# TheoCoombes/ClipCap

Measured on AMD Instinct MI355X. Metric: train samples/sec (512-d prefix, 40-tok caption), higher is better.
Workload: dtype bf16; 1 GPU; BASELINE configs[1]: TransformerMapper(8L,P=L=10,H=8)+frozen GPT-2-small; per_gpu_batch=256, global_batch=256, encoder_dim=512, train_language_model=False, parallelism=dp1

## Files before the change

clipcap_amd/csrc/api.hip:

```cpp
#include "../../include/clipcap_hip.h"
#include "gemm_api.h"
#include "kernels.h"
#include "shared.h"
#include "layout.h"
#include <vector>

using namespace CC_NS;

namespace {

#define CC_TIMED(site, st, expr)                 \
    do {                                         \
        cc_shared::ProfScope _ps(site, st);      \
        int _e = (expr);                         \
        if (_e != CC_OK) return _e;              \
    } while (0)

struct TileScope {
    int old;
    bool on;
    explicit TileScope(int mode) : old(cc_shared::g_gemm_tile_mode), on(mode != -2) { if (on) cc_shared::g_gemm_tile_mode = mode; }
    ~TileScope() { if (on) cc_shared::g_gemm_tile_mode = old; }
};
inline int env_tile(const char* name) {
// ... 29 lines not shown
    Carver cv(ws);
    const int S = c->W * c->P + c->L;
    const size_t M = (size_t)B * S, D = c->D;
    w.emb16 = cv.take<act_t>((size_t)B * c->W * c->E);
    w.lin_tmp = c->W > 1 ? cv.take<float>((size_t)B * c->W * c->P * D) : nullptr;
    const int nx = save ? c->N + 1 : 2;
    float* xb[MAX_LAYERS + 1];
    for (int i = 0; i < nx; i++) xb[i] = cv.take<float>(M * D);
    for (int l = 0; l <= c->N; l++) w.x[l] = save ? xb[l] : xb[l & 1];
    const int nl = save ? c->N : 1;
    for (int l = 0; l < c->N; l++) {
        const bool fresh = l < nl;
        w.x1[l] = fresh ? cv.take<float>(M * D) : w.x1[0];
        w.xn1[l] = fresh ? cv.take<act_t>(M * D) : w.xn1[0];
        w.xn2[l] = fresh ? cv.take<act_t>(M * D) : w.xn2[0];
        w.qkv[l] = fresh ? cv.take<act_t>(M * 3 * D) : w.qkv[0];
        w.att[l] = fresh ? cv.take<act_t>(M * D) : w.att[0];
        w.h[l] = fresh ? cv.take<act_t>(M * c->Hm) : w.h[0];
        w.lse[l] = fresh ? cv.take<float>((size_t)B * c->H * S) : w.lse[0];
        w.mean1[l] = fresh ? cv.take<float>(M) : w.mean1[0];
        w.rstd1[l] = fresh ? cv.take<float>(M) : w.rstd1[0];
        w.mean2[l] = fresh ? cv.take<float>(M) : w.mean2[0];
        w.rstd2[l] = fresh ? cv.take<float>(M) : w.rstd2[0];
    }
    if (save) {
        w.dx32 = cv.take<float>(M * D);
        w.dx16 = cv.take<act_t>(M * D);
        w.dx16b = cv.take<act_t>(M * D);
        w.dh16 = cv.take<act_t>(M * c->Hm);
        w.dxn16 = cv.take<act_t>(M * D);
        w.datt16 = cv.take<act_t>(M * D);
        w.dqkv16 = cv.take<act_t>(M * 3 * D);
        w.dlin16 = cv.take<act_t>((size_t)B * c->W * c->P * D);
        w.own_grads = !kX3 && M <= (size_t)kDeferRows && c->N <= 8;
        for (int l = 0; l < c->N; l++) {
            const bool own = w.own_grads;
            w.gdx[l] = own ? cv.take<act_t>(M * D) : w.dx16;
            w.gdxb[l] = own ? cv.take<act_t>(M * D) : w.dx16b;
            w.gdh[l] = own ? cv.take<act_t>(M * c->Hm) : w.dh16;
            w.gdqkv[l] = own ? cv.take<act_t>(M * 3 * D) : w.dqkv16;
        }
        w.wg_scratch = cv.take<float>(WGRAD_SCRATCH_BYTES / sizeof(float));
        w.red = cv.take<float>(RED_SCRATCH_FLOATS);
        w.adelta = cv.take<float>((size_t)B * c->H * S);
        w.gimg = kX3 ? reinterpret_cast<uint16_t*>(cv.take<char>(x3_img(M, std::max<size_t>(3 * (size_t)D, c->Hm)))) : nullptr;
    } else {
        w.dx32 = nullptr; w.dx16 = w.dx16b = w.dh16 = w.dxn16 = w.datt16 = w.dqkv16 = w.dlin16 = nullptr; w.wg_scratch = nullptr; w.adelta = nullptr;
        w.red = nullptr;
        w.gimg = nullptr;
        for (int l = 0; l < c->N; l++) w.gdx[l] = w.gdxb[l] = w.gdh[l] = w.gdqkv[l] = nullptr;
        w.own_grads = false;
    }
    w.x3 = nullptr; w.x3_bytes = 0;
    if (kX3) {
        const size_t Hm = c->Hm, Mb = (size_t)B * c->W, PD = (size_t)c->P * D;
        size_t need = std::max(x3_img(Mb, c->E), x3_img(M, std::max(D, Hm)));
        if (save) {
            need = std::max(need, x3_img(M, 3 * D));
            need = std::max(need, std::max(x3_img(M, D) + x3_img(M, Hm), x3_img(M, 3 * D) + x3_img(M, D)));
            need = std::max(need, x3_img(Mb, PD) + x3_img(Mb, c->E));
        }
        w.x3_bytes = need;
        w.x3 = cv.take<char>(need);
    }
    w.bytes = cv.bytes();
}

struct MapperPass {
    hipStream_t st;
    MapperOff o;
    MapperWS w;
    Call cx;
    int D, PP, S, M, H, hd, Hm, PD;
    MapperPass(const cc_mapper_cfg* c, int B, int save, void* ws, void* stream)
        : st(S_(stream)), o(c), D(c->D), PP(c->W * c->P), S(PP + c->L), M(B * S), H(c->H), hd(c->D / c->H), Hm(c->Hm), PD(c->P * c->D) {
        mapper_carve(c, B, save, ws, w);
        cx = call_of(st, w);
    }
};

static bool x3_img_on() {
    static const bool on = []() { const char* e = cc_lab_env("CC_X3_IMG"); return !e || atoi(e) != 0; }();
    return on;
}
static bool lm_exp_form(const cc_gpt2_shape* s) {
    static const bool env = []() { const char* e = cc_lab_env("CC_LM_EXPFORM"); return !e || atoi(e) != 0; }();
    if (CC_OP == 0) return env;
    if (CC_OP == 2) return env && x3_img_on() && s->mode == 1;
    return false;
}
static Act lm_logits(const cc_gpt2_cfg* c, const cc_gpt2_shape* s, act_t* logits16) { return Act(logits16, (kX3 && lm_exp_form(s)) ? c->Vp : 0); }

struct Gpt2WS {
    float* x[MAX_LAYERS + 1];
    float* x1[MAX_LAYERS];
    act_t *qkv[MAX_LAYERS], *u[MAX_LAYERS];
    Act xn1[MAX_LAYERS], xn2[MAX_LAYERS], att[MAX_LAYERS], hact[MAX_LAYERS];
    float *lse[MAX_LAYERS], *mean1[MAX_LAYERS], *rstd1[MAX_LAYERS], *mean2[MAX_LAYERS], *rstd2[MAX_LAYERS];
    act_t* hf16;
    float *meanf, *rstdf;
    int *target, *row_map;
    int* keep;
    act_t* logits16;
    float *pmax, *psum, *tgt_logit, *lse_row, *row_loss;
    float *cref, *lmfac;
    act_t* hfs16;
    float* dx32;
    Act dx16, dx16b, du16, dqkv16;
    act_t *dhf16, *dxn16, *datt16;
    float* wg_scratch;
    float* red;
    void* scat;
    float* adelta;
    char* x3;
    size_t x3_bytes;
    size_t bytes;
};

void gpt2_carve(const cc_gpt2_cfg* c, const cc_gpt2_shape* s, int cap, void* ws, Gpt2WS& w) {
    Carver cv(ws);
    const int B = s->B, T = s->T, hd = c->D / c->H;
    const size_t M = (size_t)B * T, D = c->D, Mc = (size_t)B * cap;
    const bool keep = s->mode >= 1, full = s->mode >= 2;
    const auto take_img = [&](size_t n) { return cv.take<act_t>(n * ((kX3 && !full) ? 3 : 2) / 2); };
    const bool img = kX3 && !full && x3_img_on();
    const bool bimg = img && keep && s->p_resid == 0.f && s->p_attn == 0.f && s->p_embd == 0.f;
    const int xw = img ? (int)D : 0, attw = (img && attn_fwd_can_image(T, hd)) ? (int)D : 0, hw = img ? 4 * (int)D : 0;
    const int dxw = bimg ? (int)D : 0, dqw = (bimg && attn_bwd_can_image(T, hd)) ? 3 * (int)D : 0;
    const int nx = keep ? c->NL + 1 : 2;
    float* xb[MAX_LAYERS + 1];
    for (int i = 0; i < nx; i++) xb[i] = cv.take<float>(M * D);
    for (int l = 0; l <= c->NL; l++) w.x[l] = keep ? xb[l] : xb[l & 1];
    for (int l = 0; l < c->NL; l++) {
        const bool k0 = keep || l == 0, f0 = full || l == 0;
        w.x1[l] = k0 ? cv.take<float>(M * D) : w.x1[0];
        w.qkv[l] = k0 ? cv.take<act_t>(M * 3 * D) : w.qkv[0];
        w.u[l] = k0 ? cv.take<act_t>(M * 4 * D) : w.u[0];
        w.lse[l] = k0 ? cv.take<float>((size_t)B * c->H * T) : w.lse[0];
        w.mean1[l] = k0 ? cv.take<float>(M) : w.mean1[0];
        w.rstd1[l] = k0 ? cv.take<float>(M) : w.rstd1[0];
        w.mean2[l] = k0 ? cv.take<float>(M) : w.mean2[0];
        w.rstd2[l] = k0 ? cv.take<float>(M) : w.rstd2[0];
        w.xn1[l] = f0 ? Act(take_img(M * D), xw) : w.xn1[0];
        w.xn2[l] = f0 ? Act(take_img(M * D), xw) : w.xn2[0];
        w.att[l] = k0 ? Act(take_img(M * D), attw) : w.att[0];
        w.hact[l] = f0 ? Act(take_img(M * 4 * D), hw) : w.hact[0];
    }
    const size_t Mh = std::max(M, Mc);
    w.hf16 = cv.take<act_t>(Mh * D);
    w.meanf = cv.take<float>(Mh);
    w.rstdf = cv.take<float>(Mh);
    w.target = cv.take<int>(Mh);
    w.row_map = cv.take<int>(Mh);
    w.keep = nullptr;
    if (keep) {
        const int npart = c->Vp / 64;
        w.logits16 = take_img(Mc * c->Vp);
        w.pmax = cv.take<float>(Mc * npart);
        w.psum = cv.take<float>(Mc * npart);
        w.tgt_logit = cv.take<float>(Mc);
        w.lse_row = cv.take<float>(Mc);
        w.row_loss = cv.take<float>(Mc);
        w.cref = cv.take<float>(Mc);
        w.lmfac = cv.take<float>(2 * Mc);
        w.hfs16 = full ? cv.take<act_t>(Mc * D) : nullptr;
        w.dx32 = cv.take<float>(M * D);
        w.dx16 = Act(take_img(M * D), dxw);
        w.dx16b = full ? Act(cv.take<act_t>(M * D)) : w.dx16;
        w.dhf16 = cv.take<act_t>(Mc * D);
        w.du16 = Act(take_img(M * 4 * D), hw);
        w.dxn16 = cv.take<act_t>(M * D);
        w.datt16 = cv.take<act_t>(M * D);
        w.dqkv16 = Act(take_img(M * 3 * D), dqw);
        w.wg_scratch = full ? cv.take<float>(WGRAD_SCRATCH_BYTES / sizeof(float)) : nullptr;
        w.red = full ? cv.take<float>(RED_SCRATCH_FLOATS) : nullptr;
        w.scat = full ? cv.take<char>(scatter_ws_bytes((int)Mc, (int)D)) : nullptr;
        w.adelta = cv.take<float>((size_t)B * c->H * T);
    } else {
        w.wg_scratch = nullptr; w.adelta = nullptr; w.red = nullptr; w.scat = nullptr;
        w.logits16 = nullptr; w.pmax = w.psum = w.tgt_logit = w.lse_row = w.row_loss = nullptr;
        w.cref = w.lmfac = nullptr; w.hfs16 = nullptr;
        w.dx32 = nullptr; w.dx16 = w.dx16b = w.du16 = w.dqkv16 = Act(); w.dhf16 = w.dxn16 = w.datt16 = nullptr;
        if (Mc > 0) {
            const int npart = c->Vp / 64;
            w.pmax = cv.take<float>(Mc * npart);
            w.psum = cv.take<float>(Mc * npart);
            w.tgt_logit = cv.take<float>(Mc);
            w.lse_row = cv.take<float>(Mc);
            w.keep = cv.take<int>(Mc);
        }
    }
    w.x3 = nullptr; w.x3_bytes = 0;
    if (kX3) {
        size_t need = x3_img(Mh, 4 * D);
        if (keep) need = std::max(need, x3_img(Mc, c->Vp));
        if (full) need = std::max(need, std::max(x3_img(M, D) + x3_img(M, 4 * D), x3_img(Mc, c->Vp) + x3_img(Mc, D)));
        w.x3_bytes = need;
        w.x3 = cv.take<char>(need);
    }
    w.bytes = cv.bytes();
}

struct Gpt2Pass {
    hipStream_t st;
    Gpt2Off o;
    Gpt2WS w;
    Call cx;
    int D, M, H, hd;
    Gpt2Pass(const cc_gpt2_cfg* c, const cc_gpt2_shape* s, int cap, void* ws, void* stream)
        : st(S_(stream)), o(c), D(c->D), M(s->B * s->T), H(c->H), hd(c->D / c->H) {
        gpt2_carve(c, s, cap, ws, w);
        cx = call_of(st, w);
    }
};

}

extern "C" {

int CC_API(cc_mapper_bwd_range)(const cc_mapper_cfg* c, int32_t B, const float* w32, const uint16_t* w16, void* ws, const float* dout, float* g32,
                        int32_t l_hi, int32_t l_lo, void* stream);
int CC_API(cc_gpt2_bwd_range)(const cc_gpt2_cfg* c, const cc_gpt2_shape* s, const float* w32, const uint16_t* w16, void* ws, const int64_t* tokens,
                      float* dprefix, float* g32, int32_t l_hi, int32_t l_lo, void* stream);

int64_t CC_API(cc_mapper_param_count)(const cc_mapper_cfg* cfg) {
    if (!mapper_cfg_ok(cfg)) return CC_ERR_SHAPE;
    return MapperOff(cfg).total;
}

int CC_API(cc_mapper_param_offsets)(const cc_mapper_cfg* cfg, int64_t* offs) {
    if (!mapper_cfg_ok(cfg) || !offs) return CC_ERR_SHAPE;
    const MapperOff o(cfg);
    *offs++ = o.lin_w; *offs++ = o.lin_b; *offs++ = o.prefix; *offs++ = o.pos;
    for (int l = 0; l < cfg->N; l++) offs = put_layer(offs, o.layer(l));
    return CC_OK;
}

int64_t CC_API(cc_mapper_ws_bytes)(const cc_mapper_cfg* cfg, int32_t B, int32_t save) {
    if (!mapper_cfg_ok(cfg) || B <= 0) return CC_ERR_SHAPE;
    MapperWS w;
    mapper_carve(cfg, B, save, nullptr, w);
    return (int64_t)w.bytes;
}

#if CC_OP == 2
static int mapper_sync_x3(const cc_mapper_cfg* c, const float* w32, uint16_t* w16, hipStream_t st) {
    const MapperOff o(c);
    const int D = c->D, Hm = c->Hm;
    X3SplitBatch sb;
    sb.add(w32 + o.lin_w, W16(w16, o.lin_w), c->P * D, c->E, 0, 1);
    for (int l = 0; l < c->N; l++) {
        const auto y = o.layer(l);
        const int64_t off[4] = {y.wq, y.wp, y.w1, y.w2};
        const int R[4] = {3 * D, D, Hm, D}, C[4] = {D, D, D, Hm};
        for (int i = 0; i < 4; i++) {
            if (sb.n + 2 > 32) { CC_TRY(x3_split_multi(sb, st)); sb.n = 0; }
            sb.add(w32 + off[i], W16(w16, off[i]), R[i], C[i], 0, 1);
            sb.add(w32 + off[i], W16(w16, o.total + off[i]), R[i], C[i], 1, 1);
        }
    }
    return x3_split_multi(sb, st);
}
#endif

static int mapper_transposes(const cc_mapper_cfg* c, uint16_t* w16, hipStream_t st) {
    if (kX3) return CC_ERR_ARG;
    const MapperOff o(c);
    op16_t* t = w16 + o.total;
    const int D = c->D, Hm = c->Hm;
    TransposeBatch tb;
    for (int l = 0; l < c->N; l++) {
        const auto y = o.layer(l);
        tb.add(w16 + y.wq, t + y.wq, 3 * D, D);
        tb.add(w16 + y.wp, t + y.wp, D, D);
        tb.add(w16 + y.w1, t + y.w1, Hm, D);
        tb.add(w16 + y.w2, t + y.w2, D, Hm);
        if (tb.n == 32) { CC_TRY(transpose_bf16_multi(tb, st)); tb.n = 0; }
    }
    CC_TRY(transpose_bf16_multi(tb, st));
    return CC_OK;
}

int CC_API(cc_mapper_sync_weights)(const cc_mapper_cfg* c, const float* w32, uint16_t* w16, void* stream) {
    if (!mapper_cfg_ok(c) || !w32 || !w16) return CC_ERR_ARG;
    hipStream_t st = S_(stream);
#if CC_OP == 2
    return mapper_sync_x3(c, w32, w16, st);
#else
    CC_TRY(f32_to_bf16(w32, w16, (size_t)MapperOff(c).total, st));
    return mapper_transposes(c, w16, st);
#endif
}

int CC_API(cc_mapper_transpose_weights)(const cc_mapper_cfg* c, uint16_t* w16, void* stream) {
    if (!mapper_cfg_ok(c) || !w16) return CC_ERR_ARG;
    return mapper_transposes(c, w16, S_(stream));
}

int CC_API(cc_mapper_fwd)(const cc_mapper_cfg* c, int32_t B, const float* w32, const uint16_t* w16, const float* emb, void* ws, float* out,
                  int32_t save, void* stream) {
    if (!mapper_cfg_ok(c) || B <= 0 || !w32 || !w16 || !emb || !ws || !out) return CC_ERR_ARG;
    MapperPass ps(c, B, save, ws, stream);
    auto& [st, o, w, cx, D, PP, S, M, H, hd, Hm, PD] = ps;
    CC_TRY(f32_to_act(emb, w.emb16, (size_t)B * c->W * c->E, st));
    if (c->W == 1) {
        CC_TRY(gemm_f32out(0, 0, w.emb16, c->E, W16(w16, o.lin_w), c->E, B, PD, c->E, w.x[0], S * D, w32 + o.lin_b, 0, 1.0f, 1, cx));
    } else {
        CC_TRY(gemm_f32out(0, 0, w.emb16, c->E, W16(w16, o.lin_w), c->E, B * c->W, PD, c->E, w.lin_tmp, PD, w32 + o.lin_b, 0, 1.0f, 1, cx));
        CC_TRY(copy_rows(w.lin_tmp, (size_t)PP * D, w.x[0], (size_t)S * D, PP * D, B, st));
        if (o.pos >= 0) CC_TRY(add_rows(w.x[0], (size_t)S * D, w32 + o.pos, PP * D, B, st));
    }
    CC_TRY(broadcast_rows(w.x[0] + (size_t)PP * D, (size_t)S * D, w32 + o.prefix, c->L * D, B, st));
    for (int l = 0; l < c->N; l++) {
        const auto y = o.layer(l);
        CC_TRY(ln_fwd(w.x[l], D, nullptr, w32 + y.n1w, w32 + y.n1b, w.xn1[l], nullptr, w.mean1[l], w.rstd1[l], M, D, st));
        CC_TIMED(CC_SITE_MAPPER_QKV_FWD, st, gemm_bf16out(0, 0, w.xn1[l], D, W16(w16, y.wq), D, M, 3 * D, D, w.qkv[l], 3 * D, nullptr, 0, nullptr, cx));
        CC_TRY(attn_fwd(w.qkv[l], B, S, H, hd, false, w.att[l], w.lse[l], st));
        CC_TRY(gemm_resid(0, 0, w.att[l], D, W16(w16, y.wp), D, M, D, D, w.x1[l], w.x[l], D, w32 + y.bp, cx));
        CC_TRY(ln_fwd(w.x1[l], D, nullptr, w32 + y.n2w, w32 + y.n2b, w.xn2[l], nullptr, w.mean2[l], w.rstd2[l], M, D, st));
        CC_TIMED(CC_SITE_MAPPER_FC1_FWD, st, gemm_bf16out(0, 0, w.xn2[l], D, W16(w16, y.w1), D, M, Hm, D, w.h[l], Hm, w32 + y.b1, 1, nullptr, cx));
        CC_TRY(gemm_resid(0, 0, w.h[l], Hm, W16(w16, y.w2), Hm, M, D, Hm, w.x[l + 1], w.x1[l], D, w32 + y.b2, cx));
    }
    CC_TRY(copy_rows(w.x[c->N] + (size_t)PP * D, (size_t)S * D, out, (size_t)c->L * D, c->L * D, B, st));
    return CC_OK;
}

int CC_API(cc_mapper_attention_probs)(const cc_mapper_cfg* c, int32_t B, void* ws, int32_t layer, float* out, void* stream) {
    if (!mapper_cfg_ok(c) || B <= 0 || !ws || !out || layer < 0 || layer >= c->N) return CC_ERR_ARG;
    MapperPass ps(c, B, 1, ws, stream);
    return attn_probs(ps.w.qkv[layer], B, ps.S, ps.H, ps.hd, out, ps.st);
}

int CC_API(cc_mapper_bwd)(const cc_mapper_cfg* c, int32_t B, const float* w32, const uint16_t* w16, void* ws, const float* dout, float* g32,
                  void* stream) {
    if (!mapper_cfg_ok(c)) return CC_ERR_ARG;
    return CC_API(cc_mapper_bwd_range)(c, B, w32, w16, ws, dout, g32, c->N, 0, stream);
}

int CC_API(cc_mapper_bwd_range)(const cc_mapper_cfg* c, int32_t B, const float* w32, const uint16_t* w16, void* ws, const float* dout, float* g32,
                        int32_t l_hi, int32_t l_lo, void* stream) {
    if (!mapper_cfg_ok(c) || B <= 0 || !w32 || !w16 || !ws || !dout || !g32 || l_lo < 0 || l_hi > c->N || l_lo > l_hi) return CC_ERR_ARG;
    MapperPass ps(c, B, 1, ws, stream);
    auto& [st, o, w, cx, D, PP, S, M, H, hd, Hm, PD] = ps;
    const uint16_t* w16t = W16(w16, o.total);
    if (l_hi == c->N) {
        if (hipMemsetAsync(w.dx32, 0, (size_t)M * D * sizeof(float), st) != hipSuccess) return CC_ERR_LAUNCH;
        CC_TRY(copy_rows(dout, (size_t)c->L * D, w.dx32 + (size_t)PP * D, (size_t)S * D, c->L * D, B, st));
        if (c->N > 0) CC_TRY(f32_to_act(w.dx32, w.gdx[c->N - 1], (size_t)M * D, st));
    }
    WgradBatch wb;
    wb.defer = true;
    constexpr bool kDeferAll = !kX3;
    static const bool defer_all_on = []() { const char* e = cc_lab_env("CC_MAPPER_WGRAD_DEFER"); return !e || atoi(e) != 0; }();
    static const int defer_rows = []() { const char* e = cc_lab_env("CC_MAPPER_DEFER_ROWS"); return e ? std::min(atoi(e), kDeferRows) : kDeferRows; }();
    const bool defer_all = kDeferAll && defer_all_on && w.own_grads && 4 * (l_hi - l_lo) <= 32 && M <= defer_rows;
    if (defer_all) { wb.direct = true; wb.cap = 4 * (l_hi - l_lo); }
    ColsumBatch cs;
#if CC_OP == 2
    static const bool share = []() { const char* e = cc_lab_env("CC_X3_SHARE"); return !e || atoi(e) != 0; }();
    int g2rc = CC_OK;
    auto G2 = [&](const act_t* t, int width) -> ActIn {
        if (!share) return t;
        auto& [st, o, w, cx, D, PP, S, M, H, hd, Hm, PD] = ps;
        g2rc = x3_split_rows(t, (size_t)width, w.gimg, M, width, 0, st);
        return ActIn(reinterpret_cast<const act_t*>(w.gimg), width);
    };
#else
    auto G2 = [&](const act_t* t, int) -> ActIn { return t; };
    const int g2rc = CC_OK;
#endif
    for (int l = l_hi - 1; l >= l_lo; l--) {
        const auto y = o.layer(l);
        act_t* dx16 = w.gdx[l];
        act_t* dx16b = w.gdxb[l];
        act_t* dh16 = w.gdh[l];
        act_t* dqkv16 = w.gdqkv[l];
        act_t* dx16_below = l > 0 ? w.gdx[l - 1] : w.datt16;
        const ActIn gx = G2(dx16, D);
        CC_TRY(g2rc);
        CC_TIMED(CC_SITE_MAPPER_WGRAD_FC2, st, gemm_wgrad(gx, D, w.h[l], Hm, D, Hm, M, g32 + y.w2, Hm, w.wg_scratch, cx, &wb));
        if (l == c->N - 1) CC_TRY(colsum_bf16(dx16, D, M, D, g32 + y.b2, cx));
        CC_TRY(gemm_dact(0, 0, gx, D, W16(w16t, y.w2), D, M, Hm, D, dh16, Hm, w.h[l], 1, cx));
        const ActIn gh = G2(dh16, Hm);
        CC_TRY(g2rc);
        CC_TRY(gemm_wgrad(gh, Hm, w.xn2[l], D, Hm, D, M, g32 + y.w1, D, w.wg_scratch, cx, &wb));
        if (defer_all) cs.add(dh16, g32 + y.b1);
        else CC_TRY(colsum_bf16(dh16, Hm, M, Hm, g32 + y.b1, cx));
        CC_TRY(gemm_bf16out(0, 0, gh, Hm, W16(w16t, y.w1), Hm, M, D, Hm, w.dxn16, D, nullptr, 0, nullptr, cx));
        CC_TRY(ln_bwd(w.dxn16, w.x1[l], D, nullptr, w.mean2[l], w.rstd2[l], w32 + y.n2w, w.dx32, w.dx32, dx16b, g32 + y.n2w,
                      g32 + y.n2b, M, D, cx, g32 + y.bp));
        const ActIn gb = G2(dx16b, D);
        CC_TRY(g2rc);
        CC_TRY(gemm_wgrad(gb, D, w.att[l], D, D, D, M, g32 + y.wp, D, w.wg_scratch, cx, &wb));
        CC_TRY(gemm_bf16out(0, 0, gb, D, W16(w16t, y.wp), D, M, D, D, w.datt16, D, nullptr, 0, nullptr, cx));
        CC_TRY(attn_bwd(w.qkv[l], w.datt16, w.att[l], w.lse[l], w.adelta, B, S, H, hd, false, dqkv16, st));
        const ActIn gq = G2(dqkv16, 3 * D);
        CC_TRY(g2rc);
        CC_TRY(gemm_wgrad(gq, 3 * D, w.xn1[l], D, 3 * D, D, M, g32 + y.wq, D, w.wg_scratch, cx, &wb));
        CC_TRY(gemm_bf16out(0, 0, gq, 3 * D, W16(w16t, y.wq), 3 * D, M, D, 3 * D, w.dxn16, D, nullptr, 0, nullptr, cx));
        if (!defer_all) CC_TRY(wgrad_flush(wb, st));
        CC_TRY(ln_bwd(w.dxn16, w.x[l], D, nullptr, w.mean1[l], w.rstd1[l], w32 + y.n1w, w.dx32, w.dx32, dx16_below, g32 + y.n1w,
                      g32 + y.n1b, M, D, cx, l > 0 ? g32 + o.layer(l - 1).b2 : nullptr));
    }
    CC_TRY(wgrad_flush(wb, st));
    CC_TRY(colsum_bf16_multi(cs, Hm, M, Hm, cx));
    if (l_lo > 0) return CC_OK;
    CC_TRY(batch_sum(w.dx32 + (size_t)PP * D, (size_t)S * D, g32 + o.prefix, c->L * D, B, cx));
    if (o.pos >= 0) CC_TRY(batch_sum(w.dx32, (size_t)S * D, g32 + o.pos, PP * D, B, cx));
    CC_TRY(slice_f32_to_bf16(w.dx32, (size_t)S * D, w.dlin16, (size_t)PP * D, PP * D, B, st));
    CC_TRY(gemm_wgrad(w.dlin16, PD, w.emb16, c->E, PD, c->E, B * c->W, g32 + o.lin_w, c->E, w.wg_scratch, cx));
    CC_TRY(colsum_bf16(w.dlin16, PD, B * c->W, PD, g32 + o.lin_b, cx));
    return CC_OK;
}

namespace {
static bool gelu_grad_fwd() {
    static const bool on = []() { const char* e = cc_lab_env("CC_GELU_GRAD_FWD"); return !e || atoi(e) != 0; }();
    return on;
}
static bool shape_ok(const cc_gpt2_cfg* c, const cc_gpt2_shape* s) {
    return s && s->B > 0 && s->T > 0 && s->L >= 0 && s->L <= s->T && s->cap >= s->T - s->L && s->mode >= 0 && s->mode <= 2 && s->T <= c->NPOS &&
           s->p_embd >= 0.f && s->p_embd < 1.f && s->p_attn >= 0.f && s->p_attn < 1.f && s->p_resid >= 0.f && s->p_resid < 1.f;
}
}

int64_t CC_API(cc_gpt2_param_count)(const cc_gpt2_cfg* cfg) {
    if (!gpt2_cfg_ok(cfg)) return CC_ERR_SHAPE;
    return Gpt2Off(cfg).total;
}

int CC_API(cc_gpt2_param_offsets)(const cc_gpt2_cfg* cfg, int64_t* offs) {
    if (!gpt2_cfg_ok(cfg) || !offs) return CC_ERR_SHAPE;
    const Gpt2Off o(cfg);
    *offs++ = o.wte; *offs++ = o.wpe;
    for (int l = 0; l < cfg->NL; l++) offs = put_layer(offs, o.layer(l));
    *offs++ = o.lnf_w; *offs++ = o.lnf_b;
    return CC_OK;
}

int64_t CC_API(cc_gpt2_ws_bytes)(const cc_gpt2_cfg* cfg, const cc_gpt2_shape* s) {
    if (!gpt2_cfg_ok(cfg) || !shape_ok(cfg, s)) return CC_ERR_SHAPE;
    Gpt2WS w;
    gpt2_carve(cfg, s, s->T - s->L, nullptr, w);
    return (int64_t)w.bytes;
}

#if CC_OP == 2
static int gpt2_sync_x3(const cc_gpt2_cfg* c, const float* w32, uint16_t* w16, hipStream_t st) {
    const Gpt2Off o(c);
    const int D = c->D;
    X3SplitBatch sb;
    sb.add(w32 + o.wte, W16(w16, o.wte), c->Vp, D, 0, 1);
    sb.add(w32 + o.wte, W16(w16, o.total + o.wte), c->Vp, D, 1, 1);
    CC_TRY(x3_split_multi(sb, st));
    sb.n = 0;
    for (int l = 0; l < c->NL; l++) {
        const auto y = o.layer(l);
        const int64_t off[4] = {y.aw, y.pw, y.fw, y.p2w};
        const int R[4] = {D, D, D, 4 * D}, C[4] = {3 * D, D, 4 * D, D};
        for (int i = 0; i < 4; i++) {
            if (sb.n + 2 > 32) { CC_TRY(x3_split_multi(sb, st)); sb.n = 0; }
            sb.add(w32 + off[i], W16(w16, off[i]), R[i], C[i], 0, 1);
            sb.add(w32 + off[i], W16(w16, o.total + off[i]), R[i], C[i], 1, 1);
        }
    }
    return x3_split_multi(sb, st);
}
#endif

static int gpt2_transposes(const cc_gpt2_cfg* c, uint16_t* w16, hipStream_t st) {
    if (kX3) return CC_ERR_ARG;
    const Gpt2Off o(c);
    op16_t* t = w16 + o.total;
    const int D = c->D;
    CC_TRY(transpose_bf16(w16 + o.wte, t + o.wte, c->Vp, D, st));
    TransposeBatch tb;
    for (int l = 0; l < c->NL; l++) {
        const auto y = o.layer(l);
        tb.add(w16 + y.aw, t + y.aw, D, 3 * D);
        tb.add(w16 + y.pw, t + y.pw, D, D);
        tb.add(w16 + y.fw, t + y.fw, D, 4 * D);
        tb.add(w16 + y.p2w, t + y.p2w, 4 * D, D);
        if (tb.n == 32) { CC_TRY(transpose_bf16_multi(tb, st)); tb.n = 0; }
    }
    CC_TRY(transpose_bf16_multi(tb, st));
    return CC_OK;
}

int CC_API(cc_gpt2_sync_weights)(const cc_gpt2_cfg* c, const float* w32, uint16_t* w16, void* stream) {
    if (!gpt2_cfg_ok(c) || !w32 || !w16) return CC_ERR_ARG;
    hipStream_t st = S_(stream);
#if CC_OP == 2
    return gpt2_sync_x3(c, w32, w16, st);
#else
    CC_TRY(f32_to_bf16(w32, w16, (size_t)Gpt2Off(c).total, st));
    return gpt2_transposes(c, w16, st);
#endif
}

int CC_API(cc_gpt2_transpose_weights)(const cc_gpt2_cfg* c, uint16_t* w16, void* stream) {
    if (!gpt2_cfg_ok(c) || !w16) return CC_ERR_ARG;
    return gpt2_transposes(c, w16, S_(stream));
}

int CC_API(cc_dropout_mask)(uint64_t seed, int32_t site, int32_t layer, float p, int64_t n, uint8_t* out, void* stream) {
    if (!out || n < 0 || site < 0 || site > 3 || layer < 0 || layer > 255 || p < 0.f || p >= 1.f) return CC_ERR_ARG;
    return dropout_mask_u8(out, (size_t)n, make_drop(p, seed, (unsigned)site, (unsigned)layer), S_(stream));
}

int CC_API(cc_gpt2_embed)(const cc_gpt2_cfg* c, const cc_gpt2_shape* s, const float* w32, const float* prefix, const int64_t* tokens, void* ws,
                  void* stream) {
    if (!gpt2_cfg_ok(c) || !shape_ok(c, s) || !w32 || !ws || (s->L > 0 && !prefix) || (s->T > s->L && !tokens)) return CC_ERR_ARG;
    Gpt2Pass ps(c, s, s->T - s->L, ws, stream);
    auto& [st, o, w, cx, D, M, H, hd] = ps;
    CC_TRY(embed_concat(prefix, reinterpret_cast<const long long*>(tokens), s->cap, w32 + o.wte, w32 + o.wpe, w.x[0], s->B, s->L, s->T, D, 0, st));
    return dropout_f32(w.x[0], (size_t)s->B * s->T * D, make_drop(s->p_embd, s->drop_seed, DROP_EMBD, 0), st);
}

int CC_API(cc_gpt2_embed_from)(const cc_gpt2_cfg* c, const cc_gpt2_shape* s, const float* w32, const float* inputs_embeds, void* ws,
                       void* stream) {
    if (!gpt2_cfg_ok(c) || !shape_ok(c, s) || !w32 || !ws || !inputs_embeds) return CC_ERR_ARG;
    Gpt2Pass ps(c, s, s->T - s->L, ws, stream);
    return embed_concat(inputs_embeds, nullptr, 0, w32 + ps.o.wte, w32 + ps.o.wpe, ps.w.x[0], s->B, s->T, s->T, ps.D, 0, ps.st);
}

int CC_API(cc_gpt2_fwd)(const cc_gpt2_cfg* c, const cc_gpt2_shape* s, const float* w32, const uint16_t* w16, void* ws, void* stream) {
    if (!gpt2_cfg_ok(c) || !shape_ok(c, s) || !w32 || !w16 || !ws) return CC_ERR_ARG;
    Gpt2Pass ps(c, s, s->T - s->L, ws, stream);
    auto& [st, o, w, cx, D, M, H, hd] = ps;
    const uint16_t* w16t = W16(w16, o.total);
    for (int l = 0; l < c->NL; l++) {
        const auto y = o.layer(l);
        CC_TRY(ln_fwd(w.x[l], D, nullptr, w32 + y.l1w, w32 + y.l1b, w.xn1[l], nullptr, w.mean1[l], w.rstd1[l], M, D, st));
        CC_TRY(gemm_bf16out(0, 0, w.xn1[l], D, W16(w16t, y.aw), D, M, 3 * D, D, w.qkv[l], 3 * D, w32 + y.ab, 0, nullptr, cx));
        CC_TRY(attn_fwd(w.qkv[l], s->B, s->T, H, hd, true, w.att[l], w.lse[l], st, make_drop(s->p_attn, s->drop_seed, DROP_ATTN, l)));
        {
            static const int tile_proj = env_tile("CC_TILE_PROJ");
            TileScope ts(tile_proj);
            CC_TRY(gemm_resid(0, 0, w.att[l], D, W16(w16t, y.pw), D, M, D, D, w.x1[l], w.x[l], D, w32 + y.pb, cx,
                              make_drop(s->p_resid, s->drop_seed, DROP_RESID_ATTN, l)));
        }
        CC_TRY(ln_fwd(w.x1[l], D, nullptr, w32 + y.l2w, w32 + y.l2b, w.xn2[l], nullptr, w.mean2[l], w.rstd2[l], M, D, st));
        {
            static const int tile_fc = env_tile("CC_TILE_FC");
            TileScope ts(tile_fc);
            CC_TIMED(CC_SITE_GPT2_FC_FWD, st, gemm_bf16out(0, 0, w.xn2[l], D, W16(w16t, y.fw), D, M, 4 * D, D, w.hact[l], 4 * D, w32 + y.fb, (s->mode >= 1 && gelu_grad_fwd()) ? 3 : 2,
                                                            s->mode >= 1 ? w.u[l] : nullptr, cx));
        }
        {
            static const int tile_proj2 = env_tile("CC_TILE_PROJ2");
            TileScope ts(tile_proj2);
            CC_TIMED(CC_SITE_GPT2_PROJ2_FWD, st, gemm_resid(0, 0, w.hact[l], 4 * D, W16(w16t, y.p2w), 4 * D, M, D, 4 * D, w.x[l + 1], w.x1[l], D, w32 + y.p2b, cx,
                                                           make_drop(s->p_resid, s->drop_seed, DROP_RESID_MLP, l)));
        }
    }
    return CC_OK;
}

int CC_API(cc_gpt2_logits)(const cc_gpt2_cfg* c, const cc_gpt2_shape* s, const float* w32, const uint16_t* w16, void* ws, float* logits,
                   int64_t ldl, void* stream) {
    if (!gpt2_cfg_ok(c) || !shape_ok(c, s) || !w32 || !w16 || !ws || !logits) return CC_ERR_ARG;
    const int Ns = std::min(c->Vp, rup(c->V, 8));
    if (ldl < Ns || (ldl & 3) || ldl > 0x7fffffff) return CC_ERR_SHAPE;
    Gpt2Pass ps(c, s, s->T - s->L, ws, stream);
    auto& [st, o, w, cx, D, M, H, hd] = ps;
    CC_TRY(ln_fwd(w.x[c->NL], D, nullptr, w32 + o.lnf_w, w32 + o.lnf_b, w.hf16, nullptr, w.meanf, w.rstdf, M, D, st));
    return gemm_f32out(0, 0, w.hf16, D, W16(w16, o.wte), D, M, Ns, D, logits, (int)ldl, nullptr, 0, 1.0f, 1, cx);
}

int CC_API(cc_lmhead_ce_fwd)(const cc_gpt2_cfg* c, const cc_gpt2_shape* s, const float* w32, const uint16_t* w16, void* ws, const int64_t* tokens,
                     float* stats, void* stream) {
    if (!gpt2_cfg_ok(c) || !shape_ok(c, s) || s->mode < 1 || s->L < 1 || !w32 || !w16 || !ws || !tokens || !stats) return CC_ERR_ARG;
    const int cap = s->T - s->L;
    if (cap != s->cap) return CC_ERR_SHAPE;
    Gpt2Pass ps(c, s, cap, ws, stream);
    auto& [st, o, w, cx, D, M, H, hd] = ps;
    const int Mc = s->B * cap, npart = c->Vp / 64;
    if (hipMemsetAsync(stats, 0, 2 * sizeof(float), st) != hipSuccess) return CC_ERR_LAUNCH;
    CC_TRY(ce_targets(reinterpret_cast<const long long*>(tokens), w.target, w.row_map, s->B, cap, s->L, s->T, st));
    CC_TRY(ln_fwd(w.x[c->NL], D, w.row_map, w32 + o.lnf_w, w32 + o.lnf_b, w.hf16, nullptr, w.meanf, w.rstdf, Mc, D, st));
    const bool ef = lm_exp_form(s);
    const op16_t* wte_rows = kX3 ? reinterpret_cast<const op16_t*>(w32 + o.wte) : W16(w16, o.wte);
    if (ef) CC_TRY(lm_tgt_ref(w.hf16, wte_rows, D, w.target, w.cref, Mc, st));
    CC_TIMED(CC_SITE_LMHEAD_FWD, st, gemm_lmhead(w.hf16, D, W16(w16, o.wte), D, Mc, c->Vp, c->V, D, lm_logits(c, s, w.logits16), c->Vp, w.pmax, w.psum, npart, w.target, w.tgt_logit, cx,
                                                 ef ? w.cref : nullptr));
    CC_TRY(ce_rows(w.pmax, w.psum, npart, w.target, ef ? w.cref : w.tgt_logit, w.lse_row, w.row_loss, stats, Mc, st));
    return CC_OK;
}

int CC_API(cc_lmhead_score)(const cc_gpt2_cfg* c, const cc_gpt2_shape* s, const float* w32, const uint16_t* w16, void* ws, const int64_t* tokens,
                    int32_t ignore_zero, float* token_logprob, float* sample_stats, void* stream) {
    if (!gpt2_cfg_ok(c) || !shape_ok(c, s) || s->mode != 0 || s->L < 1 || !w32 || !w16 || !ws || !tokens || !token_logprob || !sample_stats)
        return CC_ERR_ARG;
    const int cap = s->T - s->L;
    if (cap < 1 || cap != s->cap) return CC_ERR_SHAPE;
    Gpt2Pass ps(c, s, cap, ws, stream);
    auto& [st, o, w, cx, D, M, H, hd] = ps;
    const int Mc = s->B * cap, npart = c->Vp / 64;
    CC_TRY(ce_targets(reinterpret_cast<const long long*>(tokens), w.target, w.row_map, s->B, cap, s->L, s->T, st));
    CC_TRY(score_keep(reinterpret_cast<const long long*>(tokens), w.keep, Mc, ignore_zero, st));
    CC_TRY(ln_fwd(w.x[c->NL], D, w.row_map, w32 + o.lnf_w, w32 + o.lnf_b, w.hf16, nullptr, w.meanf, w.rstdf, Mc, D, st));
    CC_TIMED(CC_SITE_LMHEAD_FWD, st, gemm_lmhead_score(w.hf16, D, W16(w16, o.wte), D, Mc, c->Vp, c->V, D, w.pmax, w.psum, npart, w.target, w.tgt_logit, cx));
    return score_rows(w.pmax, w.psum, npart, w.keep, w.tgt_logit, w.lse_row, token_logprob, sample_stats, s->B, cap, st);
}

int CC_API(cc_lmhead_ce_bwd)(const cc_gpt2_cfg* c, const cc_gpt2_shape* s, const float* w32, const uint16_t* w16, void* ws, const float* denom,
                     const float* loss_scale, float* g32, void* stream) {
    if (!gpt2_cfg_ok(c) || !shape_ok(c, s) || s->mode < 1 || !w32 || !w16 || !ws || !denom || (s->mode == 2 && !g32)) return CC_ERR_ARG;
    const int cap = s->T - s->L;
    Gpt2Pass ps(c, s, cap, ws, stream);
    auto& [st, o, w, cx, D, M, H, hd] = ps;
    const int Mc = s->B * cap;
    const bool full = s->mode == 2;
    const bool ef = lm_exp_form(s);
    const LmFix fix{w.lmfac, w.target, kX3 ? reinterpret_cast<const op16_t*>(w32 + o.wte) : W16(w16, o.wte)};
    if (ef) CC_TRY(lm_rowfac(w.cref, w.lse_row, w.target, denom, loss_scale, w.lmfac, Mc, st));
    const Act lg = lm_logits(c, s, w.logits16);
    ActIn dlog = lg;
    op16_t* dimg = (kX3 && !ef && !full && x3_img_on()) ? x3_scratch_block(cx, x3_img(Mc, c->Vp)) : nullptr;
    if (dimg) dlog = ActIn(reinterpret_cast<const act_t*>(dimg), c->Vp);
    if (!ef) CC_TRY(ce_dlogits(w.logits16, c->Vp, c->V, w.target, w.lse_row, denom, loss_scale, Mc, st, dimg));
    const auto lm_dgrad = [&]() {
        auto& [st, o, w, cx, D, M, H, hd] = ps;
        const int rc = gemm_nt_deepk(dlog, c->Vp, W16(w16, o.total + o.wte), c->Vp, Mc, D, c->Vp, w.dhf16, D, reinterpret_cast<float*>(w.du16.p),
                                     (size_t)M * 4 * D * sizeof(act_t), cx, ef ? &fix : nullptr);
        if (rc != CC_ERR_SHAPE) return rc;
        const int rc2 = gemm_bf16out(0, 0, dlog, c->Vp, W16(w16, o.total + o.wte), c->Vp, Mc, D, c->Vp, w.dhf16, D, nullptr, 0, nullptr, cx);
        return (rc2 != CC_OK || !ef) ? rc2 : lm_dgrad_fix(w.dhf16, w.lmfac, w.target, fix.wte, D, Mc, st);
    };
    CC_TIMED(CC_SITE_LMHEAD_DGRAD, st, lm_dgrad());
    if (full) {
        if (ef) {
            CC_TRY(lm_scale_rows(w.hf16, w.lmfac, w.hfs16, D, Mc, st));
            CC_TRY(gemm_wgrad(lg, c->Vp, w.hfs16, D, c->Vp, D, Mc, g32 + o.wte, D, w.wg_scratch, cx));
            ScatterSrc oh;
            oh.ids32 = w.target; oh.act = w.hf16; oh.fac = w.lmfac;
            CC_TRY(scatter_rows(oh, Mc, D, c->Vp, g32 + o.wte, w.scat, st));
        } else {
            CC_TRY(gemm_wgrad(lg, c->Vp, w.hf16, D, c->Vp, D, Mc, g32 + o.wte, D, w.wg_scratch, cx));
        }
    }
    if (hipMemsetAsync(w.dx32, 0, (size_t)M * D * sizeof(float), st) != hipSuccess) return CC_ERR_LAUNCH;
    const size_t dx16_bytes = (size_t)M * D * (w.dx16.img ? 3 * sizeof(op16_t) : sizeof(act_t));
    if (hipMemsetAsync(w.dx16.p, 0, dx16_bytes, st) != hipSuccess) return CC_ERR_LAUNCH;
    CC_TRY(ln_bwd(w.dhf16, w.x[c->NL], D, w.row_map, w.meanf, w.rstdf, w32 + o.lnf_w, nullptr, w.dx32, w.dx16, full ? g32 + o.lnf_w : nullptr,
                  full ? g32 + o.lnf_b : nullptr, Mc, D, cx));
    return CC_OK;
}

int CC_API(cc_lmhead_put_x)(const cc_gpt2_cfg* c, const cc_gpt2_shape* s, void* ws, const float* x, void* stream) {
    if (!gpt2_cfg_ok(c) || !shape_ok(c, s) || !ws || !x) return CC_ERR_ARG;
    Gpt2Pass ps(c, s, s->T - s->L, ws, stream);
    const size_t bytes = (size_t)s->B * s->T * c->D * sizeof(float);
    return hipMemcpyAsync(ps.w.x[c->NL], x, bytes, hipMemcpyDeviceToDevice, ps.st) == hipSuccess ? CC_OK : CC_ERR_LAUNCH;
}

int CC_API(cc_lmhead_get)(const cc_gpt2_cfg* c, const cc_gpt2_shape* s, void* ws, int32_t field, void* dst, int64_t dst_bytes, void* stream) {
    if (!gpt2_cfg_ok(c) || !shape_ok(c, s) || !ws || !dst || field < CC_LM_LSE || field > CC_LM_DX32) return CC_ERR_ARG;
    if (s->T - s->L < 1) return CC_ERR_SHAPE;
    Gpt2Pass ps(c, s, s->T - s->L, ws, stream);
    const Gpt2WS& w = ps.w;
    const size_t Mc = (size_t)s->B * (s->T - s->L), M = (size_t)s->B * s->T, D = c->D;
    const void* src = nullptr;
    size_t bytes = 0;
    switch (field) {
        case CC_LM_LSE: src = w.lse_row; bytes = Mc * sizeof(float); break;
        case CC_LM_TGT: src = (s->mode >= 1 && lm_exp_form(s)) ? w.cref : w.tgt_logit; bytes = Mc * sizeof(float); break;
        case CC_LM_ROW_LOSS: src = w.row_loss; bytes = Mc * sizeof(float); break;
        case CC_LM_HF: src = w.hf16; bytes = Mc * D * sizeof(act_t); break;
        case CC_LM_DHF: src = w.dhf16; bytes = Mc * D * sizeof(act_t); break;
        default: src = w.dx32; bytes = M * D * sizeof(float); break;
    }
    if (!src) return CC_ERR_STATE;
    if (dst_bytes < 0 || (size_t)dst_bytes != bytes) return CC_ERR_SHAPE;
    return hipMemcpyAsync(dst, src, bytes, hipMemcpyDeviceToDevice, ps.st) == hipSuccess ? CC_OK : CC_ERR_LAUNCH;
}

int CC_API(cc_gpt2_logits_bwd)(const cc_gpt2_cfg* c, const cc_gpt2_shape* s, const float* w32, const uint16_t* w16, void* ws, const float* dlogits,
                       int64_t ldl, float* dx0, float* g32, void* stream) {
    if (!gpt2_cfg_ok(c) || !shape_ok(c, s) || s->mode < 1 || s->L != 0 || !w32 || !w16 || !ws || !dlogits || ldl < c->V || (s->mode == 2 && !g32))
        return CC_ERR_ARG;
    Gpt2Pass ps(c, s, s->T, ws, stream);
    auto& [st, o, w, cx, D, M, H, hd] = ps;
    const bool full = s->mode == 2;
    CC_TRY(f32_to_op16_pad(dlogits, ldl, c->V, w.logits16, c->Vp, M, st));
    CC_TRY(gemm_bf16out(0, 0, w.logits16, c->Vp, W16(w16, o.total + o.wte), c->Vp, M, D, c->Vp, w.dhf16, D, nullptr, 0, nullptr, cx));
    if (full) CC_TRY(gemm_wgrad(w.logits16, c->Vp, w.hf16, D, c->Vp, D, M, g32 + o.wte, D, w.wg_scratch, cx));
    if (hipMemsetAsync(w.dx32, 0, (size_t)M * D * sizeof(float), st) != hipSuccess) return CC_ERR_LAUNCH;
    CC_TRY(ln_bwd(w.dhf16, w.x[c->NL], D, nullptr, w.meanf, w.rstdf, w32 + o.lnf_w, nullptr, w.dx32, w.dx16, full ? g32 + o.lnf_w : nullptr,
                  full ? g32 + o.lnf_b : nullptr, M, D, cx));
    CC_TRY(CC_API(cc_gpt2_bwd_range)(c, s, w32, w16, ws, nullptr, nullptr, g32, c->NL, 0, stream));
    if (dx0 && hipMemcpyAsync(dx0, w.dx32, (size_t)M * D * sizeof(float), hipMemcpyDeviceToDevice, st) != hipSuccess) return CC_ERR_LAUNCH;
    return CC_OK;
}

int CC_API(cc_gpt2_bwd)(const cc_gpt2_cfg* c, const cc_gpt2_shape* s, const float* w32, const uint16_t* w16, void* ws, const int64_t* tokens,
                float* dprefix, float* g32, void* stream) {
    if (!gpt2_cfg_ok(c)) return CC_ERR_ARG;
    return CC_API(cc_gpt2_bwd_range)(c, s, w32, w16, ws, tokens, dprefix, g32, c->NL, 0, stream);
}

int CC_API(cc_gpt2_bwd_range)(const cc_gpt2_cfg* c, const cc_gpt2_shape* s, const float* w32, const uint16_t* w16, void* ws, const int64_t* tokens,
                      float* dprefix, float* g32, int32_t l_hi, int32_t l_lo, void* stream) {
    if (!gpt2_cfg_ok(c) || !shape_ok(c, s) || s->mode < 1 || !w32 || !w16 || !ws || (s->L > 0 && !dprefix) || (s->mode == 2 && !g32) ||
        l_lo < 0 || l_hi > c->NL || l_lo > l_hi)
        return CC_ERR_ARG;
    Gpt2Pass ps(c, s, s->T - s->L, ws, stream);
    auto& [st, o, w, cx, D, M, H, hd] = ps;
    const int D3 = 3 * D, D4 = 4 * D;
    const bool full = s->mode == 2;
    WgradBatch wb;
    wb.defer = full;
    WgradBatch* wbp = full ? &wb : nullptr;
    if (full && (w.dx16.img || w.dx16b.img || w.du16.img || w.dqkv16.img)) return CC_ERR_STATE;
    for (int l = l_hi - 1; l >= l_lo; l--) {
        const auto y = o.layer(l);
        const bool top = l == c->NL - 1;
        if (top) CC_TRY(dropout_bf16(w.dx16.p, (size_t)M * D, make_drop(s->p_resid, s->drop_seed, DROP_RESID_MLP, l), st));
        if (full) {
            CC_TRY(gemm_wgrad(w.hact[l], D4, w.dx16.p, D, D4, D, M, g32 + y.p2w, D, w.wg_scratch, cx, wbp));
            if (top) CC_TRY(colsum_bf16(w.dx16.p, D, M, D, g32 + y.p2b, cx));
        }
        {
            static const int tile_dact = env_tile("CC_TILE_DACT");
            TileScope ts(tile_dact);
            CC_TRY(gemm_dact(0, 0, w.dx16, D, W16(w16, y.p2w), D, M, D4, D, w.du16, D4, w.u[l], gelu_grad_fwd() ? 3 : 2, cx));
        }
        if (full) {
            CC_TRY(gemm_wgrad(w.xn2[l], D, w.du16.p, D4, D, D4, M, g32 + y.fw, D4, w.wg_scratch, cx, wbp));
            CC_TRY(colsum_bf16(w.du16.p, D4, M, D4, g32 + y.fb, cx));
        }
        CC_TIMED(CC_SITE_GPT2_FC_DGRAD, st, gemm_bf16out(0, 0, w.du16, D4, W16(w16, y.fw), D4, M, D, D4, w.dxn16, D, nullptr, 0, nullptr, cx));
        CC_TRY(ln_bwd(w.dxn16, w.x1[l], D, nullptr, w.mean2[l], w.rstd2[l], w32 + y.l2w, w.dx32, w.dx32, w.dx16b, full ? g32 + y.l2w : nullptr,
                      full ? g32 + y.l2b : nullptr, M, D, cx, full ? g32 + y.pb : nullptr,
                      make_drop(s->p_resid, s->drop_seed, DROP_RESID_ATTN, l)));
        if (full) CC_TRY(gemm_wgrad(w.att[l], D, w.dx16b.p, D, D, D, M, g32 + y.pw, D, w.wg_scratch, cx, wbp));
        CC_TRY(gemm_bf16out(0, 0, w.dx16b, D, W16(w16, y.pw), D, M, D, D, w.datt16, D, nullptr, 0, nullptr, cx));
        CC_TRY(attn_bwd(w.qkv[l], w.datt16, w.att[l].p, w.lse[l], w.adelta, s->B, s->T, H, hd, true, w.dqkv16, st,
                        make_drop(s->p_attn, s->drop_seed, DROP_ATTN, l)));
        if (full) {
            CC_TRY(gemm_wgrad(w.xn1[l], D, w.dqkv16.p, D3, D, D3, M, g32 + y.aw, D3, w.wg_scratch, cx, wbp));
            CC_TRY(colsum_bf16(w.dqkv16.p, D3, M, D3, g32 + y.ab, cx));
        }
        CC_TRY(gemm_bf16out(0, 0, w.dqkv16, D3, W16(w16, y.aw), D3, M, D, D3, w.dxn16, D, nullptr, 0, nullptr, cx));
        if (full) CC_TRY(wgrad_flush(wb, st));
        CC_TRY(ln_bwd(w.dxn16, w.x[l], D, nullptr, w.mean1[l], w.rstd1[l], w32 + y.l1w, w.dx32, w.dx32, w.dx16, full ? g32 + y.l1w : nullptr,
                      full ? g32 + y.l1b : nullptr, M, D, cx, (full && l > 0) ? g32 + o.layer(l - 1).p2b : nullptr,
                      l > 0 ? make_drop(s->p_resid, s->drop_seed, DROP_RESID_MLP, l - 1) : Drop()));
    }
    if (l_lo > 0) return CC_OK;
    CC_TRY(dropout_f32(w.dx32, (size_t)M * D, make_drop(s->p_embd, s->drop_seed, DROP_EMBD, 0), st));
    if (s->L > 0) CC_TRY(copy_rows(w.dx32, (size_t)s->T * D, dprefix, (size_t)s->L * D, s->L * D, s->B, st));
    if (full) {
        if (tokens) {
            ScatterSrc e;
            e.ids64 = reinterpret_cast<const long long*>(tokens);
            e.ids_ld = s->cap;
            e.f32 = w.dx32 + (size_t)s->L * D; e.rpb = s->T - s->L; e.bstride = (size_t)s->T * D;
            CC_TRY(scatter_rows(e, s->B * (s->T - s->L), D, c->Vp, g32 + o.wte, w.scat, st));
        }
        CC_TRY(batch_sum(w.dx32, (size_t)s->T * D, g32 + o.wpe, s->T * D, s->B, cx));
    }
    return CC_OK;
}

int CC_API(cc_adamw_step)(float* p32, const float* g32, float* m, float* v, int64_t n, float lr, float beta1, float beta2, float eps,
                  float weight_decay, int32_t step, float grad_scale, const float* loss_scale, const float* found_inf, void* stream) {
    if (!p32 || !g32 || !m || !v || n < 0 || step < 0 || (step == 0 && !loss_scale)) return CC_ERR_ARG;
    return adamw(p32, g32, m, v, (size_t)n, lr, beta1, beta2, eps, weight_decay, step, grad_scale, loss_scale, found_inf, S_(stream));
}

int CC_API(cc_adamw_step_cast)(float* p32, const float* g32, float* m, float* v, int64_t n, float lr, float beta1, float beta2, float eps,
                       float weight_decay, int32_t step, float grad_scale, const float* loss_scale, const float* found_inf, uint16_t* w16, void* stream) {
    if (!p32 || !g32 || !m || !v || !w16 || n < 0 || step < 0 || (step == 0 && !loss_scale)) return CC_ERR_ARG;
    if (kX3) return CC_ERR_ARG;
    return adamw(p32, g32, m, v, (size_t)n, lr, beta1, beta2, eps, weight_decay, step, grad_scale, loss_scale, found_inf, S_(stream), w16);
}

int CC_API(cc_adamw_step_clip)(float* p32, const float* g32, float* m, float* v, int64_t n, float lr, float beta1, float beta2, float eps,
                       float weight_decay, int32_t step, float grad_scale, const float* loss_scale, const float* found_inf, const float* clip,
                       uint16_t* w16, void* stream) {
    if (!p32 || !g32 || !m || !v || n < 0 || step < 0 || (step == 0 && !loss_scale)) return CC_ERR_ARG;
    if (w16 && kX3) return CC_ERR_ARG;
    return adamw(p32, g32, m, v, (size_t)n, lr, beta1, beta2, eps, weight_decay, step, grad_scale, loss_scale, found_inf, S_(stream), w16, clip);
}

int64_t CC_API(cc_grad_norm_scratch_floats)(void) { return (int64_t)GRAD_NORM_BLOCKS; }

int CC_API(cc_grad_sqnorm)(const float* g32, int64_t n, float* scratch, float* sumsq, void* stream) {
    if (!g32 || !scratch || !sumsq || n < 0) return CC_ERR_ARG;
    return grad_sqnorm(g32, (size_t)n, scratch, sumsq, S_(stream));
}

int CC_API(cc_grad_clip_coef)(const float* sumsq, float max_norm, float grad_scale, const float* loss_scale, float* clip, void* stream) {
    if (!sumsq || !clip || !(max_norm >= 0.f)) return CC_ERR_ARG;
    return grad_clip_coef(sumsq, max_norm, grad_scale, loss_scale, clip, S_(stream));
}

int CC_API(cc_cast_op16)(const float* src, uint16_t* dst, int64_t n, void* stream) {
    if (!src || !dst || n < 0 || kX3) return CC_ERR_ARG;
    return f32_to_bf16(src, dst, (size_t)n, S_(stream));
}

int CC_API(cc_grad_wire_pack)(const float* g32, uint16_t* wire, int64_t n, void* stream) {
    if (!g32 || !wire || n < 0) return CC_ERR_ARG;
    return wire_pack(g32, wire, (size_t)n, S_(stream));
}

int CC_API(cc_grad_wire_unpack)(const uint16_t* wire, float* g32, int64_t n, void* stream) {
    if (!g32 || !wire || n < 0) return CC_ERR_ARG;
    return wire_unpack(wire, g32, (size_t)n, S_(stream));
}

int CC_API(cc_grad_nonfinite)(const float* g32, int64_t n, float* found_inf, void* stream) {
    if (!g32 || !found_inf || n < 0) return CC_ERR_ARG;
    return grad_nonfinite(g32, (size_t)n, found_inf, S_(stream));
}

int CC_API(cc_loss_scale_update)(float* state, float* found_inf, float growth, float backoff, int32_t interval, void* stream) {
    if (!state || !found_inf || growth < 1.f || backoff <= 0.f || backoff > 1.f || interval < 1) return CC_ERR_ARG;
    return loss_scale_update(state, found_inf, growth, backoff, interval, S_(stream));
}

int CC_API(cc_gemm_op16_f32)(int32_t al, int32_t bl, const uint16_t* A, int32_t lda, const uint16_t* B, int32_t ldb, int32_t M, int32_t N, int32_t K,
                     float* C, int32_t ldc, const float* bias, int32_t ksplit, void* stream) {
    if (!A || !B || !C || kX3) return CC_ERR_ARG;
    Call cx{S_(stream)};
    return gemm_f32out(al, bl, reinterpret_cast<const act_t*>(A), lda, B, ldb, M, N, K, C, ldc, ksplit > 1 ? nullptr : bias, ksplit > 1 ? 2 : 0, 1.0f, ksplit, cx);
}

int64_t CC_API(cc_wgrad_scratch_bytes)(void) { return (int64_t)WGRAD_SCRATCH_BYTES; }

int CC_API(cc_gemm_wgrad)(const uint16_t* X, int32_t ldx, const uint16_t* Y, int32_t ldy, int32_t Mw, int32_t Nw, int32_t K, float* dW, int32_t ldw,
                  float* scratch, void* stream) {
    if (!X || !Y || !dW || kX3) return CC_ERR_ARG;
    Call cx{S_(stream)};
    return gemm_wgrad(reinterpret_cast<const act_t*>(X), ldx, reinterpret_cast<const act_t*>(Y), ldy, Mw, Nw, K, dW, ldw, scratch, cx);
}

int CC_API(cc_layernorm_fwd)(const float* x, const float* gamma, const float* beta, uint16_t* y, float* mean, float* rstd, int32_t rows, int32_t D,
                     void* stream) {
    if (!x || !gamma || !beta || !y) return CC_ERR_ARG;
    return ln_fwd(x, D, nullptr, gamma, beta, reinterpret_cast<act_t*>(y), nullptr, mean, rstd, rows, D, S_(stream));
}

int64_t CC_API(cc_red_scratch_floats)(void) { return (int64_t)RED_SCRATCH_FLOATS; }

int CC_API(cc_layernorm_bwd)(const uint16_t* dy, const float* x, int32_t ldx, const int32_t* row_map, const float* mean, const float* rstd,
                     const float* gamma, const float* dres, float* dx32, uint16_t* dx16, float* dgamma, float* dbeta, float* dcol, int32_t rows,
                     int32_t D, float* red_ws, void* stream) {
    if (!dy || !x || !mean || !rstd || !gamma || !dx32 || !dgamma != !dbeta || kX3) return CC_ERR_ARG;
    Call cx{S_(stream), red_ws};
    return ln_bwd(reinterpret_cast<const act_t*>(dy), x, ldx, row_map, mean, rstd, gamma, dres, dx32, reinterpret_cast<act_t*>(dx16), dgamma,
                  dbeta, rows, D, cx, dcol);
}

int CC_API(cc_colsum_bf16)(const uint16_t* X, int32_t ld, int32_t M, int32_t N, float* out, float* red_ws, void* stream) {
    if (!X || !out || kX3) return CC_ERR_ARG;
    Call cx{S_(stream), red_ws};
    return colsum_bf16(reinterpret_cast<const act_t*>(X), ld, M, N, out, cx);
}

int CC_API(cc_colsum_multi)(const uint16_t* const* X_host, float* const* out_host, int32_t n, int32_t ld, int32_t M, int32_t N, float* red_ws,
                    void* stream) {
    if (!X_host || !out_host || n < 0 || n > 32 || kX3) return CC_ERR_ARG;
    ColsumBatch b;
    for (int i = 0; i < n; i++) {
        if (!X_host[i] || !out_host[i]) return CC_ERR_ARG;
        b.add(reinterpret_cast<const act_t*>(X_host[i]), out_host[i]);
    }
    Call cx{S_(stream), red_ws};
    return colsum_bf16_multi(b, ld, M, N, cx);
}

int CC_API(cc_batch_sum)(const float* src, int64_t src_stride, float* dst, int32_t len, int32_t B, float* red_ws, void* stream) {
    if (!src || !dst || len < 0 || src_stride < len) return CC_ERR_ARG;
    Call cx{S_(stream), red_ws};
    return batch_sum(src, (size_t)src_stride, dst, len, B, cx);
}

int CC_API(cc_attention_fwd)(const uint16_t* qkv, int32_t B, int32_t S, int32_t H, int32_t hd, int32_t causal, uint16_t* out, float* lse, void* stream) {
    if (!qkv || !out) return CC_ERR_ARG;
    return attn_fwd(reinterpret_cast<const act_t*>(qkv), B, S, H, hd, causal != 0, reinterpret_cast<act_t*>(out), lse, S_(stream));
}

int CC_API(cc_attention_bwd)(const uint16_t* qkv, const uint16_t* dout, const uint16_t* o, const float* lse, float* delta_ws, int32_t B, int32_t S,
                     int32_t H, int32_t hd, int32_t causal, uint16_t* dqkv, void* stream) {
    if (!qkv || !dout || !lse || !dqkv) return CC_ERR_ARG;
    return attn_bwd(reinterpret_cast<const act_t*>(qkv), reinterpret_cast<const act_t*>(dout), reinterpret_cast<const act_t*>(o), lse, delta_ws, B, S, H, hd,
                    causal != 0, reinterpret_cast<act_t*>(dqkv), S_(stream));
}

int CC_API(cc_attention_fwd_x)(const uint16_t* qkv, int32_t B, int32_t S, int32_t H, int32_t hd, int32_t causal, uint16_t* out, int32_t out_img, float* lse,
                       float p, uint64_t seed, int32_t layer, void* stream) {
    if (!qkv || !out || !(p >= 0.f && p < 1.f) || layer < 0 || layer > 255 || out_img < 0 || (!kX3 && out_img)) return CC_ERR_ARG;
    return attn_fwd(reinterpret_cast<const act_t*>(qkv), B, S, H, hd, causal != 0, Act(reinterpret_cast<act_t*>(out), out_img), lse, S_(stream),
                    make_drop(p, seed, DROP_ATTN, (unsigned)layer));
}

int CC_API(cc_attention_bwd_x)(const uint16_t* qkv, const uint16_t* dout, const uint16_t* o, const float* lse, float* delta_ws, int32_t B, int32_t S,
                       int32_t H, int32_t hd, int32_t causal, uint16_t* dqkv, int32_t dqkv_img, float p, uint64_t seed, int32_t layer, void* stream) {
    if (!qkv || !dout || !lse || !dqkv || !(p >= 0.f && p < 1.f) || layer < 0 || layer > 255 || dqkv_img < 0 || (!kX3 && dqkv_img)) return CC_ERR_ARG;
    return attn_bwd(reinterpret_cast<const act_t*>(qkv), reinterpret_cast<const act_t*>(dout), reinterpret_cast<const act_t*>(o), lse, delta_ws, B, S, H, hd,
                    causal != 0, Act(reinterpret_cast<act_t*>(dqkv), dqkv_img), S_(stream), make_drop(p, seed, DROP_ATTN, (unsigned)layer));
}

namespace {
inline bool al16(const void* p) { return ((uintptr_t)p & 15) == 0; }
inline bool hook_operands_ok(int al, int bl, const void* A, int a_img, int lda, const void* B, int ldb, int M, int N, int K) {
    if (!A || !B || !al16(A) || !al16(B) || M <= 0 || N <= 0 || K <= 0 || a_img < 0) return false;
    if (!kX3 && a_img) return false;
    return lda >= (a_img ? 0 : (al ? M : K)) && ldb >= (bl ? N : K);
}
inline void hook_scratch(Call& cx, void* x3, int64_t x3_bytes) {
    if (kX3 && x3 && x3_bytes > 0 && al16(x3)) { cx.x3 = static_cast<char*>(x3); cx.x3_bytes = (size_t)x3_bytes; }
}
inline bool hook_c_img_ok(int c_img, int N) { return c_img == 0 || (kX3 && c_img == N); }
}

int64_t CC_API(cc_x3_image_bytes)(int64_t rows, int64_t depth) {
    if (rows < 0 || depth < 0) return CC_ERR_ARG;
    return (int64_t)x3_img((size_t)rows, (size_t)depth);
}

int CC_API(cc_x3_split_rows)(const float* src, int64_t ld, int32_t rows, int32_t width, int32_t form, uint16_t* dst, void* stream) {
#if CC_OP == 2
    if (!src || !dst || rows < 0 || width < 0 || ld < width || (form != 0 && form != 1)) return CC_ERR_ARG;
    return x3_split_rows(src, (size_t)ld, dst, rows, width, form, S_(stream));
#else
    (void)src; (void)ld; (void)rows; (void)width; (void)form; (void)dst; (void)stream;
    return CC_ERR_ARG;
#endif
}

int CC_API(cc_gemm_act)(int32_t al, int32_t bl, const void* A, int32_t a_img, int32_t lda, const uint16_t* B, int32_t ldb, int32_t M, int32_t N, int32_t K,
                void* C, int32_t c_img, int32_t ldc, const float* bias, int32_t act, void* pre, void* x3, int64_t x3_bytes, void* stream) {
    if (!hook_operands_ok(al, bl, A, a_img, lda, B, ldb, M, N, K) || !C || !al16(C) || !al16(pre) || !al16(bias) || ldc < N || act < 0 || act > 3 ||
        !hook_c_img_ok(c_img, N))
        return CC_ERR_ARG;
    Call cx{S_(stream)};
    hook_scratch(cx, x3, x3_bytes);
    return gemm_bf16out(al, bl, ActIn(static_cast<const act_t*>(A), a_img), lda, B, ldb, M, N, K, Act(static_cast<act_t*>(C), c_img), ldc, bias, act,
                        static_cast<act_t*>(pre), cx);
}

int CC_API(cc_gemm_resid)(int32_t al, int32_t bl, const void* A, int32_t a_img, int32_t lda, const uint16_t* B, int32_t ldb, int32_t M, int32_t N, int32_t K,
                  float* out, const float* res, int32_t ld, const float* bias, float p, uint64_t seed, int32_t site, int32_t layer, void* x3,
                  int64_t x3_bytes, void* stream) {
    if (!hook_operands_ok(al, bl, A, a_img, lda, B, ldb, M, N, K) || !out || !res || !al16(out) || !al16(res) || !al16(bias) || ld < N || site < 0 ||
        site > 3 || layer < 0 || layer > 255 || p < 0.f || p >= 1.f)
        return CC_ERR_ARG;
    Call cx{S_(stream)};
    hook_scratch(cx, x3, x3_bytes);
    return gemm_resid(al, bl, ActIn(static_cast<const act_t*>(A), a_img), lda, B, ldb, M, N, K, out, res, ld, bias, cx,
                      make_drop(p, seed, (unsigned)site, (unsigned)layer));
}

int CC_API(cc_gemm_dact)(int32_t al, int32_t bl, const void* A, int32_t a_img, int32_t lda, const uint16_t* B, int32_t ldb, int32_t M, int32_t N, int32_t K,
                 void* C, int32_t c_img, int32_t ldc, const void* aux, int32_t act, void* x3, int64_t x3_bytes, void* stream) {
    if (!hook_operands_ok(al, bl, A, a_img, lda, B, ldb, M, N, K) || !C || !aux || !al16(C) || !al16(aux) || ldc < N || act < 1 || act > 3 ||
        !hook_c_img_ok(c_img, N))
        return CC_ERR_ARG;
    Call cx{S_(stream)};
    hook_scratch(cx, x3, x3_bytes);
    return gemm_dact(al, bl, ActIn(static_cast<const act_t*>(A), a_img), lda, B, ldb, M, N, K, Act(static_cast<act_t*>(C), c_img), ldc,
                     static_cast<const act_t*>(aux), act, cx);
}

int CC_API(cc_gemm_f32)(int32_t al, int32_t bl, const void* A, int32_t a_img, int32_t lda, const uint16_t* B, int32_t ldb, int32_t M, int32_t N, int32_t K,
                float* C, int32_t ldc, const float* bias, int32_t mode, float alpha, int32_t ksplit, void* x3, int64_t x3_bytes, void* stream) {
    if (!hook_operands_ok(al, bl, A, a_img, lda, B, ldb, M, N, K) || !C || !al16(C) || !al16(bias) || ldc < N || mode < 0 || mode > 2 || ksplit < 1 ||
        (bias && mode != 0))
        return CC_ERR_ARG;
    Call cx{S_(stream)};
    hook_scratch(cx, x3, x3_bytes);
    return gemm_f32out(al, bl, ActIn(static_cast<const act_t*>(A), a_img), lda, B, ldb, M, N, K, C, ldc, bias, mode, alpha, ksplit, cx);
}

int CC_API(cc_gemm_wgrad_split)(const void* X, int32_t x_img, int32_t ldx, const float* Y, int32_t ldy, int32_t Mw, int32_t Nw, int32_t K, float* dW,
                     int32_t ldw, float* scratch, void* x3, int64_t x3_bytes, void* stream) {
#if CC_OP == 2
    if (!X || !Y || !dW || !al16(X) || !al16(Y) || !al16(dW) || Mw <= 0 || Nw <= 0 || K <= 0 || x_img < 0 || (!x_img && ldx < Mw) || ldy < Nw || ldw < Nw)
        return CC_ERR_ARG;
    Call cx{S_(stream)};
    hook_scratch(cx, x3, x3_bytes);
    return gemm_wgrad(ActIn(static_cast<const act_t*>(X), x_img), ldx, Y, ldy, Mw, Nw, K, dW, ldw, scratch, cx);
#else
    (void)X; (void)x_img; (void)ldx; (void)Y; (void)ldy; (void)Mw; (void)Nw; (void)K; (void)dW; (void)ldw; (void)scratch; (void)x3; (void)x3_bytes; (void)stream;
    return CC_ERR_ARG;
#endif
}

}
```

clipcap_amd/csrc/gemm.hip.h:

```cpp
#pragma once
#include <cstdlib>
#include <type_traits>
#include "common.hip.h"
#include "gemm_api.h"

namespace CC_NS {

constexpr int G_BM = 128, G_BN = 128, G_BK = 64, G_THREADS = 256;
constexpr int G_TILE_BYTES = G_BM * G_BK * 2;
constexpr int G_EPI_LD = 68;

struct GemmShape {
    int M, N, K;
    int lda, ldb;
    int k_chunk;
    int group_m;
    int stagger;
    int flags = 0;
};

__device__ __forceinline__ int g_lds_off(int row, int chunk) {
    return row * 128 + (((chunk ^ (row >> 1) ^ ((row >> 4) & 3)) & 7) << 4);
}

// ... 1475 lines not shown
    __device__ __forceinline__ void bias8(int col, float (&b)[8]) const { load_bias8(bias, col, Ns, b); }
    __device__ __forceinline__ void fin(int row, int col, float (&v)[8], const float (&b)[8]) const {
        if (row >= M || col >= Ns) return;
#pragma unroll
        for (int e = 0; e < 8; e++) v[e] += b[e];
        act_st8(C + (size_t)row * ldc + col, v);
    }
};

struct EpiResid {
    float* out;
    const float* res;
    const float* bias;
    int ld, M, Ns;
    Drop drop;
    __device__ __forceinline__ void operator()(int row, int col, float (&v)[8]) const {
        if (row >= M || col >= Ns) return;
        const size_t o = (size_t)row * ld + col;
        const float4 r0 = *reinterpret_cast<const float4*>(res + o);
        const float4 r1 = *reinterpret_cast<const float4*>(res + o + 4);
        float4 b0 = make_float4(0, 0, 0, 0), b1 = b0;
        if (bias) {
            b0 = *reinterpret_cast<const float4*>(bias + col);
            b1 = *reinterpret_cast<const float4*>(bias + col + 4);
        }
        float y[8] = {v[0] + b0.x, v[1] + b0.y, v[2] + b0.z, v[3] + b0.w, v[4] + b1.x, v[5] + b1.y, v[6] + b1.z, v[7] + b1.w};
        if (drop.thresh) {
#pragma unroll
            for (int e = 0; e < 8; e += 2) {
                float m0, m1;
                drop_mul_pair(drop, (unsigned)o + e, m0, m1);
                y[e] *= m0; y[e + 1] *= m1;
            }
        }
        const float r[8] = {r0.x, r0.y, r0.z, r0.w, r1.x, r1.y, r1.z, r1.w};
        store_sum(o, r, y);
    }
    bool acc_init = false;
    __device__ __forceinline__ bool init_from_input() const { return acc_init; }
    __device__ __forceinline__ void init4(int row, int col, f32x4& a) const {
        if (row >= M || col >= Ns) return;
        const float4 r = *reinterpret_cast<const float4*>(res + (size_t)row * ld + col);
        a[0] = r.x; a[1] = r.y; a[2] = r.z; a[3] = r.w;
    }
    static constexpr bool kPre = true;
    __device__ __forceinline__ void pre4(int row, int col, f32x4& a) const {
        if (acc_init || row >= M || col >= Ns) return;
        const size_t o = (size_t)row * ld + col;
        const float4 r = *reinterpret_cast<const float4*>(res + o);
        if (drop.thresh) {
            float4 b = make_float4(0, 0, 0, 0);
            if (bias) b = *reinterpret_cast<const float4*>(bias + col);
            float m0, m1, m2, m3;
            drop_mul_pair(drop, (unsigned)o, m0, m1);
            drop_mul_pair(drop, (unsigned)o + 2, m2, m3);
            a[0] = r.x + m0 * (a[0] + b.x);
            a[1] = r.y + m1 * (a[1] + b.y);
            a[2] = r.z + m2 * (a[2] + b.z);
            a[3] = r.w + m3 * (a[3] + b.w);
            return;
        }
        a[0] += r.x; a[1] += r.y; a[2] += r.z; a[3] += r.w;
    }
    __device__ __forceinline__ void bias8(int col, float (&b)[8]) const { load_bias8(drop.thresh ? nullptr : bias, col, Ns, b); }
    __device__ __forceinline__ void fin(int row, int col, float (&v)[8], const float (&b)[8]) const {
        if (row >= M || col >= Ns) return;
        store_sum((size_t)row * ld + col, v, b);
    }
  private:
    __device__ __forceinline__ void store_sum(size_t o, const float (&x)[8], const float (&y)[8]) const {
        *reinterpret_cast<float4*>(out + o) = make_float4(x[0] + y[0], x[1] + y[1], x[2] + y[2], x[3] + y[3]);
        *reinterpret_cast<float4*>(out + o + 4) = make_float4(x[4] + y[4], x[5] + y[5], x[6] + y[6], x[7] + y[7]);
    }
};

struct EpiF32 {
    float* C;
    const float* bias;
    int ldc, M, Ns;
    int mode;
    float alpha;
    size_t zstride = 0;
    __device__ __forceinline__ void operator()(int row, int col, float (&v)[8]) const {
        if (row >= M || col >= Ns) return;
        float* p = C + (size_t)row * ldc + col + (mode == 3 ? blockIdx.z * zstride : 0);
        if (mode == 2) {
#pragma unroll
            for (int e = 0; e < 8; e++) __hip_atomic_fetch_add(p + e, alpha * v[e], __ATOMIC_RELAXED, __HIP_MEMORY_SCOPE_AGENT);
            return;
        }
        float4 o0 = make_float4(alpha * v[0], alpha * v[1], alpha * v[2], alpha * v[3]);
        float4 o1 = make_float4(alpha * v[4], alpha * v[5], alpha * v[6], alpha * v[7]);
        if (mode == 0 && bias) {
            const float4 b0 = *reinterpret_cast<const float4*>(bias + col);
            const float4 b1 = *reinterpret_cast<const float4*>(bias + col + 4);
            o0.x += b0.x; o0.y += b0.y; o0.z += b0.z; o0.w += b0.w; o1.x += b1.x; o1.y += b1.y; o1.z += b1.z; o1.w += b1.w;
        }
        if (mode == 1) {
            const float4 c0 = *reinterpret_cast<const float4*>(p);
            const float4 c1 = *reinterpret_cast<const float4*>(p + 4);
            o0.x += c0.x; o0.y += c0.y; o0.z += c0.z; o0.w += c0.w; o1.x += c1.x; o1.y += c1.y; o1.z += c1.z; o1.w += c1.w;
        }
        *reinterpret_cast<float4*>(p) = o0;
        *reinterpret_cast<float4*>(p + 4) = o1;
    }
    static constexpr bool kPre = true;
    __device__ __forceinline__ void pre4(int row, int col, f32x4& a) const {
        a[0] *= alpha; a[1] *= alpha; a[2] *= alpha; a[3] *= alpha;
        if (mode != 1 || row >= M || col >= Ns) return;
        const float4 c = *reinterpret_cast<const float4*>(C + (size_t)row * ldc + col);
        a[0] += c.x; a[1] += c.y; a[2] += c.z; a[3] += c.w;
    }
    __device__ __forceinline__ void bias8(int col, float (&b)[8]) const { load_bias8(mode == 0 ? bias : nullptr, col, Ns, b); }
    __device__ __forceinline__ void fin(int row, int col, float (&v)[8], const float (&b)[8]) const {
        if (row >= M || col >= Ns) return;
        float* p = C + (size_t)row * ldc + col + (mode == 3 ? blockIdx.z * zstride : 0);
        if (mode == 2) {
#pragma unroll
            for (int e = 0; e < 8; e++) __hip_atomic_fetch_add(p + e, v[e], __ATOMIC_RELAXED, __HIP_MEMORY_SCOPE_AGENT);
            return;
        }
        *reinterpret_cast<float4*>(p) = make_float4(v[0] + b[0], v[1] + b[1], v[2] + b[2], v[3] + b[3]);
        *reinterpret_cast<float4*>(p + 4) = make_float4(v[4] + b[4], v[5] + b[5], v[6] + b[6], v[7] + b[7]);
    }
};

template <int ACT = -1>
struct EpiDActT {
    act_t* C;
    const act_t* aux;
    int ldc, M, Ns;
    int act;
    int img = 0;
    __device__ __forceinline__ int act_() const { return ACT >= 0 ? ACT : act; }
    __device__ __forceinline__ void operator()(int row, int col, float (&v)[8]) const {
        if (row >= M || col >= Ns) return;
        const size_t o = (size_t)row * ldc + col;
        float a[8];
        act_ld8(aux + o, a);
        if (act_() == 1) {
#pragma unroll
            for (int e = 0; e < 8; e++) v[e] = a[e] > 0.f ? v[e] : 0.f;
        } else if (act_() == 3) {
#pragma unroll
            for (int e = 0; e < 8; e++) v[e] *= a[e];
        } else {
#pragma unroll
            for (int e = 0; e < 8; e++) v[e] *= gelu_new_grad(a[e]);
        }
        epi_store8(C, ldc, row, col, v, img);
    }
    typedef act_raw8 StripAux;
    __device__ __forceinline__ act_raw8 load_aux(int row, int col) const {
        return (row < M && col < Ns) ? act_ldraw8(aux + (size_t)row * ldc + col) : act_zero8();
    }
    __device__ __forceinline__ void operator()(int row, int col, float (&v)[8], const act_raw8& ax) const {
        if (row >= M || col >= Ns) return;
        float a[8];
        act_unpack8(ax, a);
        if (act_() == 1) {
#pragma unroll
            for (int e = 0; e < 8; e++) v[e] = a[e] > 0.f ? v[e] : 0.f;
        } else if (act_() == 3) {
#pragma unroll
            for (int e = 0; e < 8; e++) v[e] *= a[e];
        } else {
#pragma unroll
            for (int e = 0; e < 8; e++) v[e] *= gelu_new_grad(a[e]);
        }
        epi_store8(C, ldc, row, col, v, img);
    }
    static constexpr bool kPre = true;
    __device__ __forceinline__ void pre4(int row, int col, f32x4& a) const {
        if (row >= M || col >= Ns) return;
        float x[4];
        act_unpack4(act_ldraw4(aux + (size_t)row * ldc + col), x[0], x[1], x[2], x[3]);
#pragma unroll
        for (int e = 0; e < 4; e++) a[e] = act_() == 1 ? (x[e] > 0.f ? a[e] : 0.f) : (act_() == 3 ? a[e] * x[e] : a[e] * gelu_new_grad(x[e]));
    }
    __device__ __forceinline__ void bias8(int, float (&b)[8]) const {
#pragma unroll
        for (int e = 0; e < 8; e++) b[e] = 0.f;
    }
    __device__ __forceinline__ void fin(int row, int col, float (&v)[8], const float (&)[8]) const {
        if (row >= M || col >= Ns) return;
        epi_store8(C, ldc, row, col, v, img);
    }
};
using EpiDAct = EpiDActT<>;
template <class E> struct epi_is_dact { static constexpr bool value = false; };
template <int A> struct epi_is_dact<EpiDActT<A>> { static constexpr bool value = true; };

template <int LO, int HI>
__device__ __forceinline__ float xor_max(float m) {
#pragma unroll
    for (int d = LO; d <= HI; d <<= 1) m = fmaxf(m, __shfl_xor(m, d, 64));
    return m;
}
template <int LO, int HI>
__device__ __forceinline__ float xor_sum(float s) {
#pragma unroll
    for (int d = LO; d <= HI; d <<= 1) s += __shfl_xor(s, d, 64);
    return s;
}
__device__ __forceinline__ void row_stats8(int col, int V, const float (&v)[8], float& m, float& s) {
    m = -INFINITY;
#pragma unroll
    for (int e = 0; e < 8; e++)
        if (col + e < V) m = fmaxf(m, v[e]);
    m = xor_max<1, 4>(m);
    s = 0.f;
#pragma unroll
    for (int e = 0; e < 8; e++)
        if (col + e < V) s += __expf(v[e] - m);
    s = xor_sum<1, 4>(s);
}
template <bool ZERO_PAD, bool FAST>
__device__ __forceinline__ void row_stats_strip(int ca, int cb, int V, float (&va)[8], float (&vb)[8], float& m, float& s) {
    constexpr float L2E = 1.4426950408889634f;
    s = 0.f;
    if (FAST && __builtin_amdgcn_readfirstlane(ca | 63) < V) {
        m = fmaxf(fmaxf(fmaxf(va[0], va[1]), fmaxf(va[2], va[3])), fmaxf(fmaxf(va[4], va[5]), fmaxf(va[6], va[7])));
        m = fmaxf(m, fmaxf(fmaxf(fmaxf(vb[0], vb[1]), fmaxf(vb[2], vb[3])), fmaxf(fmaxf(vb[4], vb[5]), fmaxf(vb[6], vb[7]))));
        m = xor_max<16, 32>(m);
        const float ml = -m * L2E;
#pragma unroll
        for (int e = 0; e < 8; e++) s += __builtin_amdgcn_exp2f(fmaf(va[e], L2E, ml)) + __builtin_amdgcn_exp2f(fmaf(vb[e], L2E, ml));
    } else {
        m = -INFINITY;
#pragma unroll
        for (int e = 0; e < 8; e++) {
            if (ca + e >= V) { if (ZERO_PAD) va[e] = 0.f; } else m = fmaxf(m, va[e]);
            if (cb + e >= V) { if (ZERO_PAD) vb[e] = 0.f; } else m = fmaxf(m, vb[e]);
        }
        m = xor_max<16, 32>(m);
#pragma unroll
        for (int e = 0; e < 8; e++) {
            if (ca + e < V) s += __expf(va[e] - m);
            if (cb + e < V) s += __expf(vb[e] - m);
        }
    }
    s = xor_sum<16, 32>(s);
}
template <class E>
__device__ __forceinline__ void put_partials(const E& f, int row, int col, float m, float s) {
    const int blk = col >> 6;
    f.pmax[(size_t)row * f.npart + blk] = m;
    f.psum[(size_t)row * f.npart + blk] = (m == -INFINITY) ? 0.f : s;
}

struct EpiLMHead {
    act_t* C;
    float* pmax;
    float* psum;
    const int* target;
    float* tgt_logit;
    int ldc, M, V, npart;
    __device__ __forceinline__ void operator()(int row, int col, float (&v)[8]) const {
        const bool ok = row < M && col < ldc;
        float m = -INFINITY;
#pragma unroll
        for (int e = 0; e < 8; e++) {
            if (col + e >= V) v[e] = 0.f; else m = fmaxf(m, v[e]);
        }
        m = fmaxf(m, __shfl_xor(m, 1, 64));
        m = fmaxf(m, __shfl_xor(m, 2, 64));
        m = fmaxf(m, __shfl_xor(m, 4, 64));
        float s = 0.f;
#pragma unroll
        for (int e = 0; e < 8; e++)
            if (col + e < V) s += __expf(v[e] - m);
        s += __shfl_xor(s, 1, 64);
        s += __shfl_xor(s, 2, 64);
        s += __shfl_xor(s, 4, 64);
        if (!ok) return;
        if ((col & 63) == 0) {
            const int blk = col >> 6;
            pmax[(size_t)row * npart + blk] = m;
            psum[(size_t)row * npart + blk] = (m == -INFINITY) ? 0.f : s;
        }
        const int t = target[row] - col;
        if (t >= 0 && t < 8) tgt_logit[row] = v[t];
        act_st8(C + (size_t)row * ldc + col, v);
    }
    typedef int RowAux;
    __device__ __forceinline__ int load_row(int row) const { return row < M ? target[row] : -1; }
    __device__ __forceinline__ void strip(int row, int ca, int cb, float (&va)[8], float (&vb)[8], int t) const {
        float m, s;
        row_stats_strip<true, true>(ca, cb, V, va, vb, m, s);
        if (row >= M) return;
        if ((ca & 63) == 0 && ca < ldc) put_partials(*this, row, ca, m, s);
        if (ca < ldc) {
            if (t >= ca && t < ca + 8) tgt_logit[row] = va[t - ca];
            act_st8(C + (size_t)row * ldc + ca, va);
        }
        if (cb < ldc) {
            if (t >= cb && t < cb + 8) tgt_logit[row] = vb[t - cb];
            act_st8(C + (size_t)row * ldc + cb, vb);
        }
    }
};
struct EpiLMHeadExp {
    act_t* C;
    float* pmax;
    float* psum;
    const float* cref;
    int ldc, M, V, npart;
    int img = 0;
    __device__ __forceinline__ void operator()(int row, int col, float (&v)[8]) const {
        constexpr float L2E = 1.4426950408889634f;
        const bool ok = row < M && col < ldc;
        const float ml = -(row < M ? cref[row] : 0.f) * L2E;
        float s = 0.f;
#pragma unroll
        for (int e = 0; e < 8; e++) {
            v[e] = (col + e < V) ? __builtin_amdgcn_exp2f(fminf(fmaf(v[e], L2E, ml), 80.f * L2E)) : 0.f;
            s += v[e];
        }
        s += __shfl_xor(s, 1, 64);
        s += __shfl_xor(s, 2, 64);
        s += __shfl_xor(s, 4, 64);
        if (!ok) return;
        if ((col & 63) == 0) {
            const int blk = col >> 6;
            pmax[(size_t)row * npart + blk] = col < V ? cref[row] : -INFINITY;
            psum[(size_t)row * npart + blk] = s;
        }
        epi_store8(C, ldc, row, col, v, img);
    }
    typedef float RowAux;
    __device__ __forceinline__ float load_row(int row) const { return row < M ? cref[row] : 0.f; }
    __device__ __forceinline__ void strip(int row, int ca, int cb, float (&va)[8], float (&vb)[8], float c) const {
        constexpr float L2E = 1.4426950408889634f;
        const float ml = -c * L2E;
        const bool inside = __builtin_amdgcn_readfirstlane(ca | 63) < V;
        float s = 0.f;
#pragma unroll
        for (int e = 0; e < 8; e++) {
            const float ea = __builtin_amdgcn_exp2f(fminf(fmaf(va[e], L2E, ml), 80.f * L2E));
            const float eb = __builtin_amdgcn_exp2f(fminf(fmaf(vb[e], L2E, ml), 80.f * L2E));
            va[e] = (inside || ca + e < V) ? ea : 0.f;
            vb[e] = (inside || cb + e < V) ? eb : 0.f;
            s += va[e] + vb[e];
        }
        s += __shfl_xor(s, 16, 64);
        s += __shfl_xor(s, 32, 64);
        if (row >= M) return;
        if ((ca & 63) == 0 && ca < ldc) {
            const int blk = ca >> 6;
            pmax[(size_t)row * npart + blk] = ca < V ? c : -INFINITY;
            psum[(size_t)row * npart + blk] = s;
        }
        if (ca < ldc) epi_store8(C, ldc, row, ca, va, img);
        if (cb < ldc) epi_store8(C, ldc, row, cb, vb, img);
    }
};
struct EpiLogits {
    float* C;
    float* pmax;
    float* psum;
    int ldc, M, Ns, V, npart;
    __device__ __forceinline__ void operator()(int row, int col, float (&v)[8]) const {
        const bool ok = row < M && col < Ns;
        float m, s;
        row_stats8(col, V, v, m, s);
        if (!ok) return;
        if ((col & 63) == 0) put_partials(*this, row, col, m, s);
        float* p = C + (size_t)row * ldc + col;
        *reinterpret_cast<float4*>(p) = make_float4(v[0], v[1], v[2], v[3]);
        *reinterpret_cast<float4*>(p + 4) = make_float4(v[4], v[5], v[6], v[7]);
    }
    typedef int RowAux;
    __device__ __forceinline__ int load_row(int) const { return 0; }
    __device__ __forceinline__ void strip(int row, int ca, int cb, float (&va)[8], float (&vb)[8], int) const {
        float m, s;
        row_stats_strip<false, false>(ca, cb, V, va, vb, m, s);
        if (row >= M) return;
        if ((ca & 63) == 0 && ca < Ns) put_partials(*this, row, ca, m, s);
        if (ca < Ns) {
            float* p = C + (size_t)row * ldc + ca;
            *reinterpret_cast<float4*>(p) = make_float4(va[0], va[1], va[2], va[3]);
            *reinterpret_cast<float4*>(p + 4) = make_float4(va[4], va[5], va[6], va[7]);
        }
        if (cb < Ns) {
            float* p = C + (size_t)row * ldc + cb;
            *reinterpret_cast<float4*>(p) = make_float4(vb[0], vb[1], vb[2], vb[3]);
            *reinterpret_cast<float4*>(p + 4) = make_float4(vb[4], vb[5], vb[6], vb[7]);
        }
    }
};
struct EpiLMHeadScore {
    float* pmax;
    float* psum;
    const int* target;
    float* tgt_logit;
    int M, N, V, npart;
    __device__ __forceinline__ void operator()(int row, int col, float (&v)[8]) const {
        const bool ok = row < M && col < N;
        float m, s;
        row_stats8(col, V, v, m, s);
        if (!ok) return;
        if ((col & 63) == 0) put_partials(*this, row, col, m, s);
        const int t = target[row] - col;
        if (t >= 0 && t < 8) tgt_logit[row] = v[t];
    }
    typedef int RowAux;
    __device__ __forceinline__ int load_row(int row) const { return row < M ? target[row] : -1; }
    __device__ __forceinline__ void strip(int row, int ca, int cb, float (&va)[8], float (&vb)[8], int t) const {
        float m, s;
        row_stats_strip<false, true>(ca, cb, V, va, vb, m, s);
        if (row >= M) return;
        if ((ca & 63) == 0 && ca < N) put_partials(*this, row, ca, m, s);
        if (t >= ca && t < ca + 8 && ca < N) tgt_logit[row] = va[t - ca];
        if (t >= cb && t < cb + 8 && cb < N) tgt_logit[row] = vb[t - cb];
    }
};
template <> struct epi_row_strip<EpiLogits> { static constexpr bool value = true; };
template <> struct epi_row_strip<EpiLMHead> { static constexpr bool value = true; };
template <> struct epi_row_strip<EpiLMHeadScore> { static constexpr bool value = true; };
template <> struct epi_row_strip<EpiLMHeadExp> { static constexpr bool value = true; };

template <auto Kernel, class... Args>
inline void launch_dyn(dim3 grid, dim3 block, size_t shmem, hipStream_t st, const Args&... args) {
    static bool attr = false;
    if (!attr) { (void)hipFuncSetAttribute((const void*)Kernel, hipFuncAttributeMaxDynamicSharedMemorySize, (int)shmem); attr = true; }
    hipLaunchKernelGGL(Kernel, grid, block, shmem, st, args...);
}
template <class Epi>
inline int launch_gemm_s64(const op16_t* A, int lda, const op16_t* B, int ldb, int M, int N, int K, int ksplit, int nj, const Epi& epi, int* ks_eff,
                           hipStream_t st, const op16_t* Bimg = nullptr);
inline bool x3_fused_on() {
    static const bool on = kX3 && !(cc_lab_env("CC_X3_FUSED") && atoi(cc_lab_env("CC_X3_FUSED")) == 0);
    return on;
}
template <class Epi>
inline int launch_gemm(int al, int bl, const op16_t* A, int lda, const op16_t* B, int ldb, int M, int N, int K,
                       int ksplit, const Epi& epi, hipStream_t st, int tile = -2, int group_m = 0) {
    if (M <= 0 || N <= 0 || K <= 0) return CC_OK;
    if ((lda & 7) || (ldb & 7) || ((uintptr_t)A & 15) || ((uintptr_t)B & 15)) return CC_ERR_SHAPE;
    if (al == 0 && (K & 7)) return CC_ERR_SHAPE;
    if (bl == 0 && (K & 7)) return CC_ERR_SHAPE;
    if (al == 1 && (M & 7)) return CC_ERR_SHAPE;
    if (bl == 1 && (N & 7)) return CC_ERR_SHAPE;
    if constexpr (!epi_row_strip<Epi>::value && !epi_strip_aux<Epi>::value) {
        if (g_gemm_s64 > 0 && al == 0 && bl == 0 && (K % G_BK) == 0 && M <= 1024)
            return launch_gemm_s64(A, lda, B, ldb, M, N, K, ksplit, g_gemm_s64, epi, nullptr, st);
    }
    GemmShape g;
    g.M = M; g.N = N; g.K = K; g.lda = lda; g.ldb = ldb;
    static const int env_group = []() { const char* e = cc_lab_env("CC_GROUP_M"); return e ? atoi(e) : 0; }();
    g.group_m = env_group > 0 ? env_group : (group_m > 0 ? group_m : 8);
    static const int env_stagger = []() { const char* e = cc_lab_env("CC_GEMM_STAGGER"); return e ? atoi(e) : 0; }();
    g.stagger = env_stagger;
    if (ksplit < 1) ksplit = 1;
    int kt = (K + G_BK - 1) / G_BK;
    int per = (kt + ksplit - 1) / ksplit;
    ksplit = (kt + per - 1) / per;
    g.k_chunk = per * G_BK;
    dim3 grid(((M + G_BM - 1) / G_BM) * ((N + G_BN - 1) / G_BN), 1, ksplit);
    const int s256 = tile != -2 ? tile : g_gemm_tile_mode;
    int nj = 0, ni = 8;
    constexpr bool can160 = !kX3 && !epi_row_strip<Epi>::value && !epi_is_dact<Epi>::value;
    constexpr bool zsplit_ok = std::is_same<Epi, EpiF32>::value;
    if (al == 0 && bl == 0 && (K % H_BK) == 0 && (ksplit == 1 || (zsplit_ok && tile > 0)) && s256 != 0) {
        const long tm = (M + H_BM - 1) / H_BM, t128 = (long)grid.x;
        const long t256 = tm * ((N + 255) / 256), t192 = tm * ((N + 191) / 192), t320 = (long)((M + 319) / 320) * ((N + 255) / 256);
        const double c128 = t128 <= 256 ? 16384.0 / 0.75 : (double)((t128 + 511) / 512) * 32768.0;
        const double c256 = (double)((t256 + 255) / 256) * 65536.0 / 1.2, c192 = (double)((t192 + 255) / 256) * 49152.0 / 1.15;
        const double c320 = (double)((t320 + 255) / 256) * 81920.0 / 1.3;
        constexpr bool can192 = !epi_row_strip<Epi>::value;
        constexpr bool can320 = !epi_is_dact<Epi>::value;
        const long t160 = (long)((M + 159) / 160) * ((N + 255) / 256);
        const double c160 = (double)((t160 + 255) / 256) * 40960.0 / 1.1;
        static const bool s160_on = []() { const char* e = cc_lab_env("CC_GEMM_S160"); return !e || atoi(e) != 0; }();
        if (can160 && (s256 == 6 || s256 == 7 || (s256 < 0 && s160_on && ksplit == 1 && c160 < 0.98 * c128 && c160 < 0.98 * c256 && c160 < 0.98 * c320 && (!can192 || c160 < 0.98 * c192)))) { nj = 4; ni = 5; }
        else if (s256 == 5 || (can320 && s256 < 0 && c320 < 0.98 * c128 && c320 < c256 && (!can192 || c320 < c192))) { nj = 4; ni = 10; }
        else if (s256 == 4 || (s256 < 0 && c256 < 0.98 * c128 && (!can192 || c256 <= c192))) nj = 4;
        else if (can192 && (s256 == 3 || (s256 < 0 && c192 < 0.98 * c128))) nj = 3;
    }
    if (nj) {
        const int bm = 32 * ni;
        const size_t sh = (size_t)H_NS * (bm + H_BN) * H_BK * 2;
        const dim3 gr((unsigned)(((M + bm - 1) / bm) * ((N + 64 * nj - 1) / (64 * nj))), 1, (unsigned)ksplit);
        if (nj == 4 && ni == 8) launch_dyn<gemm_nt_stag256_kernel<Epi, 4, false, 8>>(gr, dim3(512), sh, st, A, B, g, epi);
        else if (nj == 4 && ni == 5) {
            if constexpr (can160) {
                static const bool q4_on = []() { const char* e = cc_lab_env("CC_GEMM_Q4"); return !e || atoi(e) != 0; }();
                const bool fits32 = (size_t)M * (size_t)lda * 2 < 0xffff0000ull && (size_t)N * (size_t)ldb * 2 < 0xffff0000ull;
                const int ns = (K % 192 == 0 && K >= 384) ? 3 : ((K % 128 == 0 && K >= 256) ? 2 : 0);
                static const bool q4_last = []() { const char* e = cc_lab_env("CC_Q4_LAST"); return !e || atoi(e) != 0; }();
                g.flags = q4_last ? 0 : 1;
                if (ns && fits32 && ksplit == 1 && s256 != 6 && (q4_on || s256 == 7)) {
                    static const int ncu = []() { int n = 0, dev = 0; (void)hipGetDevice(&dev); (void)hipDeviceGetAttribute(&n, hipDeviceAttributeMultiprocessorCount, dev); return n > 0 ? n : 256; }();
                    const int tiles = ((M + 159) / 160) * ((N + 255) / 256);
                    const dim3 gq((unsigned)(tiles < ncu ? tiles : ncu));
                    if (ns == 3) {
                        launch_dyn<gemm_nt_q4_kernel<Epi, 5, 3>>(gq, dim3(256), (size_t)3 * (160 + 256) * 128, st, A, B, g, epi);
                    } else {
                        launch_dyn<gemm_nt_q4_kernel<Epi, 5, 2>>(gq, dim3(256), (size_t)2 * (160 + 256) * 128, st, A, B, g, epi);
                    }
                } else launch_dyn<gemm_nt_stag256_kernel<Epi, 4, false, 5>>(gr, dim3(512), sh, st, A, B, g, epi);
            }
        }
        else if (nj == 4) launch_dyn<gemm_nt_stag256_kernel<Epi, 4, false, 10>>(gr, dim3(512), sh, st, A, B, g, epi);
        else if constexpr (!epi_row_strip<Epi>::value) {
            bool fused = false;
            if constexpr (kX3) {
                const bool x3f_on = x3_fused_on();
                if (x3f_on && (K % (3 * H_BK)) == 0 && ksplit <= K / (3 * H_BK)) {
                    launch_dyn<gemm_nt_stag256_kernel<Epi, 3, false, 8, true>>(gr, dim3(512), sh, st, A, B, g, epi);
                    fused = true;
                }
            }
            if (!fused) launch_dyn<gemm_nt_stag256_kernel<Epi, 3, false, 8>>(gr, dim3(512), sh, st, A, B, g, epi);
        }
    } else
#ifdef CC_GEMM_ABLATION
    static const int abl = []() { const char* e = cc_lab_env("CC_GEMM_ABL"); return e ? atoi(e) : 0; }();
    if (al == 0 && bl == 0 && (K % G_BK) == 0 && abl == 1) { hipLaunchKernelGGL((gemm_nt_glds_kernel<Epi, 1>), grid, dim3(G_THREADS), 0, st, A, B, g, epi); }
    else if (al == 0 && bl == 0 && (K % G_BK) == 0 && abl == 2) { hipLaunchKernelGGL((gemm_nt_glds_kernel<Epi, 2>), grid, dim3(G_THREADS), 0, st, A, B, g, epi); }
    else if (al == 0 && bl == 0 && (K % G_BK) == 0 && abl == 4) { hipLaunchKernelGGL((gemm_nt_glds_kernel<Epi, 4>), grid, dim3(G_THREADS), 0, st, A, B, g, epi); }
    else if (al == 0 && bl == 0 && (K % G_BK) == 0 && abl == 5) { hipLaunchKernelGGL((gemm_nt_glds_kernel<Epi, 5>), grid, dim3(G_THREADS), 0, st, A, B, g, epi); }
    else if (al == 0 && bl == 0 && (K % G_BK) == 0 && abl == 6) { hipLaunchKernelGGL((gemm_nt_glds_kernel<Epi, 6>), grid, dim3(G_THREADS), 0, st, A, B, g, epi); }
    else
#endif
    if (al == 0 && bl == 0 && (K % G_BK) == 0 && (long)grid.x * grid.z <= 256 && g_gemm_tile_mode != 0 && K / (int)grid.z >= 4 * G_BK) {
        constexpr size_t sh4 = (size_t)8 * G_TILE_BYTES;
        bool fused = false;
        if constexpr (kX3) {
            const bool x3f_on = x3_fused_on();
            if (g_gemm_small_x2 && x3f_on && ksplit == 1 && (K % (3 * G_BK)) == 0) {
                launch_dyn<gemm_nt_glds4x2_x3f_kernel<Epi>>(grid, dim3(2 * G_THREADS), sh4, st, A, B, g, epi);
                fused = true;
            }
        }
        if (fused) {}
        else if (g_gemm_small_x2) launch_dyn<gemm_nt_glds4x2_kernel<Epi>>(grid, dim3(2 * G_THREADS), sh4, st, A, B, g, epi);
        else launch_dyn<gemm_nt_glds4_kernel<Epi>>(grid, dim3(G_THREADS), sh4, st, A, B, g, epi);
    } else if (al == 0 && bl == 0 && (K % G_BK) == 0) {
        bool fused = false;
        if constexpr (kX3) {
            const bool x3f_on = x3_fused_on();
            if (x3f_on && ksplit == 1 && (K % (3 * G_BK)) == 0) {
                hipLaunchKernelGGL((gemm_nt_glds_x3f_kernel<Epi>), grid, dim3(G_THREADS), 0, st, A, B, g, epi);
                fused = true;
            }
        }
        if (!fused) hipLaunchKernelGGL((gemm_nt_glds_kernel<Epi>), grid, dim3(G_THREADS), 0, st, A, B, g, epi);
    }
    else if (al == 0 && bl == 0)
        hipLaunchKernelGGL((gemm_bf16_kernel<0, 0, Epi>), grid, dim3(G_THREADS), 0, st, A, B, g, epi);
    else if (al == 0 && bl == 1)
        hipLaunchKernelGGL((gemm_bf16_kernel<0, 1, Epi>), grid, dim3(G_THREADS), 0, st, A, B, g, epi);
    else if (al == 1 && bl == 1)
        hipLaunchKernelGGL((gemm_bf16_kernel<1, 1, Epi>), grid, dim3(G_THREADS), 0, st, A, B, g, epi);
    else
        return CC_ERR_ARG;
    return hipGetLastError() == hipSuccess ? CC_OK : CC_ERR_LAUNCH;
}

template <class Epi>
inline int launch_gemm_s64(const op16_t* A, int lda, const op16_t* B, int ldb, int M, int N, int K, int ksplit, int nj, const Epi& epi, int* ks_eff,
                           hipStream_t st, const op16_t* Bimg) {
    if ((K % G_BK) || (lda & 7) || (ldb & 7) || ((uintptr_t)A & 15) || ((uintptr_t)B & 15)) return CC_ERR_SHAPE;
    GemmShape g;
    g.M = M; g.N = N; g.K = K; g.lda = lda; g.ldb = ldb;
    g.group_m = 8;
    g.stagger = 0;
    if (ksplit < 1) ksplit = 1;
    const int kt = K / G_BK;
    const int per = (kt + ksplit - 1) / ksplit;
    ksplit = (kt + per - 1) / per;
    g.k_chunk = per * G_BK;
    if (ks_eff) *ks_eff = ksplit;
    const int tm = (M + 63) / 64;
#ifdef CC_EXPERIMENTS
    if (nj == 3 && Bimg && (N % 64) == 0 && ((uintptr_t)Bimg & 15) == 0) {
        constexpr size_t sh = (size_t)4 * 128 * 128;
        launch_dyn<gemm_nt_s64kwb_kernel<Epi, 4>>(dim3((unsigned)(tm * (N / 64)), 1, (unsigned)ksplit), dim3(320), sh, st, A, Bimg, g, epi);
    } else
#else
    (void)Bimg;
#endif
    if (nj == 4) {
        constexpr size_t sh = (size_t)4 * 6 * 16 * 64 * sizeof(float);
        launch_dyn<gemm_nt_s80kw_kernel<Epi>>(dim3((unsigned)(((M + 79) / 80) * ((N + 63) / 64)), 1, (unsigned)ksplit), dim3(G_THREADS), sh, st, A, B, g, epi);
    } else if (nj == 3) {
        constexpr size_t sh = (size_t)4 * 128 * 128;
        launch_dyn<gemm_nt_s64kw_kernel<Epi>>(dim3((unsigned)(tm * ((N + 63) / 64)), 1, (unsigned)ksplit), dim3(G_THREADS), sh, st, A, B, g, epi);
    } else if (nj == 2) {
        launch_dyn<gemm_nt_s64_kernel<Epi, 2, 3, 1>>(dim3((unsigned)(tm * ((N + 127) / 128)), 1, (unsigned)ksplit), dim3(G_THREADS), (size_t)3 * (64 + 128) * 128, st, A, B, g, epi);
    } else {
        launch_dyn<gemm_nt_s64_kernel<Epi, 1, 4, 1>>(dim3((unsigned)(tm * ((N + 63) / 64)), 1, (unsigned)ksplit), dim3(G_THREADS), (size_t)4 * (64 + 64) * 128, st, A, B, g, epi);
    }
    return hipGetLastError() == hipSuccess ? CC_OK : CC_ERR_LAUNCH;
}

template <class Epi>
inline int launch_gemm_tt256(const op16_t* A, int lda, const op16_t* B, int ldb, int M, int N, int K, int ksplit, const Epi& epi, int* ks_eff,
                             hipStream_t st) {
    if ((K % H_BK) || (M & 7) || (N & 7) || (lda & 7) || (ldb & 7) || ((uintptr_t)A & 15) || ((uintptr_t)B & 15)) return CC_ERR_SHAPE;
    GemmShape g;
    g.M = M; g.N = N; g.K = K; g.lda = lda; g.ldb = ldb;
    g.group_m = 8;
    g.stagger = 0;
    if (ksplit < 1) ksplit = 1;
    const int kt = (K + G_BK - 1) / G_BK;
    const int per = (kt + ksplit - 1) / ksplit;
    ksplit = (kt + per - 1) / per;
    g.k_chunk = per * G_BK;
    if (ks_eff) *ks_eff = ksplit;
    constexpr size_t sh = (size_t)H_NS * H_STAGE;
    const dim3 gr((unsigned)(((M + H_BM - 1) / H_BM) * ((N + H_BN - 1) / H_BN)), 1, (unsigned)ksplit);
    launch_dyn<gemm_nt_stag256_kernel<Epi, 4, true>>(gr, dim3(512), sh, st, A, B, g, epi);
    return hipGetLastError() == hipSuccess ? CC_OK : CC_ERR_LAUNCH;
}

constexpr int TT_GROUP_MAX = 32;
struct TTGroup {
    const op16_t* A[TT_GROUP_MAX];
    const op16_t* B[TT_GROUP_MAX];
    GemmShape g[TT_GROUP_MAX];
    float* slab[TT_GROUP_MAX];
    size_t zstride[TT_GROUP_MAX];
    int ldc[TT_GROUP_MAX];
    int first[TT_GROUP_MAX + 1];
    int n;
    int mode;
    int whole = -1, split = 1;
    float* tail = nullptr;
};
__device__ __forceinline__ int tt_group_find(const TTGroup& grp, int L) {
    int i = 0;
    for (int k = 1; k < grp.n; k++)
        if (L >= grp.first[k]) i = k;
    return i;
}
static __global__ __launch_bounds__(G_THREADS, 1) void gemm_tt_glds4_group_kernel(TTGroup grp) {
    extern __shared__ __attribute__((aligned(1024))) char smemt[];
    const int L = xcd_remap(blockIdx.x, gridDim.x);
    const int i = tt_group_find(grp, L);
    const GemmShape g = grp.g[i];
    const int tiles = ((g.M + G_BM - 1) / G_BM) * ((g.N + G_BN - 1) / G_BN);
    const int local = L - grp.first[i];
    const int z = local / tiles, tile = local - z * tiles;
    EpiF32 e{grp.slab[i] + (size_t)z * grp.zstride[i], nullptr, grp.ldc[i], g.M, g.N, grp.mode, 1.0f};
    gemm_tt_glds4_body(grp.A[i], grp.B[i], g, e, tile, z, smemt);
}
static __global__ __launch_bounds__(512, 1) void gemm_tt_stag256_group_kernel(TTGroup grp) {
    extern __shared__ __attribute__((aligned(1024))) char smem[];
    if (grp.whole >= 0) {
        const int b = (int)blockIdx.x;
        const bool cut = b >= grp.whole;
        const int Lt = cut ? grp.whole + (b - grp.whole) / grp.split : xcd_remap(b, grp.whole);
        const int i = tt_group_find(grp, Lt);
// ... 89 lines not shown
```

clipcap_amd/csrc/gemm_inst_lmhead.hip:

```cpp
#include "gemm.hip.h"
#include "gemm_api.h"
namespace CC_NS {
int gemm_lmhead(ActIn A, int lda, const op16_t* B, int ldb, int M, int Vp, int V, int K, Act Co, int ldc, float* pmax,
                float* psum, int npart, const int* target, float* tgt_logit, Call& cx, const float* cref) {
    const hipStream_t st = cx.st;
    act_t* const C = Co.p;
    cc_shared::ProfScope _all(cc_shared::SITE_ALL_GEMMS, st, 2.0 * M * V * (double)K);
    if ((ldc & 63) || ldc < Vp || npart * 64 < Vp) return CC_ERR_SHAPE;
    const op16_t* A16;
    const int rca = nt_operand(cx, A, 0, 0, M, lda, ldb, K, A16);
    if (rca != CC_OK) return rca;
    if (cref) {
        EpiLMHeadExp e{C, pmax, psum, cref, ldc, M, V, npart};
        e.img = Co.img;
        return launch_gemm(0, 0, A16, lda, B, ldb, M, Vp, K, 1, e, st);
    }
    EpiLMHead e{C, pmax, psum, target, tgt_logit, ldc, M, V, npart};
    return launch_gemm(0, 0, A16, lda, B, ldb, M, Vp, K, 1, e, st);
}
int gemm_lmhead_score(ActIn A, int lda, const op16_t* B, int ldb, int M, int Vp, int V, int K, float* pmax, float* psum, int npart,
                      const int* target, float* tgt_logit, Call& cx) {
    const hipStream_t st = cx.st;
    cc_shared::ProfScope _all(cc_shared::SITE_ALL_GEMMS, st, 2.0 * M * V * (double)K);
    if ((Vp & 63) || V > Vp || npart * 64 < Vp) return CC_ERR_SHAPE;
    const op16_t* A16;
    const int rca = nt_operand(cx, A, 0, 0, M, lda, ldb, K, A16);
    if (rca != CC_OK) return rca;
    EpiLMHeadScore e{pmax, psum, target, tgt_logit, M, Vp, V, npart};
    return launch_gemm(0, 0, A16, lda, B, ldb, M, Vp, K, 1, e, st);
}
int gemm_logits_part(ActIn A, int lda, const op16_t* B, int ldb, int M, int Ns, int V, int K, float* C, int ldc, float* pmax, float* psum,
                     int npart, Call& cx) {
    const hipStream_t st = cx.st;
    cc_shared::ProfScope _all(cc_shared::SITE_ALL_GEMMS, st, 2.0 * M * V * (double)K);
    if ((ldc & 3) || (Ns & 7) || npart * 64 < Ns) return CC_ERR_SHAPE;
    const op16_t* A16;
    const int rca = nt_operand(cx, A, 0, 0, M, lda, ldb, K, A16);
    if (rca != CC_OK) return rca;
    EpiLogits e{C, pmax, psum, ldc, M, Ns, V, npart};
    return launch_gemm(0, 0, A16, lda, B, ldb, M, Ns, K, 1, e, st);
}
}
```

clipcap_amd/csrc/kernels.h:

```cpp
#pragma once
#include <algorithm>
#include <cmath>
#include <cstdlib>
#include "common.hip.h"

namespace CC_NS {

int f32_to_bf16(const float* src, op16_t* dst, size_t n, hipStream_t st);
int f32_to_act(const float* src, act_t* dst, size_t n, hipStream_t st);
int wire_pack(const float* src, unsigned short* dst, size_t n, hipStream_t st);
int wire_unpack(const unsigned short* src, float* dst, size_t n, hipStream_t st);
int slice_f32_to_bf16(const float* src, size_t src_stride, act_t* dst, size_t dst_stride, int len, int B, hipStream_t st);
int broadcast_rows(float* dst, size_t dst_stride, const float* src, int len, int B, hipStream_t st);
int add_rows(float* dst, size_t dst_stride, const float* add, int len, int B, hipStream_t st);
constexpr size_t RED_SCRATCH_FLOATS = size_t(1) << 20;
int batch_sum(const float* src, size_t src_stride, float* dst, int len, int B, Call& cx);
int copy_rows(const float* src, size_t src_stride, float* dst, size_t dst_stride, int len, int B, hipStream_t st);

int transpose_bf16(const op16_t* src, op16_t* dst, int R, int C, hipStream_t st);
struct TransposeBatch {
    struct Item { const op16_t* src; op16_t* dst; int R, C; };
    Item it[32];
    int n = 0;
    void add(const op16_t* s, op16_t* d, int R, int C) { it[n++] = Item{s, d, R, C}; }
};
int transpose_bf16_multi(const TransposeBatch& b, hipStream_t st);

int ln_fwd(const float* x, int ldx, const int* row_map, const float* gamma, const float* beta, Act y, float* y32, float* mean,
           float* rstd, int rows, int D, hipStream_t st);
int ln_bwd(const act_t* dy, const float* x, int ldx, const int* row_map, const float* mean, const float* rstd, const float* gamma,
           const float* dres, float* dx32, Act dx16, float* dgamma, float* dbeta, int rows, int D, Call& cx,
           float* dcol = nullptr, Drop dmask = Drop());
int colsum_bf16(const act_t* X, int ld, int M, int N, float* out, Call& cx);
struct ColsumBatch { const act_t* X[32]; float* out[32]; int n = 0; void add(const act_t* x, float* o) { X[n] = x; out[n] = o; n++; } };
int colsum_bf16_multi(const ColsumBatch& b, int ld, int M, int N, Call& cx);

int attn_probs(const act_t* qkv, int B, int S, int H, int hd, float* out, hipStream_t st);
int attn_fwd(const act_t* qkv, int B, int S, int H, int hd, bool causal, Act out, float* lse, hipStream_t st, Drop drop = Drop());
int attn_bwd(const act_t* qkv, const act_t* dout, const act_t* o, const float* lse, float* delta, int B, int S, int H, int hd, bool causal,
             Act dqkv, hipStream_t st, Drop drop = Drop());
bool attn_fwd_can_image(int S, int hd);
bool attn_bwd_can_image(int S, int hd);
int dropout_f32(float* x, size_t n, Drop drop, hipStream_t st);
int dropout_bf16(act_t* x, size_t n, Drop drop, hipStream_t st);
int dropout_mask_u8(unsigned char* out, size_t n, Drop drop, hipStream_t st);

int embed_concat(const float* prefix, const long long* tokens, int cap, const float* wte, const float* wpe, float* x0, int B, int L,
                 int T, int D, int pos0, hipStream_t st);
int f32_to_op16_pad(const float* src, long long lds, int V, act_t* dst, int ldd, int M, hipStream_t st);
constexpr int SCATTER_CHUNK = 512;
constexpr unsigned SC_SKIP = 0xffffffffu;
struct ScatterSrc {
    const int* ids32 = nullptr;
    const long long* ids64 = nullptr;
    const float* f32 = nullptr;
    size_t bstride = 0;
    int rpb = 1;
    size_t ids_ld = 1;
    const act_t* act = nullptr;
    const float* fac = nullptr;
};
size_t scatter_ws_bytes(int R, int D);
int scatter_rows(const ScatterSrc& s, int R, int D, int Vp, float* dst, void* ws, hipStream_t st);

int ce_rows(const float* pmax, const float* psum, int npart, const int* target, const float* tgt_logit, float* lse, float* row_loss,
            float* stats, int M, hipStream_t st);
int score_rows(const float* pmax, const float* psum, int npart, const int* keep, const float* tgt_logit, float* lse, float* token_logprob,
               float* sample_stats, int B, int cap, hipStream_t st);
int ce_dlogits(act_t* logits, int ld, int V, const int* target, const float* lse, const float* denom, const float* loss_scale, int M,
               hipStream_t st, op16_t* img = nullptr);
int ce_targets(const long long* tokens, int* target, int* row_map, int B, int cap, int L, int T, hipStream_t st);
int score_keep(const long long* tokens, int* keep, int n, int ignore_zero, hipStream_t st);
int lm_tgt_ref(const act_t* hf, const op16_t* wte, int D, const int* target, float* cref, int M, hipStream_t st);
int lm_rowfac(const float* cref, const float* lse, const int* target, const float* denom, const float* loss_scale, float* fac, int M, hipStream_t st);
int lm_dgrad_fix(act_t* dhf, const float* fac, const int* target, const op16_t* wte, int D, int M, hipStream_t st);
int lm_scale_rows(const act_t* hf, const float* fac, act_t* out, int D, int M, hipStream_t st);

int adamw(float* p, const float* g, float* m, float* v, size_t n, float lr, float b1, float b2, float eps, float wd, int step, float gscale,
          const float* loss_scale, const float* found_inf, hipStream_t st, op16_t* w16 = nullptr,
          const float* clip = nullptr);
int grad_nonfinite(const float* g, size_t n, float* found_inf, hipStream_t st);
constexpr int GRAD_NORM_BLOCKS = 1024;
constexpr int GRAD_NORM_THREADS = 256;
constexpr int GRAD_NORM_ACC = 4;
int grad_sqnorm(const float* g, size_t n, float* scratch, float* sumsq, hipStream_t st);
int grad_clip_coef(const float* sumsq, float max_norm, float grad_scale, const float* loss_scale, float* clip, hipStream_t st);

int x3_split_rows(const float* src, size_t lds, op16_t* dst, int M, int K, int form, hipStream_t st);
struct X3SplitBatch {
    struct Item { const float* src; op16_t* dst; int R, C, tr, form; };
    Item it[32];
    int n = 0;
    void add(const float* s, op16_t* d, int R, int C, int tr, int form) { it[n++] = Item{s, d, R, C, tr, form}; }
};
int x3_split_multi(const X3SplitBatch& b, hipStream_t st);
int loss_scale_update(float* state, float* found_inf, float growth, float backoff, int interval, hipStream_t st);

}
```

clipcap_amd/csrc/kernels.hip:

```cpp
#include "kernels.h"
#include "gemm_api.h"

namespace CC_NS {

__global__ void k_f32_to_bf16(const float* __restrict__ src, op16_t* __restrict__ dst, size_t n8) {
    for (size_t i = (size_t)blockIdx.x * blockDim.x + threadIdx.x; i < n8; i += (size_t)gridDim.x * blockDim.x) {
        const float4 a = reinterpret_cast<const float4*>(src)[2 * i], b = reinterpret_cast<const float4*>(src)[2 * i + 1];
        float v[8] = {a.x, a.y, a.z, a.w, b.x, b.y, b.z, b.w};
        reinterpret_cast<uint4*>(dst)[i] = pack8(v);
    }
}
int f32_to_bf16(const float* src, op16_t* dst, size_t n, hipStream_t st) {
    if (n & 7) return CC_ERR_SHAPE;
    const size_t n8 = n >> 3;
    if (!n8) return CC_OK;
    const int grid = (int)std::min<size_t>((n8 + 255) / 256, 2048);
    hipLaunchKernelGGL(k_f32_to_bf16, dim3(grid), dim3(256), 0, st, src, dst, n8);
    return CC_OK;
}

__device__ __forceinline__ unsigned short wire_bf16(float f) {
    const unsigned u = __float_as_uint(f);
    if ((u & 0x7fffffffu) > 0x7f800000u) return (unsigned short)((u >> 16) | 0x40u);
    return (unsigned short)((u + 0x7fffu + ((u >> 16) & 1u)) >> 16);
}
__global__ void k_wire_pack(const float* __restrict__ src, unsigned short* __restrict__ dst, size_t n) {
    for (size_t i = ((size_t)blockIdx.x * blockDim.x + threadIdx.x) * 4; i < n; i += (size_t)gridDim.x * blockDim.x * 4) {
        if (i + 4 <= n && ((reinterpret_cast<size_t>(src + i) & 15) == 0) && ((reinterpret_cast<size_t>(dst + i) & 7) == 0)) {
            const float4 a = *reinterpret_cast<const float4*>(src + i);
            *reinterpret_cast<uint2*>(dst + i) = make_uint2(wire_bf16(a.x) | ((unsigned)wire_bf16(a.y) << 16), wire_bf16(a.z) | ((unsigned)wire_bf16(a.w) << 16));
        } else {
            for (size_t j = i; j < n && j < i + 4; j++) dst[j] = wire_bf16(src[j]);
        }
    }
}
__global__ void k_wire_unpack(const unsigned short* __restrict__ src, float* __restrict__ dst, size_t n) {
    for (size_t i = ((size_t)blockIdx.x * blockDim.x + threadIdx.x) * 4; i < n; i += (size_t)gridDim.x * blockDim.x * 4) {
        if (i + 4 <= n && ((reinterpret_cast<size_t>(dst + i) & 15) == 0) && ((reinterpret_cast<size_t>(src + i) & 7) == 0)) {
            const uint2 a = *reinterpret_cast<const uint2*>(src + i);
            *reinterpret_cast<float4*>(dst + i) = make_float4(__uint_as_float(a.x << 16), __uint_as_float(a.x & 0xffff0000u), __uint_as_float(a.y << 16),
                                                              __uint_as_float(a.y & 0xffff0000u));
        } else {
            for (size_t j = i; j < n && j < i + 4; j++) dst[j] = __uint_as_float((unsigned)src[j] << 16);
        }
    }
}
int wire_pack(const float* src, unsigned short* dst, size_t n, hipStream_t st) {
    if (!n) return CC_OK;
    hipLaunchKernelGGL(k_wire_pack, dim3((int)std::min<size_t>((n / 4 + 255) / 256 + 1, 2048)), dim3(256), 0, st, src, dst, n);
    return CC_OK;
}
int wire_unpack(const unsigned short* src, float* dst, size_t n, hipStream_t st) {
    if (!n) return CC_OK;
    hipLaunchKernelGGL(k_wire_unpack, dim3((int)std::min<size_t>((n / 4 + 255) / 256 + 1, 2048)), dim3(256), 0, st, src, dst, n);
    return CC_OK;
}

int f32_to_act(const float* src, act_t* dst, size_t n, hipStream_t st) {
    if constexpr (kX3) {
        if (!n) return CC_OK;
        return hipMemcpyAsync(dst, src, n * sizeof(float), hipMemcpyDeviceToDevice, st) == hipSuccess ? CC_OK : CC_ERR_LAUNCH;
    } else {
        return f32_to_bf16(src, reinterpret_cast<op16_t*>(dst), n, st);
    }
}

__global__ void k_slice_f32_to_bf16(const float* __restrict__ src, size_t src_stride, act_t* __restrict__ dst,
                                    size_t dst_stride, int len8, int B) {
    const size_t total = (size_t)len8 * B;
    for (size_t i = (size_t)blockIdx.x * blockDim.x + threadIdx.x; i < total; i += (size_t)gridDim.x * blockDim.x) {
        const int b = (int)(i / len8), c = (int)(i % len8);
        const float* s = src + b * src_stride + (size_t)c * 8;
        const float4 x = *reinterpret_cast<const float4*>(s), y = *reinterpret_cast<const float4*>(s + 4);
        float v[8] = {x.x, x.y, x.z, x.w, y.x, y.y, y.z, y.w};
        act_st8(dst + b * dst_stride + (size_t)c * 8, v);
    }
}
int slice_f32_to_bf16(const float* src, size_t src_stride, act_t* dst, size_t dst_stride, int len, int B, hipStream_t st) {
    if (len & 7) return CC_ERR_SHAPE;
    const size_t total = (size_t)(len >> 3) * B;
    if (!total) return CC_OK;
    hipLaunchKernelGGL(k_slice_f32_to_bf16, dim3((int)std::min<size_t>((total + 255) / 256, 2048)), dim3(256), 0, st, src,
                       src_stride, dst, dst_stride, len >> 3, B);
    return CC_OK;
}

__global__ void k_broadcast_rows(float* __restrict__ dst, size_t dst_stride, const float* __restrict__ src, int len4, int B) {
    const size_t total = (size_t)len4 * B;
    for (size_t i = (size_t)blockIdx.x * blockDim.x + threadIdx.x; i < total; i += (size_t)gridDim.x * blockDim.x) {
        const int b = (int)(i / len4), c = (int)(i % len4);
        reinterpret_cast<float4*>(dst + b * dst_stride)[c] = reinterpret_cast<const float4*>(src)[c];
    }
}
int broadcast_rows(float* dst, size_t dst_stride, const float* src, int len, int B, hipStream_t st) {
    if (len & 3) return CC_ERR_SHAPE;
    const size_t total = (size_t)(len >> 2) * B;
    if (!total) return CC_OK;
    hipLaunchKernelGGL(k_broadcast_rows, dim3((int)std::min<size_t>((total + 255) / 256, 2048)), dim3(256), 0, st, dst, dst_stride,
                       src, len >> 2, B);
    return CC_OK;
}

__global__ void k_add_rows(float* __restrict__ dst, size_t dst_stride, const float* __restrict__ add, int len, int B) {
    const size_t total = (size_t)len * B;
    for (size_t i = (size_t)blockIdx.x * blockDim.x + threadIdx.x; i < total; i += (size_t)gridDim.x * blockDim.x) {
        const int b = (int)(i / len), c = (int)(i % len);
        dst[b * dst_stride + c] += add[c];
    }
}
int add_rows(float* dst, size_t dst_stride, const float* add, int len, int B, hipStream_t st) {
    const size_t total = (size_t)len * B;
    if (!total) return CC_OK;
    hipLaunchKernelGGL(k_add_rows, dim3((int)std::min<size_t>((total + 255) / 256, 2048)), dim3(256), 0, st, dst, dst_stride, add, len, B);
    return CC_OK;
}

static float* red_scratch(const Call& cx, size_t floats) { return floats <= RED_SCRATCH_FLOATS ? cx.red : nullptr; }

struct FoldOut { float* p[32]; int m; int k; };
__global__ __launch_bounds__(1024) void k_fold_partials(const float* __restrict__ part, int S, int n, FoldOut o) {
    __shared__ float red[16][64];
    const int t = threadIdx.x & 63, g = threadIdx.x >> 6, j = blockIdx.x * 64 + t;
    const float* __restrict__ src = part + (size_t)blockIdx.y * S * n;
    float acc = 0.f;
    if (j < n) {
        for (int k0 = 0; k0 < S; k0 += 256) {
            float v[16];
#pragma unroll
            for (int i = 0; i < 16; i++) {
                const int k = k0 + g + 16 * i;
                v[i] = k < S ? src[(size_t)k * n + j] : 0.f;
            }
#pragma unroll
            for (int w = 8; w >= 1; w >>= 1)
#pragma unroll
                for (int i = 0; i < w; i++) v[i] += v[i + w];
            acc += v[0];
        }
    }
    red[g][t] = acc;
    __syncthreads();
    if (g == 0 && j < n) {
        float s = 0.f;
#pragma unroll
        for (int q = 0; q < 16; q++) s += red[q][t];
        o.p[blockIdx.y * o.k + j / o.m][j % o.m] += s;
    }
}
static int fold_partials(const float* part, int S, int n, int groups, const FoldOut& o, hipStream_t st) {
    hipLaunchKernelGGL(k_fold_partials, dim3((n + 63) / 64, groups), dim3(1024), 0, st, part, S, n, o);
    return hipGetLastError() == hipSuccess ? CC_OK : CC_ERR_LAUNCH;
}

__global__ __launch_bounds__(256) void k_batch_sum(const float* __restrict__ src, size_t src_stride, float* __restrict__ dst, int len, int B,
                                                    int per, float* __restrict__ part) {
    const int i = blockIdx.x * blockDim.x + threadIdx.x;
    if (i >= len) return;
    const int b0 = blockIdx.y * per, b1 = min(B, b0 + per);
    float s0 = 0.f, s1 = 0.f, s2 = 0.f, s3 = 0.f;
    int b = b0;
    for (; b + 3 < b1; b += 4) {
        s0 += src[(size_t)b * src_stride + i];
        s1 += src[(size_t)(b + 1) * src_stride + i];
        s2 += src[(size_t)(b + 2) * src_stride + i];
        s3 += src[(size_t)(b + 3) * src_stride + i];
    }
    for (; b < b1; b++) s0 += src[(size_t)b * src_stride + i];
    const float s = (s0 + s1) + (s2 + s3);
    if (gridDim.y == 1) dst[i] += s;
    else part[(size_t)blockIdx.y * len + i] = s;
}
int batch_sum(const float* src, size_t src_stride, float* dst, int len, int B, Call& cx) {
    const hipStream_t st = cx.st;
    if (!len || B <= 0) return CC_OK;
    const int colb = (len + 255) / 256;
    int slices = std::max(1, std::min(B / 8, 1024 / colb));
    const int per = (B + slices - 1) / slices;
    slices = (B + per - 1) / per;
    float* part = slices > 1 ? red_scratch(cx, (size_t)slices * len) : nullptr;
    if (slices > 1 && !part) return CC_ERR_STATE;
    hipLaunchKernelGGL(k_batch_sum, dim3(colb, slices), dim3(256), 0, st, src, src_stride, dst, len, B, per, part);
    if (slices == 1) return CC_OK;
    FoldOut o{};
    o.p[0] = dst; o.m = len; o.k = 1;
    return fold_partials(part, slices, len, 1, o, st);
}

__global__ void k_copy_rows(const float* __restrict__ src, size_t src_stride, float* __restrict__ dst, size_t dst_stride, int len4, int B) {
    const size_t total = (size_t)len4 * B;
    for (size_t i = (size_t)blockIdx.x * blockDim.x + threadIdx.x; i < total; i += (size_t)gridDim.x * blockDim.x) {
        const int b = (int)(i / len4), c = (int)(i % len4);
        reinterpret_cast<float4*>(dst + b * dst_stride)[c] = reinterpret_cast<const float4*>(src + b * src_stride)[c];
    }
}
int copy_rows(const float* src, size_t src_stride, float* dst, size_t dst_stride, int len, int B, hipStream_t st) {
    if (len & 3) return CC_ERR_SHAPE;
    const size_t total = (size_t)(len >> 2) * B;
    if (!total) return CC_OK;
    hipLaunchKernelGGL(k_copy_rows, dim3((int)std::min<size_t>((total + 255) / 256, 2048)), dim3(256), 0, st, src, src_stride, dst,
                       dst_stride, len >> 2, B);
    return CC_OK;
}

__global__ __launch_bounds__(256) void k_transpose_bf16(const op16_t* __restrict__ src, op16_t* __restrict__ dst, int R, int C) {
    __shared__ op16_t tile[64][66];
    const int r0 = blockIdx.y * 64, c0 = blockIdx.x * 64;
    const int cg = threadIdx.x & 7, rl = threadIdx.x >> 3;
#pragma unroll
    for (int p = 0; p < 2; p++) {
        const int r = r0 + rl + 32 * p, c = c0 + cg * 8;
        uint4 v = make_uint4(0, 0, 0, 0);
        if (r < R && c < C) v = *reinterpret_cast<const uint4*>(src + (size_t)r * C + c);
        const op16_t* e = reinterpret_cast<const op16_t*>(&v);
#pragma unroll
        for (int k = 0; k < 8; k++) tile[rl + 32 * p][cg * 8 + k] = e[k];
    }
    __syncthreads();
#pragma unroll
    for (int p = 0; p < 2; p++) {
        const int c = c0 + rl + 32 * p, r = r0 + cg * 8;
        if (c < C && r < R) {
            op16_t e[8];
#pragma unroll
            for (int k = 0; k < 8; k++) e[k] = tile[cg * 8 + k][rl + 32 * p];
            *reinterpret_cast<uint4*>(dst + (size_t)c * R + r) = *reinterpret_cast<const uint4*>(e);
        }
    }
}
__global__ __launch_bounds__(256) void k_transpose_bf16_multi(TransposeBatch b) {
    const TransposeBatch::Item& m = b.it[blockIdx.z];
    if ((int)blockIdx.x * 64 >= m.C || (int)blockIdx.y * 64 >= m.R) return;
    __shared__ op16_t tile[64][66];
    const int r0 = blockIdx.y * 64, c0 = blockIdx.x * 64, R = m.R, C = m.C;
    const int cg = threadIdx.x & 7, rl = threadIdx.x >> 3;
#pragma unroll
    for (int p = 0; p < 2; p++) {
        const int r = r0 + rl + 32 * p, c = c0 + cg * 8;
        uint4 v = make_uint4(0, 0, 0, 0);
        if (r < R && c < C) v = *reinterpret_cast<const uint4*>(m.src + (size_t)r * C + c);
        const op16_t* e = reinterpret_cast<const op16_t*>(&v);
#pragma unroll
        for (int k = 0; k < 8; k++) tile[rl + 32 * p][cg * 8 + k] = e[k];
    }
    __syncthreads();
#pragma unroll
    for (int p = 0; p < 2; p++) {
        const int c = c0 + rl + 32 * p, r = r0 + cg * 8;
        if (c < C && r < R) {
            op16_t e[8];
#pragma unroll
            for (int k = 0; k < 8; k++) e[k] = tile[cg * 8 + k][rl + 32 * p];
            *reinterpret_cast<uint4*>(m.dst + (size_t)c * R + r) = *reinterpret_cast<const uint4*>(e);
        }
    }
}
int transpose_bf16_multi(const TransposeBatch& b, hipStream_t st) {
    if (b.n <= 0) return CC_OK;
    int mr = 0, mc = 0;
    for (int i = 0; i < b.n; i++) {
        if ((b.it[i].R & 7) || (b.it[i].C & 7)) return CC_ERR_SHAPE;
        mr = std::max(mr, b.it[i].R);
        mc = std::max(mc, b.it[i].C);
    }
    hipLaunchKernelGGL(k_transpose_bf16_multi, dim3((mc + 63) / 64, (mr + 63) / 64, b.n), dim3(256), 0, st, b);
    return hipGetLastError() == hipSuccess ? CC_OK : CC_ERR_LAUNCH;
}
int transpose_bf16(const op16_t* src, op16_t* dst, int R, int C, hipStream_t st) {
    if ((R & 7) || (C & 7)) return CC_ERR_SHAPE;
    if (R <= 0 || C <= 0) return CC_OK;
    hipLaunchKernelGGL(k_transpose_bf16, dim3((C + 63) / 64, (R + 63) / 64), dim3(256), 0, st, src, dst, R, C);
    return CC_OK;
}

constexpr int LN_MAXV = 8;

template <int NV>
__global__ __launch_bounds__(256) void k_ln_fwd(const float* __restrict__ x, int ldx, const int* __restrict__ row_map,
                                                const float* __restrict__ gamma, const float* __restrict__ beta,
                                                act_t* __restrict__ y, float* __restrict__ y32, float* __restrict__ mean,
                                                float* __restrict__ rstd, int rows, int D, float eps, int img) {
    constexpr int R = NV <= 4 ? 2 : 1;
    const int lane = threadIdx.x & 63;
    const int row0 = (blockIdx.x * 4 + (threadIdx.x >> 6)) * R;
    if (row0 >= rows) return;
    float4 v[R][NV], g[NV], bt[NV];
#pragma unroll
    for (int r = 0; r < R; r++) {
        const int row = min(row0 + r, rows - 1);
        const float* xr = x + (size_t)(row_map ? row_map[row] : row) * ldx;
#pragma unroll
        for (int it = 0; it < NV; it++) {
            const int c = lane * 4 + it * 256;
            v[r][it] = c < D ? *reinterpret_cast<const float4*>(xr + c) : make_float4(0, 0, 0, 0);
        }
    }
#pragma unroll
    for (int it = 0; it < NV; it++) {
        const int c = lane * 4 + it * 256;
        g[it] = c < D ? *reinterpret_cast<const float4*>(gamma + c) : make_float4(0, 0, 0, 0);
        bt[it] = c < D ? *reinterpret_cast<const float4*>(beta + c) : make_float4(0, 0, 0, 0);
    }
    float mu[R], rs[R];
#pragma unroll
    for (int r = 0; r < R; r++) {
        float s = 0.f;
#pragma unroll
        for (int it = 0; it < NV; it++) s += v[r][it].x + v[r][it].y + v[r][it].z + v[r][it].w;
        mu[r] = wave_sum(s) / D;
        float q = 0.f;
#pragma unroll
        for (int it = 0; it < NV; it++) {
            const int c = lane * 4 + it * 256;
            if (c < D) {
                const float a = v[r][it].x - mu[r], b = v[r][it].y - mu[r], cc_ = v[r][it].z - mu[r], d = v[r][it].w - mu[r];
                q += a * a + b * b + cc_ * cc_ + d * d;
            }
        }
        rs[r] = rsqrtf(wave_sum(q) / D + eps);
    }
#pragma unroll
    for (int r = 0; r < R; r++) {
        const int row = row0 + r;
        if (row >= rows) break;
        if (lane == 0) {
            if (mean) mean[row] = mu[r];
            if (rstd) rstd[row] = rs[r];
        }
#pragma unroll
        for (int it = 0; it < NV; it++) {
            const int c = lane * 4 + it * 256;
            if (c < D) {
                const float o0 = (v[r][it].x - mu[r]) * rs[r] * g[it].x + bt[it].x, o1 = (v[r][it].y - mu[r]) * rs[r] * g[it].y + bt[it].y;
                const float o2 = (v[r][it].z - mu[r]) * rs[r] * g[it].z + bt[it].z, o3 = (v[r][it].w - mu[r]) * rs[r] * g[it].w + bt[it].w;
#if CC_OP == 2
                if (y && img) {
                    const unsigned h01 = pack2op(o0, o1), h23 = pack2op(o2, o3);
                    float a0, a1, a2, a3;
                    unpack2(h01, a0, a1);
                    unpack2(h23, a2, a3);
                    const uint2 hi = make_uint2(h01, h23), lo = make_uint2(pack2op(o0 - a0, o1 - a1), pack2op(o2 - a2, o3 - a3));
                    op16_t* r3 = reinterpret_cast<op16_t*>(y) + (size_t)row * 3 * D + c;
                    *reinterpret_cast<uint2*>(r3) = hi;
                    *reinterpret_cast<uint2*>(r3 + D) = hi;
                    *reinterpret_cast<uint2*>(r3 + 2 * D) = lo;
                } else
#endif
                if (y) act_st4(y + (size_t)row * D + c, o0, o1, o2, o3);
                if (y32) *reinterpret_cast<float4*>(y32 + (size_t)row * D + c) = make_float4(o0, o1, o2, o3);
            }
        }
    }
}
int ln_fwd(const float* x, int ldx, const int* row_map, const float* gamma, const float* beta, Act yo, float* y32,
           float* mean, float* rstd, int rows, int D, hipStream_t st) {
    if (D > LN_MAXV * 256 || (D & 3) || (ldx & 3)) return CC_ERR_SHAPE;
    if (rows <= 0) return CC_OK;
    const int rpb = D <= 1024 ? 8 : 4;
    const dim3 gr((rows + rpb - 1) / rpb);
    act_t* const y = yo.p;
    const int img = yo.img ? 1 : 0;
    if (img && (!kX3 || yo.img != D)) return CC_ERR_STATE;
#define LN_FWD(NV) hipLaunchKernelGGL(k_ln_fwd<NV>, gr, dim3(256), 0, st, x, ldx, row_map, gamma, beta, y, y32, mean, rstd, rows, D, 1e-5f, img)
    if (D <= 256) LN_FWD(1); else if (D <= 512) LN_FWD(2); else if (D <= 768) LN_FWD(3); else if (D <= 1024) LN_FWD(4); else LN_FWD(LN_MAXV);
#undef LN_FWD
    return CC_OK;
}

template <int NV, bool DG, int NW>
__global__ __launch_bounds__(NW * 64) void k_ln_bwd(const act_t* __restrict__ dy, const float* __restrict__ x, int ldx,
                                                const int* __restrict__ row_map, const float* __restrict__ mean,
                                                const float* __restrict__ rstd, const float* __restrict__ gamma,
                                                const float* __restrict__ dres, float* __restrict__ dx32,
                                                act_t* __restrict__ dx16, float* __restrict__ dgamma, float* __restrict__ dbeta,
                                                float* __restrict__ dcol, int rows, int D, Drop dmask, int img, float* __restrict__ part) {
    extern __shared__ __attribute__((aligned(16))) float ln_red[];
    const int lane = threadIdx.x & 63, wave = threadIdx.x >> 6;
    float4 pg[DG ? NV : 1], pb[DG ? NV : 1], pc[DG ? NV : 1];
#pragma unroll
    for (int it = 0; it < (DG ? NV : 1); it++) pg[it] = pb[it] = pc[it] = make_float4(0, 0, 0, 0);
    float4 gmv[NV];
#pragma unroll
    for (int it = 0; it < NV; it++) {
        const int c = lane * 4 + it * 256;
        gmv[it] = c < D ? *reinterpret_cast<const float4*>(gamma + c) : make_float4(0, 0, 0, 0);
    }
    struct RowIn { act_raw4 d[NV]; float4 xv[NV], rr[NV]; float mu, rs; size_t xr; };
    auto fetch = [&](int row, RowIn& r) {
        r.xr = (size_t)(row_map ? row_map[row] : row) * ldx;
        r.mu = mean[row]; r.rs = rstd[row];
#pragma unroll
        for (int it = 0; it < NV; it++) {
            const int c = lane * 4 + it * 256;
            if (c < D) {
                r.d[it] = act_ldraw4(dy + (size_t)row * D + c);
                r.xv[it] = *reinterpret_cast<const float4*>(x + r.xr + c);
                r.rr[it] = dres ? *reinterpret_cast<const float4*>(dres + r.xr + c) : make_float4(0, 0, 0, 0);
            }
        }
    };
    const int rstep = gridDim.x * NW;
    int row = blockIdx.x * NW + wave;
    RowIn cur;
    if (row < rows) fetch(row, cur);
    for (; row < rows; row += rstep) {
        RowIn nxt;
        const bool more = DG && row + rstep < rows;
        if constexpr (DG) { if (more) fetch(row + rstep, nxt); }
        const size_t xr = cur.xr;
        const float mu = cur.mu, rs = cur.rs;
        float4 g[NV], xh[NV], rr[NV];
        float s1 = 0.f, s2 = 0.f;
#pragma unroll
        for (int it = 0; it < NV; it++) {
            const int c = lane * 4 + it * 256;
            if (c < D) {
                float d0, d1, d2, d3;
                act_unpack4(cur.d[it], d0, d1, d2, d3);
                const float4 xv = cur.xv[it];
                const float4 gm = gmv[it];
                rr[it] = cur.rr[it];
                xh[it] = make_float4((xv.x - mu) * rs, (xv.y - mu) * rs, (xv.z - mu) * rs, (xv.w - mu) * rs);
                g[it] = make_float4(d0 * gm.x, d1 * gm.y, d2 * gm.z, d3 * gm.w);
                s1 += g[it].x + g[it].y + g[it].z + g[it].w;
                s2 += g[it].x * xh[it].x + g[it].y * xh[it].y + g[it].z * xh[it].z + g[it].w * xh[it].w;
                if constexpr (DG) {
                    pg[it].x += d0 * xh[it].x; pg[it].y += d1 * xh[it].y; pg[it].z += d2 * xh[it].z; pg[it].w += d3 * xh[it].w;
                    pb[it].x += d0; pb[it].y += d1; pb[it].z += d2; pb[it].w += d3;
                }
            }
        }
        const float m1 = wave_sum(s1) / D, m2 = wave_sum(s2) / D;
#pragma unroll
        for (int it = 0; it < NV; it++) {
            const int c = lane * 4 + it * 256;
            if (c < D) {
                float4 o = make_float4(rs * (g[it].x - m1 - xh[it].x * m2), rs * (g[it].y - m1 - xh[it].y * m2),
                                       rs * (g[it].z - m1 - xh[it].z * m2), rs * (g[it].w - m1 - xh[it].w * m2));
                o.x += rr[it].x; o.y += rr[it].y; o.z += rr[it].z; o.w += rr[it].w;
                *reinterpret_cast<float4*>(dx32 + xr + c) = o;
                if (dx16) {
                    if (dmask.thresh) {
                        const unsigned e = (unsigned)(xr + c);
                        float m0, m1, m2, m3;
                        drop_mul_pair(dmask, e, m0, m1);
                        drop_mul_pair(dmask, e + 2, m2, m3);
                        o.x *= m0; o.y *= m1; o.z *= m2; o.w *= m3;
                    }
                    const act_raw4 pk = act_pack4(o.x, o.y, o.z, o.w);
#if CC_OP == 2
                    if (img) {
                        const unsigned h01 = pack2op(o.x, o.y), h23 = pack2op(o.z, o.w);
                        float a0, a1, a2, a3;
                        unpack2(h01, a0, a1);
                        unpack2(h23, a2, a3);
                        const uint2 hi = make_uint2(h01, h23), lo = make_uint2(pack2op(o.x - a0, o.y - a1), pack2op(o.z - a2, o.w - a3));
                        op16_t* r3 = reinterpret_cast<op16_t*>(dx16) + 3 * (size_t)xr + c;
                        *reinterpret_cast<uint2*>(r3) = hi;
                        *reinterpret_cast<uint2*>(r3 + D) = hi;
                        *reinterpret_cast<uint2*>(r3 + 2 * D) = lo;
                    } else
#endif
                    act_straw4(dx16 + xr + c, pk);
                    if constexpr (DG) {
                        if (dcol) {
                            float r0, r1, r2, r3;
                            act_unpack4(pk, r0, r1, r2, r3);
                            pc[it].x += r0; pc[it].y += r1; pc[it].z += r2; pc[it].w += r3;
                        }
                    }
                }
            }
        }
        if constexpr (DG) { if (more) cur = nxt; } else { if (row + rstep < rows) fetch(row + rstep, cur); }
    }
    if constexpr (DG) {
        float* rg = ln_red;
        float* rb = ln_red + NW * D;
        float* pp = part + (size_t)blockIdx.x * (dcol ? 3 : 2) * D;
#pragma unroll
        for (int it = 0; it < NV; it++) {
            const int c = lane * 4 + it * 256;
            if (c < D) {
                *reinterpret_cast<float4*>(rg + wave * D + c) = pg[it];
                *reinterpret_cast<float4*>(rb + wave * D + c) = pb[it];
            }
        }
        __syncthreads();
        for (int c = threadIdx.x; c < D; c += NW * 64) {
            float sg = 0.f, sb = 0.f;
#pragma unroll
            for (int w = 0; w < NW; w++) { sg += rg[w * D + c]; sb += rb[w * D + c]; }
            pp[c] = sg;
            pp[D + c] = sb;
        }
        if (dcol) {
            __syncthreads();
#pragma unroll
            for (int it = 0; it < NV; it++) {
                const int c = lane * 4 + it * 256;
                if (c < D) *reinterpret_cast<float4*>(rg + wave * D + c) = pc[it];
            }
            __syncthreads();
            for (int c = threadIdx.x; c < D; c += NW * 64) {
                float sc = 0.f;
#pragma unroll
                for (int w = 0; w < NW; w++) sc += rg[w * D + c];
                pp[2 * D + c] = sc;
            }
        }
    }
}
int ln_bwd(const act_t* dy, const float* x, int ldx, const int* row_map, const float* mean, const float* rstd,
           const float* gamma, const float* dres, float* dx32, Act dxo, float* dgamma, float* dbeta, int rows, int D,
           Call& cx, float* dcol, Drop dmask) {
    const hipStream_t st = cx.st;
    act_t* const dx16 = dxo.p;
    if (D > LN_MAXV * 256 || (D & 3) || (ldx & 3) || (dcol && (!dgamma || !dx16 || row_map)) || (dmask.thresh && (row_map || ldx != D)))
        return CC_ERR_SHAPE;
    if (rows <= 0) return CC_OK;
    const int nw = (dgamma && (size_t)16 * D * sizeof(float) <= 65536) ? 8 : 4;
    static const int dg_grid = []() { const char* e = cc_lab_env("CC_LNBWD_GRID"); return e ? atoi(e) : 256; }();
    const int nvec = dcol ? 3 : 2;
    const int grid = std::min((rows + nw - 1) / nw, dgamma ? std::max(1, std::min(dg_grid, (int)(RED_SCRATCH_FLOATS / ((size_t)nvec * D)))) : 8192);
    float* part = dgamma ? red_scratch(cx, (size_t)grid * nvec * D) : nullptr;
    if (dgamma && !part) return CC_ERR_STATE;
    const size_t sh = dgamma ? (size_t)2 * nw * D * sizeof(float) : 0;
    const int img = dxo.img ? 1 : 0;
    if (img && (!kX3 || dxo.img != D || ldx != D || dcol || dmask.thresh)) return CC_ERR_STATE;
#define LN_BWD(NV, DG, NW) hipLaunchKernelGGL((k_ln_bwd<NV, DG, NW>), dim3(grid), dim3(NW * 64), sh, st, dy, x, ldx, row_map, mean, rstd, gamma, dres, dx32, dx16, dgamma, dbeta, dcol, rows, D, dmask, img, part)
#define LN_BWD_D(DG, NW) { if (D <= 256) LN_BWD(1, DG, NW); else if (D <= 512) LN_BWD(2, DG, NW); else if (D <= 768) LN_BWD(3, DG, NW); else if (D <= 1024) LN_BWD(4, DG, NW); else LN_BWD(LN_MAXV, DG, NW); }
    if (dgamma && nw == 8) LN_BWD_D(true, 8) else if (dgamma) LN_BWD_D(true, 4) else LN_BWD_D(false, 4)
#undef LN_BWD_D
#undef LN_BWD
    if (!dgamma) return CC_OK;
    FoldOut o{};
    o.p[0] = dgamma; o.p[1] = dbeta; o.p[2] = dcol; o.m = D; o.k = nvec;
    return fold_partials(part, grid, nvec * D, 1, o, st);
}

__global__ __launch_bounds__(256) void k_colsum_bf16(const act_t* __restrict__ X, int ld, int M, int N, float* __restrict__ out,
                                                     int rows_per_slice, float* __restrict__ part) {
    __shared__ float red[32][65];
    const int cg = threadIdx.x & 7, rl = threadIdx.x >> 3;
    const int col = blockIdx.x * 64 + cg * 8;
    const int r0 = blockIdx.y * rows_per_slice, r1 = min(M, r0 + rows_per_slice);
    float acc[8] = {0, 0, 0, 0, 0, 0, 0, 0};
    if (col < N) {
        for (int r = r0 + rl; r < r1; r += 32) {
            float f[8];
            act_ld8(X + (size_t)r * ld + col, f);
#pragma unroll
            for (int e = 0; e < 8; e++) acc[e] += f[e];
        }
    }
#pragma unroll
    for (int e = 0; e < 8; e++) red[rl][cg * 8 + e] = acc[e];
    __syncthreads();
    if (threadIdx.x < 64) {
        float s = 0.f;
#pragma unroll
        for (int r = 0; r < 32; r++) s += red[r][threadIdx.x];
        const int c = blockIdx.x * 64 + threadIdx.x;
        if (c < N) {
            if (gridDim.y == 1) out[c] += s;
            else part[(size_t)blockIdx.y * N + c] = s;
        }
    }
}
__global__ __launch_bounds__(256) void k_colsum_bf16_multi(ColsumBatch b, int ld, int M, int N, int rows_per_slice, float* __restrict__ part) {
    __shared__ float red[32][65];
    const act_t* __restrict__ X = b.X[blockIdx.z];
    float* __restrict__ out = b.out[blockIdx.z];
    const int cg = threadIdx.x & 7, rl = threadIdx.x >> 3;
    const int col = blockIdx.x * 64 + cg * 8;
    const int r0 = blockIdx.y * rows_per_slice, r1 = min(M, r0 + rows_per_slice);
    float acc[8] = {0, 0, 0, 0, 0, 0, 0, 0};
    if (col < N) {
        for (int r = r0 + rl; r < r1; r += 32) {
            float f[8];
            act_ld8(X + (size_t)r * ld + col, f);
#pragma unroll
            for (int e = 0; e < 8; e++) acc[e] += f[e];
        }
    }
#pragma unroll
    for (int e = 0; e < 8; e++) red[rl][cg * 8 + e] = acc[e];
    __syncthreads();
    if (threadIdx.x < 64) {
        float s = 0.f;
#pragma unroll
        for (int r = 0; r < 32; r++) s += red[r][threadIdx.x];
        const int c = blockIdx.x * 64 + threadIdx.x;
        if (c < N) {
            if (gridDim.y == 1) out[c] += s;
            else part[((size_t)blockIdx.z * gridDim.y + blockIdx.y) * N + c] = s;
        }
    }
}
int colsum_bf16_multi(const ColsumBatch& b, int ld, int M, int N, Call& cx) {
    const hipStream_t st = cx.st;
    if ((N & 7) || (ld & 7) || b.n < 0 || b.n > 32) return CC_ERR_SHAPE;
    if (M <= 0 || N <= 0 || b.n == 0) return CC_OK;
    const int cb = (N + 63) / 64;
    int slices = std::max(1, std::min((M + 255) / 256, std::max(1, 1024 / (cb * b.n))));
    const int rps = ((M + slices - 1) / slices + 31) / 32 * 32;
    slices = (M + rps - 1) / rps;
    float* part = slices > 1 ? red_scratch(cx, (size_t)b.n * slices * N) : nullptr;
    if (slices > 1 && !part) return CC_ERR_STATE;
    hipLaunchKernelGGL(k_colsum_bf16_multi, dim3(cb, slices, b.n), dim3(256), 0, st, b, ld, M, N, rps, part);
    if (hipGetLastError() != hipSuccess) return CC_ERR_LAUNCH;
    if (slices == 1) return CC_OK;
    FoldOut o{};
    for (int i = 0; i < b.n; i++) o.p[i] = b.out[i];
    o.m = N; o.k = 1;
    return fold_partials(part, slices, N, b.n, o, st);
}
int colsum_bf16(const act_t* X, int ld, int M, int N, float* out, Call& cx) {
    const hipStream_t st = cx.st;
    if ((N & 7) || (ld & 7)) return CC_ERR_SHAPE;
    if (M <= 0 || N <= 0) return CC_OK;
    const int cb = (N + 63) / 64;
    int slices = std::max(1, std::min((M + 255) / 256, 1024 / cb));
    const int rps = ((M + slices - 1) / slices + 31) / 32 * 32;
    slices = (M + rps - 1) / rps;
    float* part = slices > 1 ? red_scratch(cx, (size_t)slices * N) : nullptr;
    if (slices > 1 && !part) return CC_ERR_STATE;
    hipLaunchKernelGGL(k_colsum_bf16, dim3(cb, slices), dim3(256), 0, st, X, ld, M, N, out, rps, part);
    if (slices == 1) return CC_OK;
    FoldOut o{};
    o.p[0] = out; o.m = N; o.k = 1;
    return fold_partials(part, slices, N, 1, o, st);
}

__global__ void k_dropout_f32(float* __restrict__ x, size_t n4, Drop d) {
    for (size_t i = (size_t)blockIdx.x * blockDim.x + threadIdx.x; i < n4; i += (size_t)gridDim.x * blockDim.x) {
        float4 v = reinterpret_cast<float4*>(x)[i];
        const unsigned e = (unsigned)(i * 4);
        float m0, m1, m2, m3;
        drop_mul_pair(d, e, m0, m1);
        drop_mul_pair(d, e + 2, m2, m3);
        v.x *= m0; v.y *= m1; v.z *= m2; v.w *= m3;
        reinterpret_cast<float4*>(x)[i] = v;
    }
}
__global__ void k_dropout_bf16(act_t* __restrict__ x, size_t n8, Drop d) {
    for (size_t i = (size_t)blockIdx.x * blockDim.x + threadIdx.x; i < n8; i += (size_t)gridDim.x * blockDim.x) {
        float f[8];
        act_ld8(x + i * 8, f);
        const unsigned e = (unsigned)(i * 8);
#pragma unroll
        for (int k = 0; k < 8; k += 2) {
            float m0, m1;
            drop_mul_pair(d, e + k, m0, m1);
            f[k] *= m0; f[k + 1] *= m1;
        }
        act_st8(x + i * 8, f);
    }
}
__global__ void k_dropout_mask(unsigned char* __restrict__ out, size_t n, Drop d) {
    for (size_t i = (size_t)blockIdx.x * blockDim.x + threadIdx.x; i < n; i += (size_t)gridDim.x * blockDim.x)
        out[i] = (d.thresh == 0 || drop_keep(d, (unsigned)i)) ? 1 : 0;
}
int dropout_f32(float* x, size_t n, Drop d, hipStream_t st) {
    if (!d.thresh || !n) return CC_OK;
    if (n & 3) return CC_ERR_SHAPE;
    hipLaunchKernelGGL(k_dropout_f32, dim3((int)std::min<size_t>((n / 4 + 255) / 256, 4096)), dim3(256), 0, st, x, n / 4, d);
    return CC_OK;
}
int dropout_bf16(act_t* x, size_t n, Drop d, hipStream_t st) {
    if (!d.thresh || !n) return CC_OK;
    if (n & 7) return CC_ERR_SHAPE;
    hipLaunchKernelGGL(k_dropout_bf16, dim3((int)std::min<size_t>((n / 8 + 255) / 256, 4096)), dim3(256), 0, st, x, n / 8, d);
    return CC_OK;
}
int dropout_mask_u8(unsigned char* out, size_t n, Drop d, hipStream_t st) {
    if (!n) return CC_OK;
    hipLaunchKernelGGL(k_dropout_mask, dim3((int)std::min<size_t>((n + 255) / 256, 4096)), dim3(256), 0, st, out, n, d);
    return CC_OK;
}

__global__ void k_embed_concat(const float* __restrict__ prefix, const long long* __restrict__ tokens, int cap,
                               const float* __restrict__ wte, const float* __restrict__ wpe, float* __restrict__ x0,
                               int B, int L, int T, int D, int pos0) {
    const int d4n = D >> 2;
    const size_t total = (size_t)B * T * d4n;
    for (size_t i = (size_t)blockIdx.x * blockDim.x + threadIdx.x; i < total; i += (size_t)gridDim.x * blockDim.x) {
        const int c = (int)(i % d4n);
        const int t = (int)((i / d4n) % T), b = (int)(i / ((size_t)d4n * T));
        float4 v;
        if (t < L)
            v = reinterpret_cast<const float4*>(prefix + ((size_t)b * L + t) * D)[c];
        else {
            long long id = tokens[(size_t)b * cap + (t - L)];
            if (id < 0) id = 0;
            v = reinterpret_cast<const float4*>(wte + (size_t)id * D)[c];
        }
        const float4 p = reinterpret_cast<const float4*>(wpe + (size_t)(pos0 + t) * D)[c];
        reinterpret_cast<float4*>(x0)[i] = make_float4(v.x + p.x, v.y + p.y, v.z + p.z, v.w + p.w);
    }
}
int embed_concat(const float* prefix, const long long* tokens, int cap, const float* wte, const float* wpe, float* x0, int B, int L,
                 int T, int D, int pos0, hipStream_t st) {
    if (D & 3) return CC_ERR_SHAPE;
    const size_t total = (size_t)B * T * (D >> 2);
    if (!total) return CC_OK;
    hipLaunchKernelGGL(k_embed_concat, dim3((int)std::min<size_t>((total + 255) / 256, 4096)), dim3(256), 0, st, prefix, tokens, cap,
                       wte, wpe, x0, B, L, T, D, pos0);
    return CC_OK;
}

__global__ __launch_bounds__(256) void k_f32_to_op16_pad(const float* __restrict__ src, long long lds, int V, act_t* __restrict__ dst, int ldd,
                                                         int M) {
    const size_t total = (size_t)M * ldd;
    for (size_t i = (size_t)blockIdx.x * blockDim.x + threadIdx.x; i < total; i += (size_t)gridDim.x * blockDim.x) {
        const int c = (int)(i % ldd);
        const size_t r = i / ldd;
        dst[i] = c < V ? f2act(src[r * lds + c]) : (act_t)0;
    }
}
int f32_to_op16_pad(const float* src, long long lds, int V, act_t* dst, int ldd, int M, hipStream_t st) {
    const size_t total = (size_t)M * ldd;
    if (!total) return CC_OK;
    hipLaunchKernelGGL(k_f32_to_op16_pad, dim3((int)std::min<size_t>((total + 255) / 256, 8192)), dim3(256), 0, st, src, lds, V, dst, ldd, M);
    return CC_OK;
}
namespace {
constexpr int SC_TILE = 2048;
typedef unsigned long long sc_key;
struct ScatterWS {
    sc_key *tkeys, *skeys;
    int2* info;
    int *heads, *mstarts, *cnt;
    float* part;
    size_t bytes;
};
ScatterWS sc_carve(void* ws, int R, int D) {
    ScatterWS w{};
    char* base = static_cast<char*>(ws);
    size_t off = 0;
    auto take = [&](size_t n) { off = (off + 255) & ~size_t(255); char* r = base ? base + off : nullptr; off += n; return r; };
    w.tkeys = reinterpret_cast<sc_key*>(take((size_t)R * sizeof(sc_key)));
    w.skeys = reinterpret_cast<sc_key*>(take((size_t)R * sizeof(sc_key)));
    w.info = reinterpret_cast<int2*>(take((size_t)R * sizeof(int2)));
    w.heads = reinterpret_cast<int*>(take((size_t)R * sizeof(int)));
    w.mstarts = reinterpret_cast<int*>(take((size_t)(R / (SCATTER_CHUNK + 1) + 1) * sizeof(int)));
    w.cnt = reinterpret_cast<int*>(take(4 * sizeof(int)));
    w.part = reinterpret_cast<float*>(take((size_t)(2 * (size_t)R / SCATTER_CHUNK) * D * sizeof(float)));
    w.bytes = (off + 255) & ~size_t(255);
    return w;
}

template <bool ACT>
__device__ __forceinline__ void sc_row(const ScatterSrc& s, unsigned r, int D, int d0, float (&v)[4]) {
#pragma clang fp contract(off)
    if (ACT) {
        const float w = -s.fac[2 * (size_t)r + 1];
        const act_t* h = s.act + (size_t)r * D + d0;
#pragma unroll
        for (int e = 0; e < 4; e++) v[e] = w * act2f(h[e]);
    } else {
        const float* f = s.f32 + (size_t)(r / s.rpb) * s.bstride + (size_t)(r % s.rpb) * D + d0;
#pragma unroll
        for (int e = 0; e < 4; e++) v[e] = f[e];
    }
}

__global__ __launch_bounds__(1024) void k_sc_sort_tile(ScatterSrc s, int R, int Vp, int n, sc_key* __restrict__ tkeys) {
    __shared__ sc_key k[SC_TILE];
    const int base = blockIdx.x * SC_TILE;
    for (int i = threadIdx.x; i < n; i += 1024) {
        const int r = base + i;
        sc_key key = ~0ull;
        if (r < R) {
            const size_t ir = (size_t)(r / s.rpb) * s.ids_ld + r % s.rpb;
            long long id = s.ids64 ? s.ids64[ir] : (long long)s.ids32[ir];
            id = id < 0 ? 0 : (id >= Vp ? Vp - 1 : id);
            unsigned hi = (unsigned)id;
            if (s.fac && s.fac[2 * (size_t)r + 1] == 0.f) hi = SC_SKIP;
            key = (sc_key)hi << 32 | (unsigned)r;
        }
        k[i] = key;
    }
    __syncthreads();
    for (int size = 2; size <= n; size <<= 1)
        for (int j = size >> 1; j > 0; j >>= 1) {
            for (int i = threadIdx.x; i < n; i += 1024) {
                const int p = i ^ j;
                if (p > i) {
                    const sc_key a = k[i], b = k[p];
                    if ((a > b) == ((i & size) == 0)) { k[i] = b; k[p] = a; }
                }
            }
            __syncthreads();
        }
    for (int i = threadIdx.x; i < n && base + i < R; i += 1024) tkeys[base + i] = k[i];
}

__global__ __launch_bounds__(256) void k_sc_rank(const sc_key* __restrict__ tkeys, int R, sc_key* __restrict__ skeys, int2* __restrict__ info) {
    __shared__ sc_key t[SC_TILE];
    const int p = blockIdx.x * 256 + threadIdx.x;
    const sc_key key = p < R ? tkeys[p] : ~0ull;
    const unsigned hi = (unsigned)(key >> 32);
    const sc_key lo_key = (sc_key)hi << 32, hi_key = hi == SC_SKIP ? ~0ull : (sc_key)(hi + 1) << 32;
    int pos = 0, ls = 0, le = 0;
    for (int base = 0; base < R; base += SC_TILE) {
        const int n = min(SC_TILE, R - base);
        __syncthreads();
        for (int i = threadIdx.x; i < n; i += 256) t[i] = tkeys[base + i];
        __syncthreads();
        int a = 0, b = 0, c = 0;
        for (int step = SC_TILE; step > 0; step >>= 1) {
            if (a + step <= n && t[a + step - 1] < key) a += step;
            if (b + step <= n && t[b + step - 1] < lo_key) b += step;
            if (c + step <= n && t[c + step - 1] < hi_key) c += step;
        }
        pos += a; ls += b; le += c;
    }
    if (p >= R) return;
    skeys[pos] = key;
    info[pos] = make_int2(ls, hi == SC_SKIP ? 0 : le - ls);
}

__global__ __launch_bounds__(1024) void k_sc_compact(const sc_key* __restrict__ skeys, const int2* __restrict__ info, int R, int* __restrict__ heads,
                                                     int* __restrict__ mstarts, int* __restrict__ cnt) {
    __shared__ int sh[1024], sm[1024];
    const int tid = threadIdx.x, span = (R + 1023) / 1024, a = min(R, tid * span), b = min(R, a + span);
    int nh = 0, nm = 0;
    for (int p = a; p < b; p++) {
        const int2 li = info[p];
        const int off = p - li.x;
        if ((unsigned)(skeys[p] >> 32) == SC_SKIP || off % SCATTER_CHUNK) continue;
        nh++;
        nm += off == 0 && li.y > SCATTER_CHUNK;
    }
    sh[tid] = nh; sm[tid] = nm;
    __syncthreads();
    for (int d = 1; d < 1024; d <<= 1) {
        const int x = tid >= d ? sh[tid - d] : 0, y = tid >= d ? sm[tid - d] : 0;
        __syncthreads();
        sh[tid] += x; sm[tid] += y;
        __syncthreads();
    }
    int oh = sh[tid] - nh, om = sm[tid] - nm;
    if (tid == 1023) { cnt[0] = sh[tid]; cnt[1] = sm[tid]; }
    for (int p = a; p < b; p++) {
        const int2 li = info[p];
        const int off = p - li.x;
        if ((unsigned)(skeys[p] >> 32) == SC_SKIP || off % SCATTER_CHUNK) continue;
        heads[oh++] = p;
        if (off == 0 && li.y > SCATTER_CHUNK) mstarts[om++] = p;
    }
}

template <bool ACT>
__global__ __launch_bounds__(256) void k_sc_sum(ScatterSrc s, const sc_key* __restrict__ skeys, const int2* __restrict__ info,
                                                const int* __restrict__ heads, const int* __restrict__ cnt, int D, int ncb,
                                                float* __restrict__ dst, float* __restrict__ part) {
#pragma clang fp contract(off)
    const int lane = threadIdx.x & 63;
    const int items = cnt[0] * ncb;
    for (int it = blockIdx.x * 4 + (threadIdx.x >> 6); it < items; it += gridDim.x * 4) {
        const int h = it / ncb, d0 = (it % ncb) * 256 + lane * 4;
        const int p = heads[h];
        const int2 li = info[p];
        const int end = min(p + SCATTER_CHUNK, li.x + li.y);
        if (d0 >= D) continue;
        float acc[4];
        sc_row<ACT>(s, (unsigned)skeys[p], D, d0, acc);
        int q = p + 1;
        for (; q + 3 < end; q += 4) {
            float v0[4], v1[4], v2[4], v3[4];
            sc_row<ACT>(s, (unsigned)skeys[q], D, d0, v0);
            sc_row<ACT>(s, (unsigned)skeys[q + 1], D, d0, v1);
            sc_row<ACT>(s, (unsigned)skeys[q + 2], D, d0, v2);
            sc_row<ACT>(s, (unsigned)skeys[q + 3], D, d0, v3);
#pragma unroll
            for (int e = 0; e < 4; e++) acc[e] = (((acc[e] + v0[e]) + v1[e]) + v2[e]) + v3[e];
        }
        for (; q < end; q++) {
            float v[4];
            sc_row<ACT>(s, (unsigned)skeys[q], D, d0, v);
#pragma unroll
            for (int e = 0; e < 4; e++) acc[e] += v[e];
        }
        float* o;
        if (li.y <= SCATTER_CHUNK) o = dst + (size_t)(skeys[p] >> 32) * D + d0;
        else o = part + (size_t)(2 * (size_t)li.x / SCATTER_CHUNK + (p - li.x) / SCATTER_CHUNK) * D + d0;
        if (li.y <= SCATTER_CHUNK) {
#pragma unroll
            for (int e = 0; e < 4; e++) o[e] = o[e] + acc[e];
        } else {
#pragma unroll
            for (int e = 0; e < 4; e++) o[e] = acc[e];
        }
    }
}

__global__ __launch_bounds__(256) void k_sc_fold(const sc_key* __restrict__ skeys, const int2* __restrict__ info, const int* __restrict__ mstarts,
                                                 const int* __restrict__ cnt, int D, int ncb, const float* __restrict__ part, float* __restrict__ dst) {
    const int lane = threadIdx.x & 63;
    const int items = cnt[1] * ncb;
    for (int it = blockIdx.x * 4 + (threadIdx.x >> 6); it < items; it += gridDim.x * 4) {
        const int m = it / ncb, d0 = (it % ncb) * 256 + lane * 4;
        if (d0 >= D) continue;
        const int p = mstarts[m];
        const int n = info[p].y, nk = (n + SCATTER_CHUNK - 1) / SCATTER_CHUNK;
        const float* src = part + (size_t)(2 * (size_t)p / SCATTER_CHUNK) * D + d0;
        float t[4];
#pragma unroll
        for (int e = 0; e < 4; e++) t[e] = src[e];
        for (int k = 1; k < nk; k++)
#pragma unroll
            for (int e = 0; e < 4; e++) t[e] += src[(size_t)k * D + e];
        float* o = dst + (size_t)(skeys[p] >> 32) * D + d0;
#pragma unroll
        for (int e = 0; e < 4; e++) o[e] = o[e] + t[e];
    }
}
}

size_t scatter_ws_bytes(int R, int D) { return R > 0 ? sc_carve(nullptr, R, D).bytes : 0; }

int scatter_rows(const ScatterSrc& s, int R, int D, int Vp, float* dst, void* ws, hipStream_t st) {
    if (R < 0 || D <= 0 || (D & 3) || Vp <= 0 || (!s.ids32 && !s.ids64) || (!s.f32 && !(s.act && s.fac)) || s.rpb <= 0) return CC_ERR_ARG;
    if (R == 0) return CC_OK;
    if (!ws) return CC_ERR_STATE;
    const ScatterWS w = sc_carve(ws, R, D);
    const int nt = (R + SC_TILE - 1) / SC_TILE;
    int n = SC_TILE;
    if (nt == 1) for (n = 1; n < R; n <<= 1) {}
    hipLaunchKernelGGL(k_sc_sort_tile, dim3(nt), dim3(1024), 0, st, s, R, Vp, n, w.tkeys);
    hipLaunchKernelGGL(k_sc_rank, dim3((R + 255) / 256), dim3(256), 0, st, w.tkeys, R, w.skeys, w.info);
    hipLaunchKernelGGL(k_sc_compact, dim3(1), dim3(1024), 0, st, w.skeys, w.info, R, w.heads, w.mstarts, w.cnt);
    const int ncb = (D + 255) / 256;
    const int sum_blocks = (int)std::min<size_t>(((size_t)R * ncb + 3) / 4, 4096);
    if (s.act) hipLaunchKernelGGL(k_sc_sum<true>, dim3(sum_blocks), dim3(256), 0, st, s, w.skeys, w.info, w.heads, w.cnt, D, ncb, dst, w.part);
    else hipLaunchKernelGGL(k_sc_sum<false>, dim3(sum_blocks), dim3(256), 0, st, s, w.skeys, w.info, w.heads, w.cnt, D, ncb, dst, w.part);
    if (R > SCATTER_CHUNK) {
        const int fold_blocks = (int)std::min<size_t>(((size_t)(R / (SCATTER_CHUNK + 1) + 1) * ncb + 3) / 4, 1024);
        hipLaunchKernelGGL(k_sc_fold, dim3(fold_blocks), dim3(256), 0, st, w.skeys, w.info, w.mstarts, w.cnt, D, ncb, w.part, dst);
    }
    return hipGetLastError() == hipSuccess ? CC_OK : CC_ERR_LAUNCH;
}

__device__ __forceinline__ void ce_row_fold(const float* __restrict__ pmax, const float* __restrict__ psum, int npart, int row, int lane,
                                            float& m, float& s) {
    m = -INFINITY;
    s = 0.f;
    if (npart <= 64 * 16) {
        float pm[16], ps[16];
#pragma unroll
        for (int i = 0; i < 16; i++) {
            const int p = lane + 64 * i;
            const bool ok = p < npart;
            const size_t at = (size_t)row * npart + min(p, npart - 1);
            const float a = pmax[at], b = psum[at];
            pm[i] = ok ? a : -INFINITY;
            ps[i] = ok ? b : 0.f;
            m = fmaxf(m, pm[i]);
        }
        m = wave_max(m);
#pragma unroll
        for (int i = 0; i < 16; i++)
            if (pm[i] != -INFINITY) s += ps[i] * __expf(pm[i] - m);
    } else {
        for (int p = lane; p < npart; p += 64) m = fmaxf(m, pmax[(size_t)row * npart + p]);
        m = wave_max(m);
        for (int p = lane; p < npart; p += 64) {
            const float pm = pmax[(size_t)row * npart + p];
            if (pm != -INFINITY) s += psum[(size_t)row * npart + p] * __expf(pm - m);
        }
    }
    s = wave_sum(s);
}
__global__ __launch_bounds__(256) void k_ce_rows(const float* __restrict__ pmax, const float* __restrict__ psum, int npart,
                                                 const int* __restrict__ target, const float* __restrict__ tgt_logit,
                                                 float* __restrict__ lse, float* __restrict__ row_loss, int M) {
    const int lane = threadIdx.x & 63;
    const int row = blockIdx.x * 4 + (threadIdx.x >> 6);
    if (row >= M) return;
    float m, s;
    ce_row_fold(pmax, psum, npart, row, lane, m, s);
    if (lane == 0) {
        const float l = m + logf(s);
        lse[row] = l;
        row_loss[row] = (target[row] != 0) ? l - tgt_logit[row] : 0.f;
    }
}
__global__ __launch_bounds__(1024) void k_ce_stats(const float* __restrict__ row_loss, const int* __restrict__ target, float* __restrict__ stats,
                                                   int M) {
    __shared__ float sl[16], sc[16];
    float a = 0.f, c = 0.f;
    for (int i = threadIdx.x; i < M; i += 1024) {
        a += row_loss[i];
        c += (target[i] != 0) ? 1.f : 0.f;
    }
    a = wave_sum(a);
    c = wave_sum(c);
    if ((threadIdx.x & 63) == 0) { sl[threadIdx.x >> 6] = a; sc[threadIdx.x >> 6] = c; }
    __syncthreads();
    if (threadIdx.x == 0) {
        float ta = 0.f, tc = 0.f;
        for (int w = 0; w < 16; w++) { ta += sl[w]; tc += sc[w]; }
        stats[0] = ta;
        stats[1] = tc;
    }
}
int ce_rows(const float* pmax, const float* psum, int npart, const int* target, const float* tgt_logit, float* lse, float* row_loss,
            float* stats, int M, hipStream_t st) {
    if (M <= 0) return CC_OK;
    hipLaunchKernelGGL(k_ce_rows, dim3((M + 3) / 4), dim3(256), 0, st, pmax, psum, npart, target, tgt_logit, lse, row_loss, M);
    hipLaunchKernelGGL(k_ce_stats, dim3(1), dim3(1024), 0, st, row_loss, target, stats, M);
    return CC_OK;
}

__global__ __launch_bounds__(256) void k_score_rows(const float* __restrict__ pmax, const float* __restrict__ psum, int npart,
                                                    const int* __restrict__ keep, const float* __restrict__ tgt_logit,
                                                    float* __restrict__ lse, float* __restrict__ token_logprob, int M) {
    const int lane = threadIdx.x & 63;
    const int row = blockIdx.x * 4 + (threadIdx.x >> 6);
    if (row >= M) return;
    float m, s;
    ce_row_fold(pmax, psum, npart, row, lane, m, s);
    if (lane == 0) {
        const float l = m + logf(s);
        lse[row] = l;
        token_logprob[row] = keep[row] ? tgt_logit[row] - l : 0.f;
    }
}
__global__ __launch_bounds__(256) void k_score_samples(const float* __restrict__ token_logprob, const int* __restrict__ keep,
                                                       float* __restrict__ sample_stats, int B, int cap) {
    const int lane = threadIdx.x & 63;
    const int b = blockIdx.x * 4 + (threadIdx.x >> 6);
    if (b >= B) return;
    float a = 0.f, c = 0.f;
    for (int i = lane; i < cap; i += 64) {
        a += token_logprob[(size_t)b * cap + i];
        c += keep[(size_t)b * cap + i] ? 1.f : 0.f;
    }
    a = wave_sum(a);
    c = wave_sum(c);
    if (lane == 0) {
        sample_stats[2 * b] = a;
        sample_stats[2 * b + 1] = c;
    }
}
int score_rows(const float* pmax, const float* psum, int npart, const int* keep, const float* tgt_logit, float* lse, float* token_logprob,
               float* sample_stats, int B, int cap, hipStream_t st) {
    const int M = B * cap;
    if (M <= 0) return CC_OK;
    hipLaunchKernelGGL(k_score_rows, dim3((M + 3) / 4), dim3(256), 0, st, pmax, psum, npart, keep, tgt_logit, lse, token_logprob, M);
    hipLaunchKernelGGL(k_score_samples, dim3((B + 3) / 4), dim3(256), 0, st, token_logprob, keep, sample_stats, B, cap);
    return CC_OK;
}

__global__ __launch_bounds__(256) void k_ce_dlogits(act_t* __restrict__ logits, int ld, int V, const int* __restrict__ target,
                                                    const float* __restrict__ lse, const float* __restrict__ denom,
                                                    const float* __restrict__ loss_scale, int M, op16_t* __restrict__ img) {
    const int col = (blockIdx.x * 256 + threadIdx.x) * 8;
    if (col >= ld) return;
    const float inv = (loss_scale ? loss_scale[0] : 1.0f) / fmaxf(denom[0], 1.0f);
    for (int row = blockIdx.y; row < M; row += gridDim.y) {
        const int t = target[row];
        const float l = lse[row];
        const float w = (t != 0) ? inv : 0.f;
        act_t* p = logits + (size_t)row * ld + col;
        float f[8];
        act_ld8(p, f);
#pragma unroll
        for (int e = 0; e < 8; e++) {
            const int c = col + e;
            f[e] = (c < V) ? (__expf(f[e] - l) - (c == t ? 1.f : 0.f)) * w : 0.f;
        }
#if CC_OP == 2
        if (img) {
            const uint4 hi = pack8(f);
            float h[8], d[8];
            unpack8(hi, h);
#pragma unroll
            for (int e = 0; e < 8; e++) d[e] = f[e] - h[e];
            const uint4 lo = pack8(d);
            op16_t* r3 = img + (size_t)row * 3 * ld + col;
            *reinterpret_cast<uint4*>(r3) = hi;
            *reinterpret_cast<uint4*>(r3 + ld) = hi;
            *reinterpret_cast<uint4*>(r3 + 2 * ld) = lo;
            continue;
        }
#endif
        act_st8(p, f);
    }
}
int ce_dlogits(act_t* logits, int ld, int V, const int* target, const float* lse, const float* denom, const float* loss_scale, int M,
               hipStream_t st, op16_t* img) {
    if (ld & 7) return CC_ERR_SHAPE;
    if (M <= 0) return CC_OK;
    hipLaunchKernelGGL(k_ce_dlogits, dim3((ld / 8 + 255) / 256, std::min(M, 32768)), dim3(256), 0, st, logits, ld, V, target, lse, denom, loss_scale, M, img);
    return CC_OK;
}

__global__ __launch_bounds__(256) void k_lm_tgt_ref(const act_t* __restrict__ hf, const op16_t* __restrict__ wte, int D, const int* __restrict__ target,
                                                    float* __restrict__ cref, int M) {
    const int lane = threadIdx.x & 63, row = blockIdx.x * 4 + (threadIdx.x >> 6);
    if (row >= M) return;
    const act_t* h = hf + (size_t)row * D;
#if CC_OP == 2
    const float* w = reinterpret_cast<const float*>(wte) + (size_t)target[row] * D;
#else
    const op16_t* w = wte + (size_t)target[row] * D;
#endif
    float acc = 0.f;
    for (int d = lane * 8; d < D; d += 512) {
        float a[8], b[8];
        act_ld8(h + d, a);
#if CC_OP == 2
        act_ld8(w + d, b);
#else
        unpack8(*reinterpret_cast<const uint4*>(w + d), b);
#endif
#pragma unroll
        for (int e = 0; e < 8; e++) acc += a[e] * b[e];
    }
    acc = wave_sum(acc);
    if (lane == 0) cref[row] = acc;
}
int lm_tgt_ref(const act_t* hf, const op16_t* wte, int D, const int* target, float* cref, int M, hipStream_t st) {
    if (D & 7) return CC_ERR_SHAPE;
    if (M <= 0) return CC_OK;
    hipLaunchKernelGGL(k_lm_tgt_ref, dim3((M + 3) / 4), dim3(256), 0, st, hf, wte, D, target, cref, M);
    return CC_OK;
}
__global__ void k_lm_rowfac(const float* __restrict__ cref, const float* __restrict__ lse, const int* __restrict__ target,
                            const float* __restrict__ denom, const float* __restrict__ loss_scale, float* __restrict__ fac, int M) {
    const int i = blockIdx.x * blockDim.x + threadIdx.x;
    if (i >= M) return;
    const float inv = (loss_scale ? loss_scale[0] : 1.0f) / fmaxf(denom[0], 1.0f);
    const float w = target[i] != 0 ? inv : 0.f;
    fac[2 * i] = w != 0.f ? __expf(cref[i] - lse[i]) * w : 0.f;
    fac[2 * i + 1] = w;
}
int lm_rowfac(const float* cref, const float* lse, const int* target, const float* denom, const float* loss_scale, float* fac, int M, hipStream_t st) {
    if (M <= 0) return CC_OK;
    hipLaunchKernelGGL(k_lm_rowfac, dim3((M + 255) / 256), dim3(256), 0, st, cref, lse, target, denom, loss_scale, fac, M);
    return CC_OK;
}
template <int MODE>
__global__ __launch_bounds__(256) void k_lm_rows(act_t* __restrict__ io, const act_t* __restrict__ hf, const float* __restrict__ fac,
                                                 const int* __restrict__ target, const op16_t* __restrict__ wte, float* __restrict__ dwte, int D, int M) {
    const int d8n = D >> 3;
    const size_t total = (size_t)M * d8n;
    for (size_t i = (size_t)blockIdx.x * blockDim.x + threadIdx.x; i < total; i += (size_t)gridDim.x * blockDim.x) {
        const int row = (int)(i / d8n), c = (int)(i % d8n) * 8;
        const float r = fac[2 * row], w = fac[2 * row + 1];
        float v[8];
        if (MODE == 0) {
            float b[8];
            act_ld8(io + (size_t)row * D + c, v);
#if CC_OP == 2
            act_ld8(reinterpret_cast<const float*>(wte) + (size_t)target[row] * D + c, b);
#else
            unpack8(*reinterpret_cast<const uint4*>(wte + (size_t)target[row] * D + c), b);
#endif
#pragma unroll
            for (int e = 0; e < 8; e++) v[e] = r * v[e] - w * b[e];
            act_st8(io + (size_t)row * D + c, v);
        } else {
            act_ld8(hf + (size_t)row * D + c, v);
#pragma unroll
            for (int e = 0; e < 8; e++) v[e] *= r;
            act_st8(io + (size_t)row * D + c, v);
        }
    }
}
template <int MODE>
static int lm_rows_launch(act_t* io, const act_t* hf, const float* fac, const int* target, const op16_t* wte, float* dwte, int D, int M, hipStream_t st) {
    if (D & 7) return CC_ERR_SHAPE;
    const size_t total = (size_t)M * (D >> 3);
    if (!total) return CC_OK;
    hipLaunchKernelGGL(k_lm_rows<MODE>, dim3((int)std::min<size_t>((total + 255) / 256, 4096)), dim3(256), 0, st, io, hf, fac, target, wte, dwte, D, M);
    return CC_OK;
}
int lm_dgrad_fix(act_t* dhf, const float* fac, const int* target, const op16_t* wte, int D, int M, hipStream_t st) {
    return lm_rows_launch<0>(dhf, nullptr, fac, target, wte, nullptr, D, M, st);
}
int lm_scale_rows(const act_t* hf, const float* fac, act_t* out, int D, int M, hipStream_t st) {
    return lm_rows_launch<1>(out, hf, fac, nullptr, nullptr, nullptr, D, M, st);
}

__global__ void k_ce_targets(const long long* __restrict__ tokens, int* __restrict__ target, int* __restrict__ row_map, int B, int cap,
                             int L, int T) {
    const int i = blockIdx.x * blockDim.x + threadIdx.x;
    if (i >= B * cap) return;
    const int b = i / cap, c = i % cap;
    long long id = tokens[i];
    target[i] = id < 0 ? 0 : (int)id;
    row_map[i] = b * T + L - 1 + c;
}
int ce_targets(const long long* tokens, int* target, int* row_map, int B, int cap, int L, int T, hipStream_t st) {
    if (B * cap <= 0) return CC_OK;
    hipLaunchKernelGGL(k_ce_targets, dim3((B * cap + 255) / 256), dim3(256), 0, st, tokens, target, row_map, B, cap, L, T);
    return CC_OK;
}
__global__ void k_score_keep(const long long* __restrict__ tokens, int* __restrict__ keep, int n, int ignore_zero) {
    const int i = blockIdx.x * blockDim.x + threadIdx.x;
    if (i >= n) return;
    const long long id = tokens[i];
    keep[i] = (id >= 0 && !(ignore_zero && id == 0)) ? 1 : 0;
}
int score_keep(const long long* tokens, int* keep, int n, int ignore_zero, hipStream_t st) {
    if (n <= 0) return CC_OK;
    hipLaunchKernelGGL(k_score_keep, dim3((n + 255) / 256), dim3(256), 0, st, tokens, keep, n, ignore_zero);
    return CC_OK;
}

template <bool DEVSTEP>
__global__ __launch_bounds__(256) void k_adamw(float* __restrict__ p, const float* __restrict__ g, float* __restrict__ m,
                                               float* __restrict__ v, size_t n4, float lr, float b1, float b2, float eps, float wd, float bc1,
                                               float bc2_sqrt, float gscale, const float* __restrict__ loss_scale,
                                               const float* __restrict__ found_inf, op16_t* __restrict__ w16,
                                               const float* __restrict__ clip) {
    if (found_inf && found_inf[0] != 0.f) return;
    if (loss_scale) gscale /= loss_scale[0];
    if (clip) gscale *= clip[0];
    if constexpr (DEVSTEP) {
        const float t = loss_scale[2] + 1.0f;
        bc1 = 1.0f - __builtin_amdgcn_exp2f(t * __log2f(b1));
        bc2_sqrt = sqrtf(1.0f - __builtin_amdgcn_exp2f(t * __log2f(b2)));
    }
    for (size_t i = (size_t)blockIdx.x * blockDim.x + threadIdx.x; i < n4; i += (size_t)gridDim.x * blockDim.x) {
        float4 P = reinterpret_cast<float4*>(p)[i], G = reinterpret_cast<const float4*>(g)[i];
        float4 M = reinterpret_cast<float4*>(m)[i], V = reinterpret_cast<float4*>(v)[i];
        float* pp = &P.x; float* gg = &G.x; float* mm = &M.x; float* vv = &V.x;
#pragma unroll
        for (int e = 0; e < 4; e++) {
            const float gr = gg[e] * gscale;
            pp[e] *= (1.0f - lr * wd);
            mm[e] = b1 * mm[e] + (1.0f - b1) * gr;
            vv[e] = b2 * vv[e] + (1.0f - b2) * gr * gr;
            const float denom = sqrtf(vv[e]) / bc2_sqrt + eps;
            pp[e] -= (lr / bc1) * (mm[e] / denom);
        }
        reinterpret_cast<float4*>(p)[i] = P;
        reinterpret_cast<float4*>(m)[i] = M;
        reinterpret_cast<float4*>(v)[i] = V;
        if (w16) reinterpret_cast<uint2*>(w16)[i] = make_uint2(pack2op(P.x, P.y), pack2op(P.z, P.w));
    }
}
int adamw(float* p, const float* g, float* m, float* v, size_t n, float lr, float b1, float b2, float eps, float wd, int step, float gscale,
          const float* loss_scale, const float* found_inf, hipStream_t st, op16_t* w16, const float* clip) {
    if (n & 3) return CC_ERR_SHAPE;
    if (!n) return CC_OK;
    if (step < 1 && !loss_scale) return CC_ERR_ARG;
    const float bc1 = 1.0f - powf(b1, (float)std::max(step, 1));
    const float bc2s = sqrtf(1.0f - powf(b2, (float)std::max(step, 1)));
    const size_t n4 = n >> 2;
    const dim3 gr((int)std::min<size_t>((n4 + 255) / 256, 4096));
    if (step < 1) hipLaunchKernelGGL(k_adamw<true>, gr, dim3(256), 0, st, p, g, m, v, n4, lr, b1, b2, eps, wd, bc1, bc2s, gscale, loss_scale, found_inf, w16, clip);
    else hipLaunchKernelGGL(k_adamw<false>, gr, dim3(256), 0, st, p, g, m, v, n4, lr, b1, b2, eps, wd, bc1, bc2s, gscale, loss_scale, found_inf, w16, clip);
    return CC_OK;
}

__global__ __launch_bounds__(256) void k_grad_nonfinite(const float* __restrict__ g, size_t n4, float* __restrict__ found_inf) {
    bool bad = false;
    for (size_t i = (size_t)blockIdx.x * blockDim.x + threadIdx.x; i < n4; i += (size_t)gridDim.x * blockDim.x) {
        const float4 G = reinterpret_cast<const float4*>(g)[i];
        const float z = (G.x - G.x) + (G.y - G.y) + (G.z - G.z) + (G.w - G.w);
        bad |= !(z == 0.f);
    }
    if (__any(bad) && (threadIdx.x & 63) == 0) found_inf[0] = 1.0f;
}
int grad_nonfinite(const float* g, size_t n, float* found_inf, hipStream_t st) {
    if (n & 3) return CC_ERR_SHAPE;
    if (!n) return CC_OK;
    const size_t n4 = n >> 2;
    hipLaunchKernelGGL(k_grad_nonfinite, dim3((int)std::min<size_t>((n4 + 255) / 256, 2048)), dim3(256), 0, st, g, n4, found_inf);
    return CC_OK;
}
__global__ void k_loss_scale_update(float* state, float* found_inf, float growth, float backoff, int interval) {
    if (threadIdx.x != 0 || blockIdx.x != 0) return;
    if (found_inf[0] != 0.f) {
        state[0] = fmaxf(state[0] * backoff, 1.0f);
        state[1] = 0.f;
    } else {
        const float good = state[1] + 1.f;
        if (good >= (float)interval) {
            state[0] = fminf(state[0] * growth, 16777216.0f);
            state[1] = 0.f;
        } else {
            state[1] = good;
        }
        state[2] += 1.f;
    }
    found_inf[0] = 0.f;
}
int loss_scale_update(float* state, float* found_inf, float growth, float backoff, int interval, hipStream_t st) {
    hipLaunchKernelGGL(k_loss_scale_update, dim3(1), dim3(64), 0, st, state, found_inf, growth, backoff, interval);
    return CC_OK;
}

__device__ __forceinline__ float sq4(const float4 G) { return (G.x * G.x + G.y * G.y) + (G.z * G.z + G.w * G.w); }
__global__ __launch_bounds__(GRAD_NORM_THREADS) void k_grad_sqnorm(const float* __restrict__ g, size_t n4, float* __restrict__ part) {
    static_assert(GRAD_NORM_THREADS == 256 && GRAD_NORM_ACC == 4, "the fold below is written for 4 waves and 4 accumulators");
    __shared__ float red[4];
    const float4* g4 = reinterpret_cast<const float4*>(g);
    const size_t S = (size_t)gridDim.x * GRAD_NORM_THREADS;
    size_t i = (size_t)blockIdx.x * GRAD_NORM_THREADS + threadIdx.x;
    float a0 = 0.f, a1 = 0.f, a2 = 0.f, a3 = 0.f;
    for (; i + 3 * S < n4; i += 4 * S) {
        const float4 G0 = g4[i], G1 = g4[i + S], G2 = g4[i + 2 * S], G3 = g4[i + 3 * S];
        a0 += sq4(G0); a1 += sq4(G1); a2 += sq4(G2); a3 += sq4(G3);
    }
    if (i < n4) a0 += sq4(g4[i]);
    if (i + S < n4) a1 += sq4(g4[i + S]);
    if (i + 2 * S < n4) a2 += sq4(g4[i + 2 * S]);
    const float w = wave_sum((a0 + a1) + (a2 + a3));
// ... 145 lines not shown
```

Before: 22730 samples/s.

## Fuse small launches, drop redundant memsets, and trim prefix-only backward work

Merges the embedding cast with the prefix broadcast, and the dout seeding with the memset/copy/cast, into single kernels. The full-buffer memsets are replaced by zeroing only the unmapped rows. The exp-form LM head stops writing pmax, and the CE row reduction only sums psum against cref. For frozen-LM prefix-only training, the last GPT-2 layer-norm backward computes only the prefix rows and writes them straight to dprefix, skipping the full-sequence LN backward, dropout and row copy. These changes remove launches and memory traffic, but add correctness risk around which dx32 rows are left uninitialized.

```diff
diff --git a/clipcap_amd/csrc/api.hip b/clipcap_amd/csrc/api.hip
--- a/clipcap_amd/csrc/api.hip
+++ b/clipcap_amd/csrc/api.hip
@@ -355,7 +355,7 @@
     if (!mapper_cfg_ok(c) || B <= 0 || !w32 || !w16 || !emb || !ws || !out) return CC_ERR_ARG;
     MapperPass ps(c, B, save, ws, stream);
     auto& [st, o, w, cx, D, PP, S, M, H, hd, Hm, PD] = ps;
-    CC_TRY(f32_to_act(emb, w.emb16, (size_t)B * c->W * c->E, st));
+    CC_TRY(cast_and_broadcast(emb, w.emb16, (size_t)B * c->W * c->E, w.x[0] + (size_t)PP * D, (size_t)S * D, w32 + o.prefix, c->L * D, B, st));
     if (c->W == 1) {
         CC_TRY(gemm_f32out(0, 0, w.emb16, c->E, W16(w16, o.lin_w), c->E, B, PD, c->E, w.x[0], S * D, w32 + o.lin_b, 0, 1.0f, 1, cx));
     } else {
@@ -363,7 +363,6 @@
         CC_TRY(copy_rows(w.lin_tmp, (size_t)PP * D, w.x[0], (size_t)S * D, PP * D, B, st));
         if (o.pos >= 0) CC_TRY(add_rows(w.x[0], (size_t)S * D, w32 + o.pos, PP * D, B, st));
     }
-    CC_TRY(broadcast_rows(w.x[0] + (size_t)PP * D, (size_t)S * D, w32 + o.prefix, c->L * D, B, st));
     for (int l = 0; l < c->N; l++) {
         const auto y = o.layer(l);
         CC_TRY(ln_fwd(w.x[l], D, nullptr, w32 + y.n1w, w32 + y.n1b, w.xn1[l], nullptr, w.mean1[l], w.rstd1[l], M, D, st));
@@ -396,11 +395,7 @@
     MapperPass ps(c, B, 1, ws, stream);
     auto& [st, o, w, cx, D, PP, S, M, H, hd, Hm, PD] = ps;
     const uint16_t* w16t = W16(w16, o.total);
-    if (l_hi == c->N) {
-        if (hipMemsetAsync(w.dx32, 0, (size_t)M * D * sizeof(float), st) != hipSuccess) return CC_ERR_LAUNCH;
-        CC_TRY(copy_rows(dout, (size_t)c->L * D, w.dx32 + (size_t)PP * D, (size_t)S * D, c->L * D, B, st));
-        if (c->N > 0) CC_TRY(f32_to_act(w.dx32, w.gdx[c->N - 1], (size_t)M * D, st));
-    }
+    if (l_hi == c->N) CC_TRY(seed_rows(dout, w.dx32, c->N > 0 ? w.gdx[c->N - 1] : nullptr, PP, c->L, D, B, st));
     WgradBatch wb;
     wb.defer = true;
     constexpr bool kDeferAll = !kX3;
@@ -629,7 +624,7 @@
     Gpt2Pass ps(c, s, cap, ws, stream);
     auto& [st, o, w, cx, D, M, H, hd] = ps;
     const int Mc = s->B * cap, npart = c->Vp / 64;
-    if (hipMemsetAsync(stats, 0, 2 * sizeof(float), st) != hipSuccess) return CC_ERR_LAUNCH;
+    if (Mc <= 0 && hipMemsetAsync(stats, 0, 2 * sizeof(float), st) != hipSuccess) return CC_ERR_LAUNCH;
     CC_TRY(ce_targets(reinterpret_cast<const long long*>(tokens), w.target, w.row_map, s->B, cap, s->L, s->T, st));
     CC_TRY(ln_fwd(w.x[c->NL], D, w.row_map, w32 + o.lnf_w, w32 + o.lnf_b, w.hf16, nullptr, w.meanf, w.rstdf, Mc, D, st));
     const bool ef = lm_exp_form(s);
@@ -637,7 +632,8 @@
     if (ef) CC_TRY(lm_tgt_ref(w.hf16, wte_rows, D, w.target, w.cref, Mc, st));
     CC_TIMED(CC_SITE_LMHEAD_FWD, st, gemm_lmhead(w.hf16, D, W16(w16, o.wte), D, Mc, c->Vp, c->V, D, lm_logits(c, s, w.logits16), c->Vp, w.pmax, w.psum, npart, w.target, w.tgt_logit, cx,
                                                  ef ? w.cref : nullptr));
-    CC_TRY(ce_rows(w.pmax, w.psum, npart, w.target, ef ? w.cref : w.tgt_logit, w.lse_row, w.row_loss, stats, Mc, st));
+    if (ef) CC_TRY(ce_rows_exp(w.psum, npart, w.target, w.cref, w.lse_row, w.row_loss, stats, Mc, st));
+    else CC_TRY(ce_rows(w.pmax, w.psum, npart, w.target, w.tgt_logit, w.lse_row, w.row_loss, stats, Mc, st));
     return CC_OK;
 }
 
@@ -659,7 +655,7 @@
 
 int CC_API(cc_lmhead_ce_bwd)(const cc_gpt2_cfg* c, const cc_gpt2_shape* s, const float* w32, const uint16_t* w16, void* ws, const float* denom,
                      const float* loss_scale, float* g32, void* stream) {
-    if (!gpt2_cfg_ok(c) || !shape_ok(c, s) || s->mode < 1 || !w32 || !w16 || !ws || !denom || (s->mode == 2 && !g32)) return CC_ERR_ARG;
+    if (!gpt2_cfg_ok(c) || !shape_ok(c, s) || s->mode < 1 || s->L < 1 || !w32 || !w16 || !ws || !denom || (s->mode == 2 && !g32)) return CC_ERR_ARG;
     const int cap = s->T - s->L;
     Gpt2Pass ps(c, s, cap, ws, stream);
     auto& [st, o, w, cx, D, M, H, hd] = ps;
@@ -693,9 +689,8 @@
             CC_TRY(gemm_wgrad(lg, c->Vp, w.hf16, D, c->Vp, D, Mc, g32 + o.wte, D, w.wg_scratch, cx));
         }
     }
-    if (hipMemsetAsync(w.dx32, 0, (size_t)M * D * sizeof(float), st) != hipSuccess) return CC_ERR_LAUNCH;
-    const size_t dx16_bytes = (size_t)M * D * (w.dx16.img ? 3 * sizeof(op16_t) : sizeof(act_t));
-    if (hipMemsetAsync(w.dx16.p, 0, dx16_bytes, st) != hipSuccess) return CC_ERR_LAUNCH;
+    const size_t dx16_row = (size_t)D * (w.dx16.img ? 3 * sizeof(op16_t) : sizeof(act_t));
+    CC_TRY(zero_unmapped_rows(w.dx32, (size_t)D * sizeof(float), w.dx16.p, dx16_row, s->B, s->L, s->T, st));
     CC_TRY(ln_bwd(w.dhf16, w.x[c->NL], D, w.row_map, w.meanf, w.rstdf, w32 + o.lnf_w, nullptr, w.dx32, w.dx16, full ? g32 + o.lnf_w : nullptr,
                   full ? g32 + o.lnf_b : nullptr, Mc, D, cx));
     return CC_OK;
@@ -739,7 +734,6 @@
     CC_TRY(f32_to_op16_pad(dlogits, ldl, c->V, w.logits16, c->Vp, M, st));
     CC_TRY(gemm_bf16out(0, 0, w.logits16, c->Vp, W16(w16, o.total + o.wte), c->Vp, M, D, c->Vp, w.dhf16, D, nullptr, 0, nullptr, cx));
     if (full) CC_TRY(gemm_wgrad(w.logits16, c->Vp, w.hf16, D, c->Vp, D, M, g32 + o.wte, D, w.wg_scratch, cx));
-    if (hipMemsetAsync(w.dx32, 0, (size_t)M * D * sizeof(float), st) != hipSuccess) return CC_ERR_LAUNCH;
     CC_TRY(ln_bwd(w.dhf16, w.x[c->NL], D, nullptr, w.meanf, w.rstdf, w32 + o.lnf_w, nullptr, w.dx32, w.dx16, full ? g32 + o.lnf_w : nullptr,
                   full ? g32 + o.lnf_b : nullptr, M, D, cx));
     CC_TRY(CC_API(cc_gpt2_bwd_range)(c, s, w32, w16, ws, nullptr, nullptr, g32, c->NL, 0, stream));
@@ -765,6 +759,8 @@
     WgradBatch wb;
     wb.defer = full;
     WgradBatch* wbp = full ? &wb : nullptr;
+    const Drop embd_drop = make_drop(s->p_embd, s->drop_seed, DROP_EMBD, 0);
+    const bool prefix_only = s->mode == 1 && s->L > 0 && dprefix && s->p_embd == 0.f;
     if (full && (w.dx16.img || w.dx16b.img || w.du16.img || w.dqkv16.img)) return CC_ERR_STATE;
     for (int l = l_hi - 1; l >= l_lo; l--) {
         const auto y = o.layer(l);
@@ -797,12 +793,16 @@
         }
         CC_TRY(gemm_bf16out(0, 0, w.dqkv16, D3, W16(w16, y.aw), D3, M, D, D3, w.dxn16, D, nullptr, 0, nullptr, cx));
         if (full) CC_TRY(wgrad_flush(wb, st));
+        if (l == 0 && prefix_only) {
+            CC_TRY(ln_bwd_prefix(w.dxn16, w.x[0], w.mean1[0], w.rstd1[0], w32 + y.l1w, w.dx32, dprefix, s->B, s->L, s->T, D, st));
+            return CC_OK;
+        }
         CC_TRY(ln_bwd(w.dxn16, w.x[l], D, nullptr, w.mean1[l], w.rstd1[l], w32 + y.l1w, w.dx32, w.dx32, w.dx16, full ? g32 + y.l1w : nullptr,
                       full ? g32 + y.l1b : nullptr, M, D, cx, (full && l > 0) ? g32 + o.layer(l - 1).p2b : nullptr,
                       l > 0 ? make_drop(s->p_resid, s->drop_seed, DROP_RESID_MLP, l - 1) : Drop()));
     }
     if (l_lo > 0) return CC_OK;
-    CC_TRY(dropout_f32(w.dx32, (size_t)M * D, make_drop(s->p_embd, s->drop_seed, DROP_EMBD, 0), st));
+    CC_TRY(dropout_f32(w.dx32, (size_t)M * D, embd_drop, st));
     if (s->L > 0) CC_TRY(copy_rows(w.dx32, (size_t)s->T * D, dprefix, (size_t)s->L * D, s->L * D, s->B, st));
     if (full) {
         if (tokens) {
diff --git a/clipcap_amd/csrc/gemm.hip.h b/clipcap_amd/csrc/gemm.hip.h
--- a/clipcap_amd/csrc/gemm.hip.h
+++ b/clipcap_amd/csrc/gemm.hip.h
@@ -1801,7 +1801,6 @@
 };
 struct EpiLMHeadExp {
     act_t* C;
-    float* pmax;
     float* psum;
     const float* cref;
     int ldc, M, V, npart;
@@ -1820,11 +1819,7 @@
         s += __shfl_xor(s, 2, 64);
         s += __shfl_xor(s, 4, 64);
         if (!ok) return;
-        if ((col & 63) == 0) {
-            const int blk = col >> 6;
-            pmax[(size_t)row * npart + blk] = col < V ? cref[row] : -INFINITY;
-            psum[(size_t)row * npart + blk] = s;
-        }
+        if ((col & 63) == 0) psum[(size_t)row * npart + (col >> 6)] = s;
         epi_store8(C, ldc, row, col, v, img);
     }
     typedef float RowAux;
@@ -1845,11 +1840,7 @@
         s += __shfl_xor(s, 16, 64);
         s += __shfl_xor(s, 32, 64);
         if (row >= M) return;
-        if ((ca & 63) == 0 && ca < ldc) {
-            const int blk = ca >> 6;
-            pmax[(size_t)row * npart + blk] = ca < V ? c : -INFINITY;
-            psum[(size_t)row * npart + blk] = s;
-        }
+        if ((ca & 63) == 0 && ca < ldc) psum[(size_t)row * npart + (ca >> 6)] = s;
         if (ca < ldc) epi_store8(C, ldc, row, ca, va, img);
         if (cb < ldc) epi_store8(C, ldc, row, cb, vb, img);
     }
diff --git a/clipcap_amd/csrc/gemm_inst_lmhead.hip b/clipcap_amd/csrc/gemm_inst_lmhead.hip
--- a/clipcap_amd/csrc/gemm_inst_lmhead.hip
+++ b/clipcap_amd/csrc/gemm_inst_lmhead.hip
@@ -11,7 +11,7 @@
     const int rca = nt_operand(cx, A, 0, 0, M, lda, ldb, K, A16);
     if (rca != CC_OK) return rca;
     if (cref) {
-        EpiLMHeadExp e{C, pmax, psum, cref, ldc, M, V, npart};
+        EpiLMHeadExp e{C, psum, cref, ldc, M, V, npart};
         e.img = Co.img;
         return launch_gemm(0, 0, A16, lda, B, ldb, M, Vp, K, 1, e, st);
     }
diff --git a/clipcap_amd/csrc/kernels.h b/clipcap_amd/csrc/kernels.h
--- a/clipcap_amd/csrc/kernels.h
+++ b/clipcap_amd/csrc/kernels.h
@@ -7,15 +7,17 @@
 namespace CC_NS {
 
 int f32_to_bf16(const float* src, op16_t* dst, size_t n, hipStream_t st);
-int f32_to_act(const float* src, act_t* dst, size_t n, hipStream_t st);
 int wire_pack(const float* src, unsigned short* dst, size_t n, hipStream_t st);
 int wire_unpack(const unsigned short* src, float* dst, size_t n, hipStream_t st);
 int slice_f32_to_bf16(const float* src, size_t src_stride, act_t* dst, size_t dst_stride, int len, int B, hipStream_t st);
-int broadcast_rows(float* dst, size_t dst_stride, const float* src, int len, int B, hipStream_t st);
 int add_rows(float* dst, size_t dst_stride, const float* add, int len, int B, hipStream_t st);
 constexpr size_t RED_SCRATCH_FLOATS = size_t(1) << 20;
 int batch_sum(const float* src, size_t src_stride, float* dst, int len, int B, Call& cx);
 int copy_rows(const float* src, size_t src_stride, float* dst, size_t dst_stride, int len, int B, hipStream_t st);
+int zero_unmapped_rows(void* a, size_t a_row, void* b, size_t b_row, int B, int L, int T, hipStream_t st);
+int seed_rows(const float* src, float* d32, act_t* d16, int PP, int L, int D, int B, hipStream_t st);
+int cast_and_broadcast(const float* src, act_t* dst16, size_t n, float* brd, size_t brd_stride, const float* blk, int len, int B,
+                       hipStream_t st);
 
 int transpose_bf16(const op16_t* src, op16_t* dst, int R, int C, hipStream_t st);
 struct TransposeBatch {
@@ -31,6 +33,8 @@
 int ln_bwd(const act_t* dy, const float* x, int ldx, const int* row_map, const float* mean, const float* rstd, const float* gamma,
            const float* dres, float* dx32, Act dx16, float* dgamma, float* dbeta, int rows, int D, Call& cx,
            float* dcol = nullptr, Drop dmask = Drop());
+int ln_bwd_prefix(const act_t* dy, const float* x, const float* mean, const float* rstd, const float* gamma, const float* dres,
+                  float* dprefix, int B, int L, int T, int D, hipStream_t st);
 int colsum_bf16(const act_t* X, int ld, int M, int N, float* out, Call& cx);
 struct ColsumBatch { const act_t* X[32]; float* out[32]; int n = 0; void add(const act_t* x, float* o) { X[n] = x; out[n] = o; n++; } };
 int colsum_bf16_multi(const ColsumBatch& b, int ld, int M, int N, Call& cx);
@@ -65,6 +69,8 @@
 
 int ce_rows(const float* pmax, const float* psum, int npart, const int* target, const float* tgt_logit, float* lse, float* row_loss,
             float* stats, int M, hipStream_t st);
+int ce_rows_exp(const float* psum, int npart, const int* target, const float* cref, float* lse, float* row_loss, float* stats, int M,
+                hipStream_t st);
 int score_rows(const float* pmax, const float* psum, int npart, const int* keep, const float* tgt_logit, float* lse, float* token_logprob,
                float* sample_stats, int B, int cap, hipStream_t st);
 int ce_dlogits(act_t* logits, int ld, int V, const int* target, const float* lse, const float* denom, const float* loss_scale, int M,
diff --git a/clipcap_amd/csrc/kernels.hip b/clipcap_amd/csrc/kernels.hip
--- a/clipcap_amd/csrc/kernels.hip
+++ b/clipcap_amd/csrc/kernels.hip
@@ -54,15 +54,6 @@
     if (!n) return CC_OK;
     hipLaunchKernelGGL(k_wire_unpack, dim3((int)std::min<size_t>((n / 4 + 255) / 256 + 1, 2048)), dim3(256), 0, st, src, dst, n);
     return CC_OK;
-}
-
-int f32_to_act(const float* src, act_t* dst, size_t n, hipStream_t st) {
-    if constexpr (kX3) {
-        if (!n) return CC_OK;
-        return hipMemcpyAsync(dst, src, n * sizeof(float), hipMemcpyDeviceToDevice, st) == hipSuccess ? CC_OK : CC_ERR_LAUNCH;
-    } else {
-        return f32_to_bf16(src, reinterpret_cast<op16_t*>(dst), n, st);
-    }
 }
 
 __global__ void k_slice_f32_to_bf16(const float* __restrict__ src, size_t src_stride, act_t* __restrict__ dst,
@@ -82,22 +73,6 @@
     if (!total) return CC_OK;
     hipLaunchKernelGGL(k_slice_f32_to_bf16, dim3((int)std::min<size_t>((total + 255) / 256, 2048)), dim3(256), 0, st, src,
                        src_stride, dst, dst_stride, len >> 3, B);
-    return CC_OK;
-}
-
-__global__ void k_broadcast_rows(float* __restrict__ dst, size_t dst_stride, const float* __restrict__ src, int len4, int B) {
-    const size_t total = (size_t)len4 * B;
-    for (size_t i = (size_t)blockIdx.x * blockDim.x + threadIdx.x; i < total; i += (size_t)gridDim.x * blockDim.x) {
-        const int b = (int)(i / len4), c = (int)(i % len4);
-        reinterpret_cast<float4*>(dst + b * dst_stride)[c] = reinterpret_cast<const float4*>(src)[c];
-    }
-}
-int broadcast_rows(float* dst, size_t dst_stride, const float* src, int len, int B, hipStream_t st) {
-    if (len & 3) return CC_ERR_SHAPE;
-    const size_t total = (size_t)(len >> 2) * B;
-    if (!total) return CC_OK;
-    hipLaunchKernelGGL(k_broadcast_rows, dim3((int)std::min<size_t>((total + 255) / 256, 2048)), dim3(256), 0, st, dst, dst_stride,
-                       src, len >> 2, B);
     return CC_OK;
 }
 
@@ -199,6 +174,80 @@
     if (!total) return CC_OK;
     hipLaunchKernelGGL(k_copy_rows, dim3((int)std::min<size_t>((total + 255) / 256, 2048)), dim3(256), 0, st, src, src_stride, dst,
                        dst_stride, len >> 2, B);
+    return CC_OK;
+}
+
+__global__ void k_zero_unmapped_rows(uint4* __restrict__ a, int a16, uint4* __restrict__ b, int b16, int B, int L, int T) {
+    const int per = a16 + b16;
+    const size_t total = (size_t)per * L * B;
+    for (size_t i = (size_t)blockIdx.x * blockDim.x + threadIdx.x; i < total; i += (size_t)gridDim.x * blockDim.x) {
+        const int r = (int)(i / per), c = (int)(i % per);
+        const int s = r / L, k = r % L;
+        const size_t row = (size_t)s * T + (k < L - 1 ? k : T - 1);
+        if (c < a16) a[row * a16 + c] = make_uint4(0, 0, 0, 0);
+        else b[row * b16 + (c - a16)] = make_uint4(0, 0, 0, 0);
+    }
+}
+int zero_unmapped_rows(void* a, size_t a_row, void* b, size_t b_row, int B, int L, int T, hipStream_t st) {
+    if ((a_row & 15) || (b_row & 15) || L < 1 || L > T) return CC_ERR_SHAPE;
+    const size_t total = (a_row + b_row) / 16 * L * B;
+    if (!total) return CC_OK;
+    hipLaunchKernelGGL(k_zero_unmapped_rows, dim3((int)std::min<size_t>((total + 255) / 256, 2048)), dim3(256), 0, st,
+                       reinterpret_cast<uint4*>(a), (int)(a_row / 16), reinterpret_cast<uint4*>(b), (int)(b_row / 16), B, L, T);
+    return CC_OK;
+}
+
+__global__ void k_seed_rows(const float* __restrict__ src, float* __restrict__ d32, act_t* __restrict__ d16, int PP, int L, int D8, int B) {
+    const int S = PP + L;
+    const size_t total = (size_t)S * D8 * B;
+    for (size_t i = (size_t)blockIdx.x * blockDim.x + threadIdx.x; i < total; i += (size_t)gridDim.x * blockDim.x) {
+        const int c = (int)(i % D8);
+        const size_t row = i / D8;
+        const int b = (int)(row / S), s = (int)(row % S);
+        float4 x = make_float4(0, 0, 0, 0), y = x;
+        if (s >= PP) {
+            const float* p = src + (((size_t)b * L + (s - PP)) * D8 + c) * 8;
+            x = *reinterpret_cast<const float4*>(p);
+            y = *reinterpret_cast<const float4*>(p + 4);
+        }
+        reinterpret_cast<float4*>(d32)[2 * i] = x;
+        reinterpret_cast<float4*>(d32)[2 * i + 1] = y;
+        if (d16) {
+            const float v[8] = {x.x, x.y, x.z, x.w, y.x, y.y, y.z, y.w};
+            act_st8(d16 + i * 8, v);
+        }
+    }
+}
+int seed_rows(const float* src, float* d32, act_t* d16, int PP, int L, int D, int B, hipStream_t st) {
+    if (D & 7) return CC_ERR_SHAPE;
+    const size_t total = (size_t)(PP + L) * (D >> 3) * B;
+    if (!total) return CC_OK;
+    hipLaunchKernelGGL(k_seed_rows, dim3((int)std::min<size_t>((total + 255) / 256, 2048)), dim3(256), 0, st, src, d32, d16, PP, L, D >> 3, B);
+    return CC_OK;
+}
+
+__global__ void k_cast_and_broadcast(const float* __restrict__ src, act_t* __restrict__ dst16, size_t n8, float* __restrict__ brd,
+                                     size_t brd_stride, const float* __restrict__ blk, int len4, int B) {
+    const size_t total = n8 + (size_t)len4 * B;
+    for (size_t i = (size_t)blockIdx.x * blockDim.x + threadIdx.x; i < total; i += (size_t)gridDim.x * blockDim.x) {
+        if (i < n8) {
+            const float4 a = reinterpret_cast<const float4*>(src)[2 * i], b = reinterpret_cast<const float4*>(src)[2 * i + 1];
+            const float v[8] = {a.x, a.y, a.z, a.w, b.x, b.y, b.z, b.w};
+            act_st8(dst16 + i * 8, v);
+        } else {
+            const size_t j = i - n8;
+            const int b = (int)(j / len4), c = (int)(j % len4);
+            reinterpret_cast<float4*>(brd + b * brd_stride)[c] = reinterpret_cast<const float4*>(blk)[c];
+        }
+    }
+}
+int cast_and_broadcast(const float* src, act_t* dst16, size_t n, float* brd, size_t brd_stride, const float* blk, int len, int B,
+                       hipStream_t st) {
+    if ((n & 7) || (len & 3)) return CC_ERR_SHAPE;
+    const size_t total = (n >> 3) + (size_t)(len >> 2) * B;
+    if (!total) return CC_OK;
+    hipLaunchKernelGGL(k_cast_and_broadcast, dim3((int)std::min<size_t>((total + 255) / 256, 2048)), dim3(256), 0, st, src, dst16, n >> 3,
+                       brd, brd_stride, blk, len >> 2, B);
     return CC_OK;
 }
 
@@ -366,7 +415,7 @@
     return CC_OK;
 }
 
-template <int NV, bool DG, int NW>
+template <int NV, bool DG, int NW, bool PFX = false>
 __global__ __launch_bounds__(NW * 64) void k_ln_bwd(const act_t* __restrict__ dy, const float* __restrict__ x, int ldx,
                                                 const int* __restrict__ row_map, const float* __restrict__ mean,
                                                 const float* __restrict__ rstd, const float* __restrict__ gamma,
@@ -385,14 +434,21 @@
         gmv[it] = c < D ? *reinterpret_cast<const float4*>(gamma + c) : make_float4(0, 0, 0, 0);
     }
     struct RowIn { act_raw4 d[NV]; float4 xv[NV], rr[NV]; float mu, rs; size_t xr; };
+    static_assert(!PFX || !DG, "the prefix form has no parameter gradients");
     auto fetch = [&](int row, RowIn& r) {
-        r.xr = (size_t)(row_map ? row_map[row] : row) * ldx;
-        r.mu = mean[row]; r.rs = rstd[row];
+        int in = row;
+        if constexpr (PFX) {
+            in = (row / img) * (ldx / D) + row % img;
+            r.xr = (size_t)in * D;
+        } else {
+            r.xr = (size_t)(row_map ? row_map[row] : row) * ldx;
+        }
+        r.mu = mean[in]; r.rs = rstd[in];
 #pragma unroll
         for (int it = 0; it < NV; it++) {
             const int c = lane * 4 + it * 256;
             if (c < D) {
-                r.d[it] = act_ldraw4(dy + (size_t)row * D + c);
+                r.d[it] = act_ldraw4(dy + (size_t)in * D + c);
                 r.xv[it] = *reinterpret_cast<const float4*>(x + r.xr + c);
                 r.rr[it] = dres ? *reinterpret_cast<const float4*>(dres + r.xr + c) : make_float4(0, 0, 0, 0);
             }
@@ -437,7 +493,7 @@
                 float4 o = make_float4(rs * (g[it].x - m1 - xh[it].x * m2), rs * (g[it].y - m1 - xh[it].y * m2),
                                        rs * (g[it].z - m1 - xh[it].z * m2), rs * (g[it].w - m1 - xh[it].w * m2));
                 o.x += rr[it].x; o.y += rr[it].y; o.z += rr[it].z; o.w += rr[it].w;
-                *reinterpret_cast<float4*>(dx32 + xr + c) = o;
+                *reinterpret_cast<float4*>(dx32 + (PFX ? (size_t)row * D : xr) + c) = o;
                 if (dx16) {
                     if (dmask.thresh) {
                         const unsigned e = (unsigned)(xr + c);
@@ -537,6 +593,17 @@
     o.p[0] = dgamma; o.p[1] = dbeta; o.p[2] = dcol; o.m = D; o.k = nvec;
     return fold_partials(part, grid, nvec * D, 1, o, st);
 }
+int ln_bwd_prefix(const act_t* dy, const float* x, const float* mean, const float* rstd, const float* gamma, const float* dres,
+                  float* dprefix, int B, int L, int T, int D, hipStream_t st) {
+    if (D > LN_MAXV * 256 || (D & 3) || L < 1 || L > T || (size_t)T * D > 0x7fffffffu) return CC_ERR_SHAPE;
+    const int rows = B * L;
+    if (rows <= 0) return CC_OK;
+    const int grid = std::min((rows + 3) / 4, 8192);
+#define LN_BWD_P(NV) hipLaunchKernelGGL((k_ln_bwd<NV, false, 4, true>), dim3(grid), dim3(256), 0, st, dy, x, T * D, nullptr, mean, rstd, gamma, dres, dprefix, nullptr, nullptr, nullptr, nullptr, rows, D, Drop(), L, nullptr)
+    if (D <= 256) LN_BWD_P(1); else if (D <= 512) LN_BWD_P(2); else if (D <= 768) LN_BWD_P(3); else if (D <= 1024) LN_BWD_P(4); else LN_BWD_P(LN_MAXV);
+#undef LN_BWD_P
+    return CC_OK;
+}
 
 __global__ __launch_bounds__(256) void k_colsum_bf16(const act_t* __restrict__ X, int ld, int M, int N, float* __restrict__ out,
                                                      int rows_per_slice, float* __restrict__ part) {
@@ -987,6 +1054,34 @@
         row_loss[row] = (target[row] != 0) ? l - tgt_logit[row] : 0.f;
     }
 }
+__global__ __launch_bounds__(256) void k_ce_rows_exp(const float* __restrict__ psum, int npart, const int* __restrict__ target,
+                                                     const float* __restrict__ cref, float* __restrict__ lse,
+                                                     float* __restrict__ row_loss, int M) {
+    const int lane = threadIdx.x & 63;
+    const int row = blockIdx.x * 4 + (threadIdx.x >> 6);
+    if (row >= M) return;
+    float s = 0.f;
+    if (npart <= 64 * 16) {
+        float ps[16];
+#pragma unroll
+        for (int i = 0; i < 16; i++) {
+            const int p = lane + 64 * i;
+            const float b = psum[(size_t)row * npart + min(p, npart - 1)];
+            ps[i] = p < npart ? b : 0.f;
+        }
+#pragma unroll
+        for (int i = 0; i < 16; i++) s += ps[i];
+    } else {
+        for (int p = lane; p < npart; p += 64) s += psum[(size_t)row * npart + p];
+    }
+    s = wave_sum(s);
+    if (lane == 0) {
+        const float m = cref[row];
+        const float l = m + logf(s);
+        lse[row] = l;
+        row_loss[row] = (target[row] != 0) ? l - m : 0.f;
+    }
+}
 __global__ __launch_bounds__(1024) void k_ce_stats(const float* __restrict__ row_loss, const int* __restrict__ target, float* __restrict__ stats,
                                                    int M) {
     __shared__ float sl[16], sc[16];
@@ -1010,6 +1105,13 @@
             float* stats, int M, hipStream_t st) {
     if (M <= 0) return CC_OK;
     hipLaunchKernelGGL(k_ce_rows, dim3((M + 3) / 4), dim3(256), 0, st, pmax, psum, npart, target, tgt_logit, lse, row_loss, M);
+    hipLaunchKernelGGL(k_ce_stats, dim3(1), dim3(1024), 0, st, row_loss, target, stats, M);
+    return CC_OK;
+}
+int ce_rows_exp(const float* psum, int npart, const int* target, const float* cref, float* lse, float* row_loss, float* stats, int M,
+                hipStream_t st) {
+    if (M <= 0) return CC_OK;
+    hipLaunchKernelGGL(k_ce_rows_exp, dim3((M + 3) / 4), dim3(256), 0, st, psum, npart, target, cref, lse, row_loss, M);
     hipLaunchKernelGGL(k_ce_stats, dim3(1), dim3(1024), 0, st, row_loss, target, stats, M);
     return CC_OK;
 }
```

Measured after the change: 22720 samples/s (median of 2 runs). Within noise of the previous version (-0.0%).
